# hidasib/GRU4Rec

Hardware: AMD Instinct MI355X
Metric: mini-batches/sec (gru4rec.py:661), RSC15-shaped batch=128 n_sample=2048 BPR-max (higher is better)
Workload: dtype f32

## Files before the change

gru4rec_amd/build.py:

```python
import glob
import os
import subprocess
import sys

HERE = os.path.dirname(os.path.abspath(__file__))
SRC = os.path.join(HERE, 'csrc', 'g4r_api.hip')
SRC_HOST = os.path.join(HERE, 'csrc', 'g4r_io.cpp')
OUT = os.path.join(HERE, 'libgru4rec_hip.so')
DEPS = sorted(p for ext in ('hip', 'cuh', 'hpp', 'cpp') for p in glob.glob(os.path.join(HERE, 'csrc', '*.' + ext))) + \
       [os.path.join(os.path.dirname(HERE), 'include', 'gru4rec_hip.h'), os.path.abspath(__file__)]


def build(force=False, verbose=False, out=None, defs=(), flags=()):
    if out is not None:
        return _compile(out, list(defs), verbose, list(flags))
    if not force and os.path.exists(OUT) and all(os.path.getmtime(OUT) >= os.path.getmtime(d) for d in DEPS):
        return OUT
    return _compile(OUT, [], verbose)


COMMON_FLAGS = ['-mllvm', '-amdgpu-kernarg-preload-count=16']


MUTANTS = {1: 'sparse accumulator increments x 1.01', 2: 'sparse Adagrad steps x 1.01', 3: 'dense accumulator increments x 1.01',
           4: "round 3's stale-register pipeline of gemm_tile2k (tied wait operands in two branches): fails the ISA audit, so it is the "
              "one library built with audit=False",
           5: 'the 1 / nranks factor of the exact-replica joint update (REDUCE / MEAN forms) x 1.01',
           6: 'the Adagrad step of ONE item row per step (the item of score column 0) x 1.5: a single wrong row must not pass',
           7: 'top-k selection (g4r_recommend_step) breaks equal scores by the HIGHER column',
           8: "k_update_l's owner scan skips the last id of every 1024-id slice after the first (an occurrence of a hot item lost)",
           9: "the merge-time exclusion search of g4r_recommend_step_filtered never matches the LAST item of a row's sorted list",
           10: "k_replay_final (g4r_recommend_sessions) reads every row's final state from the buffer of the chunk's LONGEST history",
           11: "k_score_cand (g4r_score_candidates*): a work item past a row's first slice reads the items of the row's first slice",
           12: "the two-stage top-k (g4r_recommend_*_scan) ranks its candidates by the APPROXIMATE bf16 scores: the fp32 re-scoring is skipped",
           13: "cosine (g4r_similar_items): the candidate's inverse norm is read at the candidate POSITION instead of its item index",
           14: "k_rollout_feed (g4r_continue_sessions): the sorted insertion drops an item that sorts ABOVE every item already in the row's "
               "exclusion list, so it is never excluded and can be generated again",
           15: "k_beam_advance (g4r_beam_sessions) reads the hidden state of beam row i ITSELF instead of the row of its parent: a new beam "
               "carries on from the wrong state wherever the selection re-parents",
           16: "the owner walk of k_sparse_update_generic drops the first hit of every pass after the first (an item with more than 64 "
               "earlier occurrences in a step loses one of them per later pass)",
           17: "opt_rule's new second statistic (adadelta's update average, Adam's mean) x 1.01",
           18: "k_loss_rows' grp_fast takes a group of V columns whose last column is the first inactive in-batch one (column M) as wholly "
               "active: the unmasked copy of the element loops runs over it",
           19: "k_loss_rows' first pass starts its loop past the prefetched groups one STEP late: the columns of the first trip keep "
               "whatever the LDS held",
           20: "gumbel_noise (g4r_sample_sessions) ignores the decoding step (Philox counter word 2 = 0): every step of a draw gets the "
               "noise of step 0"}


def mutant_path(k):
    return os.path.join(HERE, '_variants', 'libgru4rec_hip_mut%d.so' % k)


def build_mutants(force=False, verbose=False):
    import fcntl
    from concurrent.futures import ThreadPoolExecutor
    os.makedirs(os.path.join(HERE, '_variants'), exist_ok=True)

    def stale():
        return [k for k in MUTANTS if force or not os.path.exists(mutant_path(k)) or
                any(os.path.getmtime(mutant_path(k)) < os.path.getmtime(d) for d in DEPS)]
    if not stale():
        return [mutant_path(k) for k in MUTANTS]
    with open(os.path.join(HERE, '_variants', '.lock'), 'w') as lock:
        fcntl.flock(lock, fcntl.LOCK_EX)
        todo = stale()
        if todo:
            _host_object(verbose)
            with ThreadPoolExecutor(min(len(todo), 2)) as ex:
                list(ex.map(lambda k: _device(mutant_path(k), ['G4R_MUTATE=%d' % k], verbose, audit=(k != 4)), todo))
    return [mutant_path(k) for k in MUTANTS]


def _host_object(verbose):
    obj = os.path.join(HERE, 'csrc', 'g4r_io.o')
    host = [os.environ.get('CXX', 'g++'), '-O3', '-std=c++17', '-fPIC', '-pthread', '-c', SRC_HOST, '-o', obj]
    if verbose:
        print(' '.join(host))
    subprocess.check_call(host)
    return obj


class AuditError(RuntimeError):
    """The generated code uses the destination of a hand-counted asm load before the wait that retires it (isa_audit.py)."""


def hipcc_version():
    rocm = os.environ.get('ROCM_PATH', '/opt/rocm')
    try:
        out = subprocess.run([os.path.join(rocm, 'bin', 'hipcc'), '--version'], capture_output=True, text=True).stdout
    except OSError:
        return 'unknown'
    hip = [ln for ln in out.splitlines() if ln.startswith('HIP version')]
    return hip[0].split(':', 1)[1].strip() if hip else 'unknown'


def build_dir(OUT):
    return os.path.join(HERE, '_build', os.path.splitext(os.path.basename(OUT))[0])


def kernels_without_device_code(lib, device_kernels):
    import re
    blob = open(lib, 'rb').read()
    out = []
    for mt in set(re.findall(rb'_Z(\d+)__device_stub__(\w+)', blob)):
        n = int(mt[0]) - len('__device_stub__')
        name, rest = mt[1][:n].decode(), mt[1][n:].decode()
        sym = '_Z%d%s%s' % (n, name, rest)
        if sym not in device_kernels:
            out.append(sym)
    return sorted(out)


def _device(OUT, defs, verbose, audit=True, flags=()):
    import glob
    import json
    import shutil
    from . import isa_audit
    rocm = os.environ.get('ROCM_PATH', '/opt/rocm')
    obj = os.path.join(HERE, 'csrc', 'g4r_io.o')
    trace = ['-DG4R_CLK_TRACE'] if os.environ.get('G4R_BUILD_CLK') else []
    tmp = build_dir(OUT)
    shutil.rmtree(tmp, ignore_errors=True)
    os.makedirs(tmp)
    ver = hipcc_version()
    cmd = [os.path.join(rocm, 'bin', 'hipcc'), '--offload-arch=gfx950', '-O3', '-std=c++17', '-shared', '-fPIC', '-save-temps=obj',
           '-DG4R_HIPCC_VERSION="%s"' % ver] + COMMON_FLAGS + list(flags) + trace + ['-D' + d for d in defs] + [
           '-I' + os.path.join(rocm, 'include'), '-o', os.path.join(tmp, os.path.basename(OUT)), SRC, '-Wl,' + obj, '-pthread',
           '-L' + os.path.join(rocm, 'lib'), '-lrccl', '-Wl,-rpath,' + os.path.join(rocm, 'lib')]
    if verbose:
        print(' '.join(cmd))
    subprocess.check_call(cmd)
    listing = glob.glob(os.path.join(tmp, '*amdgcn*gfx950.s'))
    if len(listing) != 1:
        raise AuditError('no device listing next to the library (%s): cannot audit the asm loads' % tmp)
    asm = open(listing[0]).read()
    findings, counted = isa_audit.audit(asm)
    with open(os.path.join(tmp, 'resources.json'), 'w') as f:
        json.dump({'hipcc': ver, 'validated_hipcc': isa_audit.VALIDATED_HIPCC, 'asm_register_loads': counted,
                   'audit_findings': [list(x) for x in findings], 'kernels': isa_audit.resources(asm)}, f, indent=1, sort_keys=True)
    for junk in glob.glob(os.path.join(tmp, '*')):
        if not (junk.endswith('gfx950.s') or junk.endswith('resources.json') or junk.endswith('.so')):
            os.remove(junk)
    built = os.path.join(tmp, os.path.basename(OUT))
    missing = kernels_without_device_code(built, isa_audit.resources(asm))
    if missing:
        os.remove(built)
        if os.path.exists(OUT):
            os.remove(OUT)
        raise AuditError('the host code launches %d kernel(s) the device code does not hold (a __global__ template is only emitted for an '
                         'explicit instantiation: g4r_eval_kernels.cuh), first: %s -- library NOT installed' % (len(missing), missing[0]))
    if findings and audit:
        os.remove(built)
        if os.path.exists(OUT):
            os.remove(OUT)
        raise AuditError('%d premature use(s) of an asm load destination in the code %s generated, first: %s line %d `%s` names '
                         'in-flight v%s -- library NOT installed (gru4rec_amd/isa_audit.py)' % ((len(findings), ver) + tuple(findings[0])))
    if not any('k_score_bwd2' in k for k in counted) and audit:
        os.remove(built)
        raise AuditError('the audit no longer sees the asm loads of k_score_bwd2 it was written for: %s' % sorted(counted))
    os.replace(built, OUT)
    return OUT


def _compile(OUT, defs, verbose, flags=()):
    _host_object(verbose)
    return _device(OUT, defs, verbose, flags=flags)


if __name__ == '__main__':
    if '--variant' in sys.argv:
        k = sys.argv.index('--variant')
        rest = sys.argv[k + 2:]
        print(build(out=os.path.abspath(sys.argv[k + 1]), defs=[a for a in rest if not a.startswith('-')],
                    flags=[a for a in rest if a.startswith('-')], verbose=True))
    else:
        print(build(force='--force' in sys.argv, verbose=True))
```

gru4rec_amd/csrc/g4r_device.cuh:

```cuda
#pragma once
#include <hip/hip_runtime.h>
#include <stdint.h>

#include "../../include/gru4rec_hip.h"

typedef float f32x4 __attribute__((ext_vector_type(4)));

#define G4R_EPS_LOSS 1e-24f
#define G4R_EPS_ADAGRAD 1e-6f
#define G4R_OWN_INLINE 15

#if defined(G4R_MUTATE) && G4R_MUTATE == 1
#define G4R_MUT_ACC(x) ((x) * 1.01f)
#else
#define G4R_MUT_ACC(x) (x)
#endif
#if defined(G4R_MUTATE) && G4R_MUTATE == 2
#define G4R_MUT_STEP(x) ((x) * 1.01f)
#else
#define G4R_MUT_STEP(x) (x)
#endif
#if defined(G4R_MUTATE) && G4R_MUTATE == 3
#define G4R_MUT_DACC(x) ((x) * 1.01f)
#else
#define G4R_MUT_DACC(x) (x)
#endif

#if defined(G4R_MUTATE) && G4R_MUTATE == 6
#define G4R_MUT_ROW(n, x) ((n) == 0 ? (x) * 1.5f : (x))
#else
#define G4R_MUT_ROW(n, x) (x)
#endif
#if defined(G4R_MUTATE) && G4R_MUTATE == 8
#define G4R_MUT_SLICE_SKIP(j, base0, start) ((base0) > (start) && (j) == (base0) + 1023)
#else
#define G4R_MUT_SLICE_SKIP(j, base0, start) false
#endif
#if defined(G4R_MUTATE) && G4R_MUTATE == 5
#define G4R_MUT_XSCALE(x) ((x) * 1.01f)
#else
#define G4R_MUT_XSCALE(x) (x)
#endif
#if defined(G4R_MUTATE) && G4R_MUTATE == 16
#define G4R_MUT_PASS_SKIP(pass, ri) ((pass) > 0 && (ri) == 0)
#else
#define G4R_MUT_PASS_SKIP(pass, ri) false
#endif
#if defined(G4R_MUTATE) && G4R_MUTATE == 17
#define G4R_MUT_STAT2(x) ((x) * 1.01f)
#else
#define G4R_MUT_STAT2(x) (x)
#endif
#if defined(G4R_MUTATE) && G4R_MUTATE == 18
#define G4R_MUT_FAST_M(M) ((M) + 1)
#else
#define G4R_MUT_FAST_M(M) (M)
#endif
#if defined(G4R_MUTATE) && G4R_MUTATE == 19
#define G4R_MUT_FIRST_LATE(step) (step)
#else
#define G4R_MUT_FIRST_LATE(step) 0
#endif

#define G4R_STREAM_SAMPLE 0x53414D50u
#define G4R_STREAM_DROP_EMBED 0x44454D42u
#define G4R_STREAM_DROP_HIDDEN 0x44484944u
#define G4R_STREAM_TIEBREAK 0x54494542u

#if defined(__HIP_DEVICE_COMPILE__)
#define GAS __attribute__((address_space(1)))
#else
#define GAS
#endif
#define GP(T) GAS T*

__device__ __forceinline__ float4 ld4(const GAS float* p) { return *(const GAS float4*)p; }
__device__ __forceinline__ void st4(GAS float* p, float4 v) { *(GAS float4*)p = v; }
__device__ __forceinline__ int4 ldi4(const GAS int* p) { return *(const GAS int4*)p; }
#if defined(__HIP_DEVICE_COMPILE__)
__device__ __forceinline__ float4 ld4(const float* p) { return *(const float4*)p; }
__device__ __forceinline__ void st4(float* p, float4 v) { *(float4*)p = v; }
#endif
__device__ __forceinline__ float4 ld4_if(const GAS float* base, size_t off, bool ok) {
    const float4 v = ld4(base + (ok ? off : (size_t)0));
    return make_float4(ok ? v.x : 0.f, ok ? v.y : 0.f, ok ? v.z : 0.f, ok ? v.w : 0.f);
}
__device__ __forceinline__ float4 ld4_at(const GAS float* base, size_t off, bool ok) { return ld4(base + (ok ? off : (size_t)0)); }
__device__ __forceinline__ float ldf_at(const GAS float* base, size_t off, bool ok) { return base[ok ? off : (size_t)0]; }
__device__ __forceinline__ float ldf_if(const GAS float* base, size_t off, bool ok) {
    const float v = base[ok ? off : (size_t)0];
    return ok ? v : 0.f;
}

#define G4R_NORM_BLOCKS 256

struct StepState {
    long long t_a, t_b;
    long long g_a, g_b;
    int M_a, M_b;
    int nan_flag;
    int pad;
};

struct DevModel {
    int n_items, n_layers, B, ns, N, R, ldSc;
    int loss, final_act, hidden_act, embed_mode;
    float fa_p0, fa_p1, ha_p0, ha_p1;
    float lr, mom, lmbd, bpreg, logq, inv_B, smoothing, pad_f;
    int generic, adapt;
    float ap0, ap1, grad_cap, pad_g;
    GP(float) acc2Wy; GP(float) acc2By; GP(float) acc2E; GP(float) cntWy; GP(float) cntBy; GP(float) cntE;
    GP(float) dense_acc2; GP(float) dense_cnt;
    GP(float) gsq_part;
    GP(float) gclip;
    float drop_h, drop_e;
    unsigned long long seed;
    int D[G4R_MAX_LAYERS], IN[G4R_MAX_LAYERS];
    int Dtop, Ein;
    int offWx[G4R_MAX_LAYERS], offWh[G4R_MAX_LAYERS], offWrz[G4R_MAX_LAYERS], offBh[G4R_MAX_LAYERS];
    int dense_count;
    GP(float) dense_p; GP(float) dense_acc; GP(float) dense_vel; GP(float) dense_g;
    int apply_dense_inplace;
    float grad_scale;
    GP(float) Wy; GP(float) accWy; GP(float) velWy; GP(float) By; GP(float) accBy; GP(float) velBy;
    GP(float) E; GP(float) accE; GP(float) velE;
    GP(float) H[G4R_MAX_LAYERS][2];
    GP(float) r[G4R_MAX_LAYERS]; GP(float) z[G4R_MAX_LAYERS]; GP(float) c[G4R_MAX_LAYERS];
    GP(float) hd[G4R_MAX_LAYERS]; GP(float) Hr[G4R_MAX_LAYERS];
    GP(float) dV[G4R_MAX_LAYERS]; GP(float) dyl[G4R_MAX_LAYERS]; GP(float) Vc[G4R_MAX_LAYERS];
    GP(float) Sc; GP(float) dSx; GP(float) dSy; GP(float) dSBy; GP(float) dhpart; GP(float) lossrow; GP(float) loss_steps;
    GP(float) dAx; GP(float) dAy; GP(float) dABy;
    int ksplit, kch;
    GP(float) yin0;
    GP(int) occ_idx;
    GP(int) col_item;
    GP(int) cur_in;
    GP(int) cur_col;
    GP(int) occ_fl;
    GP(unsigned char) touched;
    GP(const int) in_idx; GP(const int) out_idx; GP(const int) Mplan;
    GP(const unsigned char) reset;
    GP(const int) ST;
    int gl;
    GP(const float) lq_tgt; GP(const float) lq_smp;
    GP(StepState) st;
    GP(long long) dbgclk;
    GP(const float) zrow;
    GP(long long) dbgtile;
    GP(float) xbase;
    long long xstride;
    int xn, xoffSx, xoffSy, xoffSBy;
    int xmode, xoffDg;
    GP(float) dyp;
    int bbn[G4R_MAX_LAYERS];
    GP(float) vp;
    int defer_mask, dRcap;
    long long dSx_stride, dSy_stride, dSBy_stride;
    GP(int) last_use;
    GP(int) dcand;
    GP(int) dlist;
    GP(unsigned) dstat;
    GP(float) drp;
    GP(int) own_pos;
};
#define G4R_SLOT(m, g) ((size_t)((g) & (long long)(m).defer_mask))
#define G4R_DSX(m, g) ((m).dSx + G4R_SLOT(m, g) * (size_t)(m).dSx_stride)
#define G4R_DSY(m, g) ((m).dSy + G4R_SLOT(m, g) * (size_t)(m).dSy_stride)
#define G4R_DSBY(m, g) ((m).dSBy + G4R_SLOT(m, g) * (size_t)(m).dSBy_stride)

#if defined(G4R_CLK_TRACE)
#define G4R_DBGCLK(m) ((m).dbgclk)
#define G4R_DBGTILE(m) ((m).dbgtile)
#else
#define G4R_DBGCLK(m) ((GAS long long*)nullptr)
#define G4R_DBGTILE(m) ((GAS long long*)nullptr)
#endif
#define G4R_TICK(m, kern, phase)                                                                     \
    do {                                                                                             \
        if (G4R_DBGCLK(m) && blockIdx.x == 0 && blockIdx.y == 0 && threadIdx.x == 0)                  \
            G4R_DBGCLK(m)[(kern) * 16 + (phase)] = wall_clock64();                                       \
    } while (0)

template <int CTRL>
__device__ __forceinline__ float dpp_mov(float v) {
    return __builtin_bit_cast(float, __builtin_amdgcn_update_dpp(0, __builtin_bit_cast(int, v), CTRL, 0xF, 0xF, true));
}
__device__ __forceinline__ float readlane_f(float v, int l) {
    return __builtin_bit_cast(float, __builtin_amdgcn_readlane(__builtin_bit_cast(int, v), l));
}
__device__ __forceinline__ float wave_sum(float v) {
    v += dpp_mov<0xB1>(v);
    v += dpp_mov<0x4E>(v);
    v += dpp_mov<0x141>(v);
    v += dpp_mov<0x140>(v);
    return (readlane_f(v, 0) + readlane_f(v, 16)) + (readlane_f(v, 32) + readlane_f(v, 48));
}
__device__ __forceinline__ float wave_max(float v) {
    v = fmaxf(v, dpp_mov<0xB1>(v));
    v = fmaxf(v, dpp_mov<0x4E>(v));
    v = fmaxf(v, dpp_mov<0x141>(v));
    v = fmaxf(v, dpp_mov<0x140>(v));
    return fmaxf(fmaxf(readlane_f(v, 0), readlane_f(v, 16)), fmaxf(readlane_f(v, 32), readlane_f(v, 48)));
}

__device__ __forceinline__ float block_sum_256(float v, float* red) {
    v = wave_sum(v);
    const int lane = threadIdx.x & 63, w = threadIdx.x >> 6;
    __syncthreads();
    if (lane == 0) red[w] = v;
    __syncthreads();
    return (red[0] + red[1]) + (red[2] + red[3]);
}
__device__ __forceinline__ float block_max_256(float v, float* red) {
    v = wave_max(v);
// ... 120 lines not shown
```

gru4rec_amd/csrc/g4r_host_create.hpp:

```cpp

int g4r_device_count(void) {
    int n = 0;
    if (hipGetDeviceCount(&n) != hipSuccess) return 0;
    return n;
}
const char* g4r_last_error(void) { return g_err.c_str(); }
#ifndef G4R_HIPCC_VERSION
#define G4R_HIPCC_VERSION "unknown"
#endif
const char* g4r_version(void) { return "gru4rec_hip 0.4 (gfx950; hipcc " G4R_HIPCC_VERSION "; isa-audited)"; }
int g4r_sizeof_config(void) { return (int)sizeof(g4r_config); }

static int build_lean_args(g4r_model* m) {
    DevModel& d = m->dm;
    const StepKernels& k = m->kern;
    const int L = d.n_layers;
    std::vector<LeanV> av(L); std::vector<LeanH> ah(L); std::vector<LeanDa> aa(L); std::vector<LeanDy> ay(L);
    const bool constrained = d.embed_mode == G4R_EMBED_CONSTRAINED;
    bool any_layer = false;
    for (int l = 0; l < L; ++l) {
        if (k.fwd[l] != FWD_LEAN) continue;
        any_layer = true;
        LeanV& v = av[l]; memset(&v, 0, sizeof(v));
        v.Wx = d.dense_p + d.offWx[l]; v.Wrz = d.dense_p + d.offWrz[l]; v.Bh = d.dense_p + d.offBh[l];
        v.H0 = d.H[l][0]; v.H1 = d.H[l][1];
        v.ysrc = (l == 0) ? (constrained ? d.Wy : d.E) : d.hd[l - 1];
        v.cur_in = d.cur_in; v.Vc = d.Vc[l]; v.r = d.r[l]; v.Hr = d.Hr[l]; v.z = d.z[l]; v.yin0 = d.yin0;
        v.occ_idx = d.occ_idx; v.occ_fl = d.occ_fl + 4 * (constrained ? (size_t)0 : (size_t)d.n_items);
        v.st = d.st; v.seed = d.seed; v.B = d.B; v.D = d.D[l]; v.IN = d.IN[l]; v.R = d.R; v.first = (l == 0) ? 1 : 0; v.pub_fl = d.xmode == 0 ? 1 : 0;
        v.drop_e = d.drop_e; v.dbg = d.dbgclk; v.dbgtile = d.dbgtile; v.n_items = d.n_items;
        LeanH& h = ah[l]; memset(&h, 0, sizeof(h));
        h.Wh = d.dense_p + d.offWh[l]; h.H0 = d.H[l][0]; h.H1 = d.H[l][1]; h.Hr = d.Hr[l]; h.Vc = d.Vc[l]; h.z = d.z[l];
        h.cur_rst = d.cur_in + d.B; h.c = d.c[l]; h.hd = d.hd[l]; h.st = d.st; h.seed = d.seed; h.B = d.B; h.D = d.D[l];
        h.hidden_act = d.hidden_act; h.stream = (int)(G4R_STREAM_DROP_HIDDEN + (unsigned)l); h.ha_p0 = d.ha_p0; h.ha_p1 = d.ha_p1; h.drop_h = d.drop_h; h.dbg = d.dbgclk; h.dbgtile = d.dbgtile;
        LeanDa& q = aa[l]; memset(&q, 0, sizeof(q));
        q.Wh = h.Wh; q.H0 = h.H0; q.H1 = h.H1; q.z = d.z[l]; q.c = d.c[l];
        if (l == L - 1) { q.dsrc = d.dhpart; q.ks = d.ksplit; }
        else if (d.bbn[l + 1] > 0) { q.dsrc = d.dyp; q.ks = d.bbn[l + 1]; }
        else { q.dsrc = d.dyl[l]; q.ks = 1; }
        q.dV = d.dV[l]; q.drp = d.drp; q.st = d.st; q.seed = d.seed; q.B = d.B; q.D = d.D[l]; q.hidden_act = d.hidden_act; q.stream = h.stream;
        q.ha_p0 = d.ha_p0; q.ha_p1 = d.ha_p1; q.drop_h = d.drop_h; q.dbg = d.dbgclk; q.dbgtile = d.dbgtile;
        LeanDy& y = ay[l]; memset(&y, 0, sizeof(y));
        y.Wx = v.Wx; y.H0 = h.H0; y.H1 = h.H1; y.r = d.r[l]; y.drp = d.drp; y.dV = d.dV[l]; y.occ_idx = d.occ_idx; y.occ_fl = v.occ_fl;
        y.accT = constrained ? d.accWy : d.accE; y.dSx = d.dSx; y.dAx = d.dAx; y.dylo = (l > 0) ? d.dyl[l - 1] : nullptr;
        y.st = d.st; y.seed = d.seed; y.dSx_stride = d.dSx_stride; y.B = d.B; y.D = d.D[l]; y.IN = d.IN[l]; y.layer0 = (l == 0) ? 1 : 0;
        y.generic = d.generic; y.defer_mask = d.defer_mask; y.lr = d.lr; y.drop_e = d.drop_e; y.dbg = d.dbgclk; y.dbgtile = d.dbgtile; y.n_items = d.n_items;
    }
    m->h_leanV = av; m->h_leanH = ah; m->h_leanDa = aa; m->h_leanDy = ay;
    if (any_layer) {
        if (dalloc(m, &m->d_leanV, (size_t)L) || dalloc(m, &m->d_leanH, (size_t)L) || dalloc(m, &m->d_leanDa, (size_t)L) || dalloc(m, &m->d_leanDy, (size_t)L)) return -1;
        HIPCHK(hipMemcpyAsync(m->d_leanV, av.data(), L * sizeof(LeanV), hipMemcpyHostToDevice, m->stream));
        HIPCHK(hipMemcpyAsync(m->d_leanH, ah.data(), L * sizeof(LeanH), hipMemcpyHostToDevice, m->stream));
        HIPCHK(hipMemcpyAsync(m->d_leanDa, aa.data(), L * sizeof(LeanDa), hipMemcpyHostToDevice, m->stream));
        HIPCHK(hipMemcpyAsync(m->d_leanDy, ay.data(), L * sizeof(LeanDy), hipMemcpyHostToDevice, m->stream));
    }
    if (k.score_fwd == SF_LEAN) {
        LeanS q; memset(&q, 0, sizeof(q));
        q.col_item = d.col_item; q.occ_idx = d.occ_idx + d.B; q.occ_fl = d.occ_fl; q.mp = nullptr; q.dbg = d.dbgclk; q.dbgtile = d.dbgtile; q.R = d.R; q.pub_fl = d.xmode == 0 ? 1 : 0; q.logq = d.logq;
        m->h_leanS = q;
        if (dalloc(m, &m->d_leanS, (size_t)1)) return -1;
    }
    if (k.score_bwd == SB_LEAN) {
        LeanB q; memset(&q, 0, sizeof(q));
        q.accBy = d.accBy; q.occ_fl = d.occ_fl; q.dSy = d.dSy; q.dAy = d.dAy; q.dSBy = d.dSBy; q.dABy = d.dABy; q.dhpart = d.dhpart; q.dbg = d.dbgclk; q.dbgtile = d.dbgtile;
        q.dSy_stride = d.dSy_stride; q.dSBy_stride = d.dSBy_stride; q.defer_mask = d.defer_mask; q.generic = d.generic;
        q.ndh = cdiv(d.Dtop + 1, 64); q.nA = cdiv(d.ldSc, 16) * q.ndh; q.nrb = cdiv(d.B, 16); q.ndb = cdiv(d.Dtop, 64); q.lr = d.lr;
        m->h_leanB = q;
        if (dalloc(m, &m->d_leanB, (size_t)1)) return -1;
        HIPCHK(hipMemcpyAsync(m->d_leanB, &m->h_leanB, sizeof(LeanB), hipMemcpyHostToDevice, m->stream));
    }
    if (k.update == UP_LEAN) {
        LeanU u; memset(&u, 0, sizeof(u));
        u.mp = nullptr; u.st = d.st; u.Wy = d.Wy; u.E = d.E; u.accWy = d.accWy; u.accE = d.accE; u.velWy = d.velWy; u.velE = d.velE;
        u.By = d.By; u.accBy = d.accBy; u.velBy = d.velBy; u.dAx = d.dAx; u.dAy = d.dAy; u.dABy = d.dABy;
        u.dense_p = d.dense_p; u.dense_acc = d.dense_acc; u.dense_vel = d.dense_vel; u.yin0 = d.yin0; u.meta = d.cur_in + 2 * d.B;
        u.dbg = d.dbgclk; u.dbgtile = d.dbgtile; u.n_items = d.n_items; u.constrained = constrained ? 1 : 0; u.wE = d.Ein; u.wY = d.Dtop;
        u.lr = d.lr; u.mom = d.mom; u.lmbd = d.lmbd;
        m->h_leanU = u;
        const std::vector<DenseTile> tiles = dense_tiles(d, 16, 64);
        m->ntiles16 = (int)tiles.size();
        const size_t nslot = cdiv((long long)d.R * 16 * sizeof(int), (long long)sizeof(DenseTile));
        if (dalloc(m, &m->d_tiles16, tiles.size() + nslot) || dalloc(m, &m->d_leanU, (size_t)1)) return -1;
        d.own_pos = m->sw.owner_scan_in_update ? nullptr : (int*)(m->d_tiles16 + tiles.size());
        m->h_leanU.own_on = d.own_pos ? 1 : 0;
        HIPCHK(hipMemcpyAsync(m->d_tiles16, tiles.data(), tiles.size() * sizeof(DenseTile), hipMemcpyHostToDevice, m->stream));
        HIPCHK(hipStreamSynchronize(m->stream));
    }
    HIPCHK(hipStreamSynchronize(m->stream));
    return 0;
}

static KernelSwitches read_switches(const g4r_config& cfg) {
    KernelSwitches w;
    w.no_lean = getenv("G4R_NO_LEAN") != nullptr; w.no_mt = getenv("G4R_NO_MT") != nullptr; w.no_bmt = getenv("G4R_NO_BMT") != nullptr;
    w.no_merge = getenv("G4R_NO_MERGE") != nullptr; w.owner_scan_in_update = env_int("G4R_OWNER_SCAN", 0) != 0;
    w.score_b_split = env_int("G4R_SCORE_B_SPLIT", 1) != 0;
    w.allow_lean_update = env_int("G4R_LEAN_UPDATE", 1) != 0; w.defer = env_int("G4R_DEFER", cfg.defer_updates) != 0;
    w.p2_geo = env_int("G4R_P2_GEO", -1); w.ba_geo = env_int("G4R_BA_GEO", -1);
    w.wide2 = env_int("G4R_WIDE2", -1); w.p1_ks = env_int("G4R_P1_KS", 128); w.bb_ks = env_int("G4R_BB_KS", 0);
    const char* skip = getenv("G4R_SKIP_KN");
    w.skip_kn = skip ? strtoull(skip, nullptr, 0) : 0ull;
    return w;
}

int g4r_create(const g4r_config* cfg, g4r_model** out) {
    if (!cfg || !out) return fail("null argument");
    if (cfg->n_layers < 1 || cfg->n_layers > G4R_MAX_LAYERS) return fail("n_layers out of range");
    if (cfg->batch_size < 1 || cfg->n_items < 1) return fail("batch_size / n_items must be positive");
    for (int l = 0; l < cfg->n_layers; ++l)
        if (cfg->layers[l] % 4 != 0 || cfg->layers[l] < 4 || cfg->layers[l] > 1024)
            return fail("layer sizes must be multiples of 4 in [4, 1024]");
    if (cfg->embed_mode == G4R_EMBED_SEPARATE && (cfg->embedding % 4 != 0 || cfg->embedding < 4 || cfg->embedding > 1024))
        return fail("embedding must be a multiple of 4 in [4, 1024]");
    if (cfg->embed_mode != G4R_EMBED_CONSTRAINED && cfg->embed_mode != G4R_EMBED_SEPARATE && cfg->embed_mode != G4R_EMBED_ONEHOT)
        return fail("unsupported embedding mode");
    if (cfg->embed_mode == G4R_EMBED_ONEHOT && 3 * cfg->layers[0] > 1024)
        return fail("one-hot input: 3 * layers[0] must be <= 1024 (row width of the Wx[0] table)");
    if (cfg->loss < 0 || cfg->loss > G4R_LOSS_XE_LOGIT) return fail("unsupported loss");
    if (cfg->smoothing != 0.f && cfg->loss != G4R_LOSS_XE && cfg->loss != G4R_LOSS_XE_LOGIT) return fail("smoothing needs a cross-entropy loss");
    if (cfg->hidden_act == G4R_ACT_SOFTMAX_LOGIT) return fail("softmax_logit is not a hidden activation");
    if (cfg->adapt < 0 || cfg->adapt > G4R_ADAPT_NONE) return fail("unknown adapt");
    if (cfg->grad_cap < 0.f) return fail("grad_cap must be >= 0");
    if (cfg->hidden_act == G4R_ACT_SOFTMAX) return fail("softmax is not a hidden activation");
    int ndev = g4r_device_count();
    if (ndev <= 0) return fail("no HIP device visible: the gfx950 path has no CPU fallback");
    if (cfg->device < 0 || cfg->device >= ndev) return fail("device ordinal out of range");
    HIPCHK(hipSetDevice(cfg->device));
    int n_cu = 0;
    HIPCHK(hipDeviceGetAttribute(&n_cu, hipDeviceAttributeMultiprocessorCount, cfg->device));
    g4r_model* m = new g4r_model();
    m->cfg = *cfg;
    m->n_cu = std::max(n_cu, 1);
    if (hipStreamCreateWithFlags(&m->stream, hipStreamNonBlocking) != hipSuccess) { delete m; return fail("stream create"); }
    DevModel& d = m->dm;
    memset(&d, 0, sizeof(d));
    const int L = cfg->n_layers, B = cfg->batch_size;
    d.n_items = cfg->n_items; d.n_layers = L; d.B = B;
    const int ns = std::max(cfg->n_sample, 0);
    int64_t gl = (ns > 0 && cfg->sample_store > 0) ? cfg->sample_store / ns : 0;
    if (ns > 0 && gl <= 1) gl = 1;
    m->gl = gl;
    d.ns = ns; d.N = B + ns; d.R = 2 * B + ns; d.ldSc = (d.N + 15) & ~15;
    d.gl = (int)std::max<int64_t>(gl, 1);
    d.loss = cfg->loss; d.final_act = cfg->final_act; d.hidden_act = cfg->hidden_act; d.embed_mode = cfg->embed_mode;
    d.fa_p0 = cfg->final_act_p0; d.fa_p1 = cfg->final_act_p1; d.ha_p0 = cfg->hidden_act_p0; d.ha_p1 = cfg->hidden_act_p1;
    d.lr = cfg->learning_rate; d.mom = cfg->momentum; d.lmbd = cfg->lmbd; d.bpreg = cfg->bpreg; d.logq = cfg->logq;
    d.inv_B = 1.0f / (float)B;
    d.smoothing = cfg->smoothing;
    d.adapt = cfg->adapt; d.ap0 = cfg->adapt_p0; d.ap1 = cfg->adapt_p1; d.grad_cap = cfg->grad_cap;
    const bool exact = cfg->sparse_exact != 0 && (cfg->nranks > 1 || getenv("G4R_FORCE_STAGED") != nullptr);
    if (cfg->sparse_exact != 0 && cfg->grad_cap > 0.f) { g4r_destroy(m); return fail("sparse_exact does not support grad_cap (the norm would be per rank)"); }
    m->exact = exact;
    d.generic = (cfg->adapt != G4R_ADAPT_ADAGRAD || cfg->grad_cap > 0.f || exact) ? 1 : 0;
    d.drop_h = cfg->dropout_p_hidden; d.drop_e = cfg->dropout_p_embed;
    d.seed = cfg->seed + ((cfg->sparse_exact != 0 && cfg->nranks > 1) ? 7919ull * (unsigned long long)cfg->rank : 0ull);
    d.Dtop = cfg->layers[L - 1];
    d.Ein = (cfg->embed_mode == G4R_EMBED_CONSTRAINED) ? d.Dtop : (cfg->embed_mode == G4R_EMBED_ONEHOT ? 3 * cfg->layers[0] : cfg->embedding);
    int off = 0;
    for (int l = 0; l < L; ++l) {
        d.D[l] = cfg->layers[l];
        d.IN[l] = (l == 0) ? (cfg->embed_mode == G4R_EMBED_ONEHOT ? 0 : d.Ein) : cfg->layers[l - 1];
        d.offWx[l] = off; off += d.IN[l] * 3 * d.D[l];
        d.offWh[l] = off; off += d.D[l] * d.D[l];
        d.offWrz[l] = off; off += d.D[l] * 2 * d.D[l];
        d.offBh[l] = off; off += 3 * d.D[l];
    }
    d.dense_count = off;
    d.apply_dense_inplace = (cfg->nranks <= 1 && !getenv("G4R_FORCE_STAGED") && !d.generic) ? 1 : 0;
    d.grad_scale = 1.0f / (float)std::max(cfg->nranks, 1);
    d.xn = exact ? cfg->nranks : 1;
    d.xmode = exact ? std::min(std::max(cfg->sparse_exact, 1), 3) : 0;
    m->sw = read_switches(*cfg);
    if (m->sw.skip_kn)
        fprintf(stderr, "[g4r] G4R_SKIP_KN=0x%llx: launches are left out of every training step -- its results are invalid (a measurement aid)\n", m->sw.skip_kn);
    m->defer_on = d.apply_dense_inplace && !d.generic && cfg->momentum <= 0.f && cfg->lmbd == 0.f && m->sw.defer;
    m->kern = choose_kernels(d, m->n_cu, m->sw, m->defer_on);
    const StepKernels& k = m->kern;
    d.kch = k.kch; d.ksplit = k.ksplit;
    for (int l = 0; l < L; ++l) d.bbn[l] = (k.wg[l].use & 8) ? k.wg[l].bbn : 0;
    const size_t I = cfg->n_items;
#define DA(p, n) if (dalloc(m, &(p), (n))) { g4r_destroy(m); return -1; }
    DA(d.dense_p, off); DA(d.dense_acc, off); DA(d.dense_vel, off); DA(d.dense_g, off);
    DA(d.Wy, I * d.Dtop); DA(d.accWy, I * d.Dtop); DA(d.By, I); DA(d.accBy, I);
    if (cfg->momentum > 0.f) { DA(d.velWy, I * d.Dtop); DA(d.velBy, I); }
    if (cfg->embed_mode != G4R_EMBED_CONSTRAINED) {
        DA(d.E, I * d.Ein); DA(d.accE, I * d.Ein);
        if (cfg->momentum > 0.f) DA(d.velE, I * d.Ein);
    }
    if (d.generic) {
        const bool two = (cfg->adapt == G4R_ADAPT_ADADELTA || cfg->adapt == G4R_ADAPT_ADAM), cnt = (cfg->adapt == G4R_ADAPT_ADAM);
        if (two) { DA(d.acc2Wy, I * d.Dtop); DA(d.acc2By, I); DA(d.dense_acc2, off); if (d.E) DA(d.acc2E, I * d.Ein); }
        if (cnt) { DA(d.cntWy, I * d.Dtop); DA(d.cntBy, I); DA(d.dense_cnt, off); if (d.E) DA(d.cntE, I * d.Ein); }
        DA(d.gsq_part, G4R_NORM_BLOCKS); DA(d.gclip, 1);
        const float one = 1.f;
        if (hipMemcpyAsync(d.gclip, &one, sizeof(float), hipMemcpyHostToDevice, m->stream) != hipSuccess || hipStreamSynchronize(m->stream) != hipSuccess) {
            g4r_destroy(m); return fail("gclip init");
        }
    }
    int maxD = 0;
    for (int l = 0; l < L; ++l) {
        const size_t bd = (size_t)B * d.D[l];
        maxD = std::max(maxD, d.D[l]);
        DA(d.H[l][0], bd); DA(d.H[l][1], bd);
        DA(d.r[l], bd); DA(d.z[l], bd); DA(d.c[l], bd); DA(d.hd[l], bd); DA(d.Hr[l], bd);
        DA(d.dV[l], bd * 3); DA(d.dyl[l], bd); DA(d.Vc[l], bd);
    }
    DA(m->d_tmpH, (size_t)B * maxD);
    {
        size_t drp_floats = 0;
        for (int l = 0; l < L; ++l) if (k.fwd[l] == FWD_LEAN) drp_floats = std::max(drp_floats, (size_t)cdiv(d.D[l], 16) * B * d.D[l]);
        if (drp_floats) DA(d.drp, drp_floats);
    }
    DA(d.yin0, (size_t)B * std::max(d.IN[0], 4));
    DA(d.Sc, (size_t)B * d.ldSc);
    {
        auto up64 = [](size_t n) { return (n + 63) & ~(size_t)63; };
        const size_t nOcc = up64((size_t)((d.R + 255) & ~255) + 256 + 64);
        d.xoffSx = (int)nOcc;
        d.xoffSy = (int)(nOcc + up64((size_t)B * d.Ein));
        d.xoffSBy = (int)(d.xoffSy + up64((size_t)d.ldSc * d.Dtop));
        d.xoffDg = (int)(d.xoffSBy + up64((size_t)d.ldSc));
        d.xstride = (long long)(d.xoffDg + (exact ? up64((size_t)d.dense_count) : 0));
        float* xb = nullptr;
        DA(xb, (size_t)d.xn * (size_t)d.xstride);
        d.xbase = xb;
        float* own = xb + (size_t)(exact ? cfg->rank : 0) * (size_t)d.xstride;
        d.occ_idx = (int*)own; d.dSx = own + d.xoffSx; d.dSy = own + d.xoffSy; d.dSBy = own + d.xoffSBy;
        if (exact) d.dense_g = own + d.xoffDg;
    }
    DA(d.dAx, (size_t)B * d.Ein); DA(d.dAy, (size_t)d.ldSc * d.Dtop); DA(d.dABy, d.ldSc);
    if (m->defer_on) {
        const size_t W = G4R_DEFER_SLOTS;
        d.defer_mask = (int)W - 1;
        d.dRcap = cdiv(d.R, SP_WAVES) * SP_WAVES;
        d.dSx_stride = (long long)(((size_t)B * d.Ein + 63) & ~(size_t)63);
        d.dSy_stride = (long long)(((size_t)d.ldSc * d.Dtop + 63) & ~(size_t)63);
        d.dSBy_stride = (long long)(((size_t)d.ldSc + 63) & ~(size_t)63);
        float *rx = nullptr, *ry = nullptr, *rb = nullptr;
        DA(rx, W * (size_t)d.dSx_stride); DA(ry, W * (size_t)d.dSy_stride); DA(rb, W * (size_t)d.dSBy_stride);
        d.dSx = rx; d.dSy = ry; d.dSBy = rb;
        DA(d.last_use, (size_t)(cfg->embed_mode != G4R_EMBED_CONSTRAINED ? 2 : 1) * I);
        DA(d.dcand, W * (size_t)d.dRcap); DA(d.dlist, W * (size_t)d.dRcap); DA(d.dstat, 2048);
        if (hipMemsetAsync(d.dlist, 0xFF, W * (size_t)d.dRcap * sizeof(int), m->stream) != hipSuccess) { g4r_destroy(m); return fail("dlist init"); }
        for (auto& e : m->ev_df) if (hipEventCreate(&e) != hipSuccess) { g4r_destroy(m); return fail("event create"); }
    }
    DA(d.lossrow, B);
    DA(d.col_item, d.ldSc); DA(d.cur_in, 2 * (size_t)B + 8); DA(d.cur_col, d.ldSc);
    DA(d.occ_fl, (size_t)(cfg->embed_mode != G4R_EMBED_CONSTRAINED ? 2 : 1) * I * 4);
    DA(d.st, 1);
    DA(d.dhpart, (size_t)d.ksplit * B * d.Dtop);
    m->nblk_occ = cdiv(d.R, SP_WAVES);
    m->nblk_occ_g = m->nblk_occ;
    m->smem_sparse = (size_t)(((d.R + 255) & ~255) + 256) * sizeof(int) + (2 + 64) * SP_WAVES * sizeof(int) +
                     (size_t)SP_WAVES * (std::max(d.Dtop, d.Ein) + 4) * sizeof(float);
    if (ns > 0) DA(m->d_ST, (size_t)gl * ns);
    d.ST = m->d_ST;
    auto tile_table = [&](int edge, DenseTile** dst, int* n) {
        const std::vector<DenseTile> tiles = dense_tiles(d, edge, edge);
        *n = (int)tiles.size();
        return dalloc(m, dst, tiles.size()) == 0 && hipMemcpyAsync(*dst, tiles.data(), tiles.size() * sizeof(DenseTile), hipMemcpyHostToDevice, m->stream) == hipSuccess &&
               hipStreamSynchronize(m->stream) == hipSuccess;
    };
    if (!tile_table(32, &m->d_tiles, &m->ntiles) || (k.wide_dense && !tile_table(64, &m->d_tiles64, &m->ntiles64))) { g4r_destroy(m); return fail("tile upload"); }
    {
        size_t dyp_floats = 0, vp_floats = 0;
        for (int l = 0; l < L; ++l) {
            const WideGeo& G = k.wg[l];
            if (G.use & 1) vp_floats = std::max(vp_floats, (size_t)(G.ny + G.nh) * B * 3 * d.D[l]);
            if (G.use & 8) dyp_floats = std::max(dyp_floats, (size_t)G.bbn * B * d.IN[l]);
        }
        if (dyp_floats) DA(d.dyp, dyp_floats);
        if (vp_floats) DA(d.vp, vp_floats);
    }
#undef DA
    m->smem_score = ((size_t)(SC_BM + 32) * (SC_KC + 2) + 32) * sizeof(float);
    m->smem_loss = (size_t)((k.loss_long ? 1 : 2) * d.ldSc + 18 * LOSS_NW) * sizeof(float);
    const int big = 156 * 1024;
    HIPCHK(hipFuncSetAttribute((const void*)k_gru_p1_n32, hipFuncAttributeMaxDynamicSharedMemorySize, big));
    HIPCHK(hipFuncSetAttribute((const void*)k_gru_p1_n64, hipFuncAttributeMaxDynamicSharedMemorySize, big));
    HIPCHK(hipFuncSetAttribute((const void*)k_gru_p2_w4, hipFuncAttributeMaxDynamicSharedMemorySize, big));
    HIPCHK(hipFuncSetAttribute((const void*)k_gru_p2_w8d, hipFuncAttributeMaxDynamicSharedMemorySize, big));
    HIPCHK(hipFuncSetAttribute((const void*)k_score_fwd_k128, hipFuncAttributeMaxDynamicSharedMemorySize, big));
    HIPCHK(hipFuncSetAttribute((const void*)k_score_fwd_k64, hipFuncAttributeMaxDynamicSharedMemorySize, big));
    HIPCHK(hipFuncSetAttribute((const void*)k_score_fwd_t2, hipFuncAttributeMaxDynamicSharedMemorySize, big));
    HIPCHK(hipFuncSetAttribute((const void*)k_score_fwd_t3, hipFuncAttributeMaxDynamicSharedMemorySize, big));
    HIPCHK(hipFuncSetAttribute((const void*)k_score_mt_4s, hipFuncAttributeMaxDynamicSharedMemorySize, big));
    HIPCHK(hipFuncSetAttribute((const void*)k_score_bmt, hipFuncAttributeMaxDynamicSharedMemorySize, big));
    HIPCHK(hipFuncSetAttribute((const void*)k_score_bwd_n, hipFuncAttributeMaxDynamicSharedMemorySize, big));
    HIPCHK(hipFuncSetAttribute((const void*)k_gru_bwd_fused, hipFuncAttributeMaxDynamicSharedMemorySize, big));
    HIPCHK(hipFuncSetAttribute((const void*)k_gru_fwd_fused, hipFuncAttributeMaxDynamicSharedMemorySize, big));
    HIPCHK(hipFuncSetAttribute((const void*)k_score_bwd_w, hipFuncAttributeMaxDynamicSharedMemorySize, big));
    HIPCHK(hipFuncSetAttribute((const void*)k_score_bwd2, hipFuncAttributeMaxDynamicSharedMemorySize, big));
    HIPCHK(hipFuncSetAttribute((const void*)k_gru_bwd_a_w4, hipFuncAttributeMaxDynamicSharedMemorySize, big));
    HIPCHK(hipFuncSetAttribute((const void*)k_gru_bwd_a_w8d, hipFuncAttributeMaxDynamicSharedMemorySize, big));
    HIPCHK(hipFuncSetAttribute((const void*)k_gru_bwd_b, hipFuncAttributeMaxDynamicSharedMemorySize, big));
    HIPCHK(hipFuncSetAttribute((const void*)k_dense_grad<32>, hipFuncAttributeMaxDynamicSharedMemorySize, big));
    HIPCHK(hipFuncSetAttribute((const void*)k_sparse_update<1, false>, hipFuncAttributeMaxDynamicSharedMemorySize, big));
    HIPCHK(hipFuncSetAttribute((const void*)k_sparse_update<1, true>, hipFuncAttributeMaxDynamicSharedMemorySize, big));
    HIPCHK(hipFuncSetAttribute((const void*)k_sparse_update<2, false>, hipFuncAttributeMaxDynamicSharedMemorySize, big));
    HIPCHK(hipFuncSetAttribute((const void*)k_sparse_update<2, true>, hipFuncAttributeMaxDynamicSharedMemorySize, big));
    HIPCHK(hipFuncSetAttribute((const void*)k_sparse_update_generic<1>, hipFuncAttributeMaxDynamicSharedMemorySize, big));
    HIPCHK(hipFuncSetAttribute((const void*)k_sparse_update_generic<2>, hipFuncAttributeMaxDynamicSharedMemorySize, big));
    HIPCHK(hipFuncSetAttribute((const void*)k_sparse_update<4, false>, hipFuncAttributeMaxDynamicSharedMemorySize, big));
    HIPCHK(hipFuncSetAttribute((const void*)k_sparse_update<4, true>, hipFuncAttributeMaxDynamicSharedMemorySize, big));
    HIPCHK(hipFuncSetAttribute((const void*)k_sparse_update_generic<4>, hipFuncAttributeMaxDynamicSharedMemorySize, big));
    HIPCHK(hipFuncSetAttribute((const void*)k_update<1, 32, false>, hipFuncAttributeMaxDynamicSharedMemorySize, big));
    HIPCHK(hipFuncSetAttribute((const void*)k_update<1, 32, true>, hipFuncAttributeMaxDynamicSharedMemorySize, big));
    HIPCHK(hipFuncSetAttribute((const void*)k_update<2, 32, false>, hipFuncAttributeMaxDynamicSharedMemorySize, big));
    HIPCHK(hipFuncSetAttribute((const void*)k_update<2, 32, true>, hipFuncAttributeMaxDynamicSharedMemorySize, big));
    HIPCHK(hipFuncSetAttribute((const void*)k_score_store, hipFuncAttributeMaxDynamicSharedMemorySize, big));
    HIPCHK(hipFuncSetAttribute((const void*)k_score_count, hipFuncAttributeMaxDynamicSharedMemorySize, big));
    HIPCHK(hipFuncSetAttribute((const void*)k_topk_fused, hipFuncAttributeMaxDynamicSharedMemorySize, big));
    HIPCHK(hipFuncSetAttribute((const void*)k_topk_stored, hipFuncAttributeMaxDynamicSharedMemorySize, big));
    HIPCHK(hipFuncSetAttribute((const void*)k_topk_fused_x, hipFuncAttributeMaxDynamicSharedMemorySize, big));
    HIPCHK(hipFuncSetAttribute((const void*)k_topk_stored_x, hipFuncAttributeMaxDynamicSharedMemorySize, big));
    HIPCHK(hipFuncSetAttribute((const void*)k_topk_fused_g, hipFuncAttributeMaxDynamicSharedMemorySize, big));
    HIPCHK(hipFuncSetAttribute((const void*)k_topk_stored_g, hipFuncAttributeMaxDynamicSharedMemorySize, big));
    HIPCHK(hipFuncSetAttribute((const void*)k_topk_sample, hipFuncAttributeMaxDynamicSharedMemorySize, big));
    HIPCHK(hipFuncSetAttribute((const void*)k_topk_rank, hipFuncAttributeMaxDynamicSharedMemorySize, big));
    HIPCHK(hipFuncSetAttribute((const void*)k_topk_rank_x, hipFuncAttributeMaxDynamicSharedMemorySize, big));
    HIPCHK(hipFuncSetAttribute((const void*)k_topk_stored_ev, hipFuncAttributeMaxDynamicSharedMemorySize, big));
    HIPCHK(hipFuncSetAttribute((const void*)k_sim_range<false>, hipFuncAttributeMaxDynamicSharedMemorySize, big));
    HIPCHK(hipFuncSetAttribute((const void*)k_sim_range<true>, hipFuncAttributeMaxDynamicSharedMemorySize, big));
    HIPCHK(hipFuncSetAttribute((const void*)k_scan_bf16<2>, hipFuncAttributeMaxDynamicSharedMemorySize, big));
    HIPCHK(hipFuncSetAttribute((const void*)k_scan_bf16<4>, hipFuncAttributeMaxDynamicSharedMemorySize, big));
    HIPCHK(hipFuncSetAttribute((const void*)k_scan_bf16<8>, hipFuncAttributeMaxDynamicSharedMemorySize, big));
    HIPCHK(hipFuncSetAttribute((const void*)k_scan_bf16<2, TkGrow>, hipFuncAttributeMaxDynamicSharedMemorySize, big));
    HIPCHK(hipFuncSetAttribute((const void*)k_scan_bf16<4, TkGrow>, hipFuncAttributeMaxDynamicSharedMemorySize, big));
    HIPCHK(hipFuncSetAttribute((const void*)k_scan_bf16<8, TkGrow>, hipFuncAttributeMaxDynamicSharedMemorySize, big));
#define G4R_LOSS_ATTR(L, S)                                                                                                    \
    if (!L) HIPCHK(hipFuncSetAttribute((const void*)k_loss_rows<false, S, 1>, hipFuncAttributeMaxDynamicSharedMemorySize, big)); \
    HIPCHK(hipFuncSetAttribute((const void*)k_loss_rows<L, S, 4>, hipFuncAttributeMaxDynamicSharedMemorySize, big))
    G4R_LOSS_ATTR(false, 0); G4R_LOSS_ATTR(false, 1); G4R_LOSS_ATTR(false, 2); G4R_LOSS_ATTR(false, 3);
    G4R_LOSS_ATTR(true, 0); G4R_LOSS_ATTR(true, 1); G4R_LOSS_ATTR(true, 2); G4R_LOSS_ATTR(true, 3);
#undef G4R_LOSS_ATTR
    if (m->smem_loss > (size_t)big) { g4r_destroy(m); return fail("batch_size + n_sample too large for the row-loss kernel (one copy of a score row must fit the 160 KB of LDS)"); }
    if (m->smem_sparse > (size_t)big) { g4r_destroy(m); return fail("2 * batch_size + n_sample too large for the sparse update (the step's list of gathered rows must fit the 160 KB of LDS)"); }
    if (m->exact) {
        const size_t rlist = d.xmode == 3 ? (size_t)d.xn * 2 * B + d.ns : (size_t)d.R * d.xn;
        m->smem_exact = (size_t)(((rlist + 255) & ~(size_t)255) + 256) * sizeof(int) + 64 * SP_WAVES * sizeof(int);
        if (m->smem_exact > (size_t)big) {
            g4r_destroy(m);
            return fail("sparse_exact: the exchanged occurrence list (REDUCE form: nranks * 2 * batch_size + n_sample entries; MEAN / SUM: nranks * (2 * batch_size + n_sample)) does not fit the 160 KB of LDS the update stages it in -- use the GPU-local mode (sync_every) at this shape");
        }
    }
    { float* z = nullptr; if (dalloc(m, &z, ZROW_FLOATS)) { g4r_destroy(m); return -1; } d.zrow = z; }
    if (getenv("G4R_CLK")) {
        if (dalloc(m, &d.dbgclk, 64 + 8 * (size_t)d.R) || dalloc(m, &d.dbgtile, 8 * (size_t)(4096 + 4096))) { g4r_destroy(m); return -1; }
    }
    if (build_lean_args(m)) { g4r_destroy(m); return -1; }
    if (dalloc(m, &m->d_dm, 1) || sync_dm(m)) { g4r_destroy(m); return -1; }
    if (m->d_leanU) {
        m->h_leanU.mp = m->d_dm;
        if (hipMemcpyAsync(m->d_leanU, &m->h_leanU, sizeof(LeanU), hipMemcpyHostToDevice, m->stream) != hipSuccess || hipStreamSynchronize(m->stream) != hipSuccess) { g4r_destroy(m); return fail("lean args upload"); }
    }
    if (m->d_leanS) {
        m->h_leanS.mp = m->d_dm;
        if (hipMemcpyAsync(m->d_leanS, &m->h_leanS, sizeof(LeanS), hipMemcpyHostToDevice, m->stream) != hipSuccess || hipStreamSynchronize(m->stream) != hipSuccess) { g4r_destroy(m); return fail("lean args upload"); }
    }
    *out = m;
    return 0;
}

void g4r_destroy(g4r_model* m) {
    if (!m) return;
    (void)hipSetDevice(m->cfg.device);
    if (m->stream) (void)hipStreamSynchronize(m->stream);
    if (m->gexec) (void)hipGraphExecDestroy(m->gexec);
    if (m->gexec_small) (void)hipGraphExecDestroy(m->gexec_small);
    if (m->gexec_head) (void)hipGraphExecDestroy(m->gexec_head);
    if (m->comm_ready) (void)ncclCommDestroy(m->comm);
    for (void* q : m->p2p_peer) if (q) (void)hipIpcCloseMemHandle(q);
    if (m->p2p_region) (void)hipFree(m->p2p_region);
    for (auto e : m->evs) (void)hipEventDestroy(e);
    for (auto e : m->ev_df) if (e) (void)hipEventDestroy(e);
    for (g4r_model::Scratch* sc : {&m->sc_ids, &m->sc_blk, &m->sc_cnt, &m->sc_all, &m->sc_send, &m->sc_pack, &m->sc_recv, &m->sc_hall}) {
        if (sc->p) { if (sc->host) (void)hipHostFree(sc->p); else (void)hipFree(sc->p); }
        sc->p = nullptr; sc->cap = 0;
    }
    for (void* p : m->allocs) (void)hipFree(p);
    if (m->stream) (void)hipStreamDestroy(m->stream);
    delete m;
}
```

gru4rec_amd/csrc/g4r_host_debug.hpp:

```cpp
int g4r_get_debug(g4r_model* m, const char* name, float* host, int64_t count) {
    if (!m || !name || !host) return fail("null argument");
    HIPCHK(hipSetDevice(m->cfg.device));
    DevModel& d = m->dm;
    const StepKernels& k = m->kern;
    std::string s(name);
    const float* p = nullptr; int64_t n = 0;
    int l = 0;
    if (!s.empty() && isdigit((unsigned char)s.back())) { l = s.back() - '0'; s.pop_back(); }
    if (l >= d.n_layers) return fail("layer out of range");
    const int64_t bd = (int64_t)d.B * d.D[l];
    if (s == "scores") { p = d.Sc; n = (int64_t)d.B * d.ldSc; }
    else if (s == "dSx") { p = d.dSx + (size_t)((m->gstep - 1) & d.defer_mask) * (size_t)d.dSx_stride; n = (int64_t)d.B * d.Ein; }
    else if (s == "dSy") { p = d.dSy + (size_t)((m->gstep - 1) & d.defer_mask) * (size_t)d.dSy_stride; n = (int64_t)d.ldSc * d.Dtop; }
    else if (s == "dSBy") { p = d.dSBy + (size_t)((m->gstep - 1) & d.defer_mask) * (size_t)d.dSBy_stride; n = d.ldSc; }
    else if (s == "defer_stats") {
        if (count < 4) return fail("count");
        double rows = 0, bias = 0;
        if (m->defer_on) {
            std::vector<unsigned> st(2048);
            HIPCHK(hipStreamSynchronize(m->stream));
            HIPCHK(hipMemcpy(st.data(), d.dstat, st.size() * sizeof(unsigned), hipMemcpyDeviceToHost));
            for (size_t i = 0; i < st.size(); i += 2) { rows += st[i]; bias += st[i + 1]; }
        }
        host[0] = (float)rows; host[1] = (float)bias; host[2] = m->defer_on ? 1.f : 0.f; host[3] = (float)(d.defer_mask + 1);
        return 0;
    }
    else if (s == "scan_table") {
        if (count < 3) return fail("count");
        host[0] = (float)((double)m->s_tab.cap * 16.0); host[1] = m->s_tab_valid ? 1.f : 0.f; host[2] = (float)m->s_tab_builds;
        return 0;
    }
    else if (s == "sim_norms") {
        if (count < 3) return fail("count");
        host[0] = (float)(((m->sim_inv[0] ? 1.0 : 0.0) + (m->sim_inv[1] ? 1.0 : 0.0)) * (double)d.n_items * 4.0);
        host[1] = (m->sim_valid[0] || m->sim_valid[1]) ? 1.f : 0.f; host[2] = (float)m->sim_builds;
        return 0;
    }
    else if (s == "continue_steps") {
        if (count < 2) return fail("count");
        host[0] = (float)m->ro_calls; host[1] = (float)m->ro_steps;
        return 0;
    }
    else if (s == "events_launches") {
        if (count < 4) return fail("count");
        host[0] = (float)m->ev_steps; host[1] = (float)m->ev_scans; host[2] = (float)m->ev_launches; host[3] = (float)m->ev_pieces;
        return 0;
    }
    else if (s == "dhpart") { p = d.dhpart; n = (int64_t)d.ksplit * d.B * d.Dtop; }
    else if (s == "lossrow") { p = d.lossrow; n = d.B; }
    else if (s == "hd") { p = d.hd[l]; n = bd; }
    else if (s == "r") { p = d.r[l]; n = bd; }
    else if (s == "z") { p = d.z[l]; n = bd; }
    else if (s == "c") { p = d.c[l]; n = bd; }
    else if (s == "Hr") { p = d.Hr[l]; n = bd; }
    else if (s == "dV") { p = d.dV[l]; n = bd * 3; }
    else if (s == "dyl") { p = d.dyl[l]; n = bd; }
    else if (s == "Hprev") { p = d.H[l][(m->gstep + 1) & 1]; n = bd; }
    else if (s == "occ_idx") { p = (const float*)d.occ_idx; n = d.R; }
    else if (s == "own_pos") { if (!d.own_pos) return fail("no owner table (k_update_l not chosen, or G4R_OWNER_SCAN=1)"); p = (const float*)d.own_pos; n = 16 * (int64_t)d.R; }
#if !defined(G4R_CLK_TRACE)
    else if (s == "dbgclk" || s == "dbgtile") return fail("in-kernel traces need a library built with G4R_BUILD_CLK=1 (python -m gru4rec_amd.build --force) and G4R_CLK=1 at run time");
#endif
    else if (s == "dbgclk") { if (!d.dbgclk) return fail("G4R_CLK not set"); p = (const float*)d.dbgclk; n = 2 * (64 + 8 * (int64_t)d.R); }
    else if (s == "dbgtile") { if (!d.dbgtile) return fail("G4R_CLK not set"); p = (const float*)d.dbgtile; n = 2 * 8 * (int64_t)8192; }
    else if (s == "ntiles") { if (count < 1) return fail("count"); host[0] = (float)m->ntiles; return 0; }
    else if (s == "ldSc") { if (count < 1) return fail("count"); host[0] = (float)d.ldSc; return 0; }
    else if (s == "wide_mask") {
        if (count < 1) return fail("count");
        int mk = k.wide_dense ? 16 : 0;
        for (int l = 0; l < d.n_layers; ++l) mk |= k.wg[l].use;
        host[0] = (float)mk; return 0;
    }
    else if (s == "deep_geo") {
        if (count < 1) return fail("count");
        host[0] = (float)(k.p2_deep[0] + 2 * k.ba_deep[0]); return 0;
    }
    else if (s == "score_mt") { if (count < 1) return fail("count"); host[0] = k.score_fwd == SF_MT ? 272.f : 0.f; return 0; }
    else if (s == "score_bmt") { if (count < 1) return fail("count"); host[0] = (float)k.bmt_slabs; return 0; }
    else if (s == "lean") {
        if (count < 4) return fail("count");
        int mk = 0;
        for (int l = 0; l < d.n_layers; ++l) mk |= k.fwd[l] == FWD_LEAN ? 1 << l : 0;
        host[0] = (float)mk; host[1] = k.score_fwd == SF_LEAN ? 1.f : 0.f; host[2] = k.score_bwd == SB_LEAN ? 1.f : 0.f;
        host[3] = k.update == UP_LEAN ? 1.f : 0.f;
        return 0;
    }
    else if (s == "kernels") {
        const int ML = G4R_MAX_LAYERS;
        const int tail[] = {k.score_fwd, k.loss_spec, k.loss_long, k.loss_quads, k.score_bwd, k.kch, k.ksplit, k.bmt_slabs, k.update, k.chunks, k.wide_dense, k.finish_rows};
        if (count < 4 * ML + 12) return fail("count");
        for (int i = 0; i < 4 * ML + 12; ++i) host[i] = i < 4 * ML ? 0.f : (float)tail[i - 4 * ML];
        for (int l = 0; l < d.n_layers; ++l) {
            host[l] = (float)k.fwd[l]; host[ML + l] = (float)k.bwd[l]; host[2 * ML + l] = (float)(k.p2_deep[l] + 2 * k.ba_deep[l]); host[3 * ML + l] = (float)k.wg[l].use;
        }
        return 0;
    }
    else if (s == "generic") { if (count < 1) return fail("count"); host[0] = (float)d.generic; return 0; }
    else if (s == "score_b_split") { if (count < 1) return fail("count"); host[0] = (float)k.score_a_host; return 0; }
    else if (s == "n_cu") { if (count < 1) return fail("count"); host[0] = (float)m->n_cu; return 0; }
    else if (s == "ksplit") { if (count < 1) return fail("count"); host[0] = (float)d.ksplit; return 0; }
    else if (s == "dev_syncs") { if (count < 1) return fail("count"); host[0] = (float)m->n_dev_syncs; return 0; }
    else if (s == "dense_count") { if (count < 1) return fail("count"); host[0] = (float)d.dense_count; return 0; }
    else if (s == "occ_score_tile") {
        if (count < 1) return fail("count");
        int nb = 0;
        for (size_t lds = SMEM_SF2; lds >= SMEM_SF2 - 2048; lds -= 512) {
            HIPCHK(hipOccupancyMaxActiveBlocksPerMultiprocessor(&nb, (const void*)k_score_fwd_t2, GT_NTH, lds));
            fprintf(stderr, "[g4r] k_score_fwd_t2 dynamic LDS %zu -> %d workgroups per CU\n", lds, nb);
        }
        host[0] = (float)nb;
        return 0;
    }
    else if (s == "graph_mode") {
        if (count < 1) return fail("count");
        host[0] = m->gexec ? 1.f : (m->gexec_head ? 2.f : 0.f);
        return 0;
    }
    else return fail(std::string("unknown debug buffer ") + name);
    if (count != n) return fail(std::string("size mismatch for debug buffer ") + name + " expected " + std::to_string(n));
    HIPCHK(hipStreamSynchronize(m->stream));
    HIPCHK(hipMemcpy(host, p, n * sizeof(float), hipMemcpyDeviceToHost));
    return 0;
}

int g4r_debug_loss_rows(g4r_model* m, float* scores, int64_t count, int32_t M, float* lossrow) {
    if (!m || !scores || !lossrow) return fail("null argument");
    DevModel& d = m->dm;
    if (count != (int64_t)d.B * d.ldSc) return fail("size mismatch for the score rows: expected " + std::to_string((int64_t)d.B * d.ldSc));
    if (M < 1 || M > d.B) return fail("M outside [1, batch_size]");
    HIPCHK(hipSetDevice(m->cfg.device));
    HIPCHK(hipStreamSynchronize(m->stream));
    StepState saved, mine;
    HIPCHK(hipMemcpy(&saved, (const void*)d.st, sizeof(saved), hipMemcpyDeviceToHost));
    HIPCHK(hipMemcpy((void*)d.Sc, scores, (size_t)count * sizeof(float), hipMemcpyHostToDevice));
    mine = saved;
    mine.M_b = M;
    HIPCHK(hipMemcpy((void*)d.st, &mine, sizeof(mine), hipMemcpyHostToDevice));
    launch_loss_rows(m, dim3(d.B), false, nullptr, nullptr);
    hipError_t e = hipGetLastError();
    if (e == hipSuccess) e = hipStreamSynchronize(m->stream);
    const hipError_t r = hipMemcpy((void*)d.st, &saved, sizeof(saved), hipMemcpyHostToDevice);
    if (e != hipSuccess) return fail(std::string("k_loss_rows: ") + hipGetErrorString(e));
    if (r != hipSuccess) return fail(std::string("step state: ") + hipGetErrorString(r));
    HIPCHK(hipMemcpy(scores, (const void*)d.Sc, (size_t)count * sizeof(float), hipMemcpyDeviceToHost));
    HIPCHK(hipMemcpy(lossrow, (const void*)d.lossrow, (size_t)d.B * sizeof(float), hipMemcpyDeviceToHost));
    return 0;
}

int g4r_debug_gumbel(g4r_model* m, uint64_t seed, uint32_t row_id, uint32_t step, const int32_t* items, int64_t n, float* out) {
    if (!m || !items || !out) return fail("null argument");
    if (n < 1) return fail("n must be positive");
    for (int64_t p = 0; p < n; ++p)
        if (items[p] < 0) return fail("item index out of range");
    HIPCHK(hipSetDevice(m->cfg.device));
    CallTemps tmp(m);
    int* d_it = nullptr;
    float* d_out = nullptr;
    if (tmp.get(&d_it, (size_t)n, false) || tmp.get(&d_out, (size_t)n, false)) return -1;
    HIPCHK(hipMemcpyAsync(d_it, items, (size_t)n * sizeof(int32_t), hipMemcpyHostToDevice, m->stream));
    hipLaunchKernelGGL(k_debug_gumbel, dim3((unsigned)((n + 255) / 256)), dim3(256), 0, m->stream, (unsigned long long)seed, (unsigned)row_id,
                       (unsigned)step, (const int*)d_it, (long long)n, d_out);
    HIPCHK(hipGetLastError());
    HIPCHK(hipMemcpyAsync(out, d_out, (size_t)n * sizeof(float), hipMemcpyDeviceToHost, m->stream));
    HIPCHK(hipStreamSynchronize(m->stream));
    return 0;
}

int g4r_bench_rows(int32_t device, int64_t n_items, int32_t W, int64_t rows_per_launch, int32_t launches, int32_t mode, uint64_t seed,
                   double* kernel_us, double* wall_us) {
    if (n_items < 1 || W < 4 || W % 4 != 0 || W > 512 || rows_per_launch < 1 || launches < 1 || mode < 0 || mode > 2 || !kernel_us || !wall_us)
        return fail("bad argument");
    if (device < 0 || device >= g4r_device_count()) return fail("device ordinal out of range");
    HIPCHK(hipSetDevice(device));
    float *table = nullptr, *acc = nullptr, *buf = nullptr;
    int* idx = nullptr;
    hipStream_t s = nullptr;
    std::vector<hipEvent_t> ev;
    auto cleanup = [&]() {
        (void)hipFree(table); (void)hipFree(acc); (void)hipFree(buf); (void)hipFree(idx);
        for (auto e : ev) (void)hipEventDestroy(e);
        if (s) (void)hipStreamDestroy(s);
    };
#define MBCHK(x) do { hipError_t e_ = (x); if (e_ != hipSuccess) { cleanup(); return fail(std::string(#x ": ") + hipGetErrorString(e_)); } } while (0)
    const size_t tab = (size_t)n_items * W;
    const int warm = 3, total = launches + warm;
    MBCHK(hipStreamCreateWithFlags(&s, hipStreamNonBlocking));
    MBCHK(hipMalloc((void**)&table, tab * sizeof(float)));
    MBCHK(hipMemsetAsync(table, 0, tab * sizeof(float), s));
    if (mode == 2) { MBCHK(hipMalloc((void**)&acc, tab * sizeof(float))); MBCHK(hipMemsetAsync(acc, 0, tab * sizeof(float), s)); }
    MBCHK(hipMalloc((void**)&buf, (size_t)rows_per_launch * W * sizeof(float)));
    MBCHK(hipMemsetAsync(buf, 0, (size_t)rows_per_launch * W * sizeof(float), s));
    std::vector<int> h((size_t)total * rows_per_launch);
    unsigned long long x = seed * 0x9E3779B97F4A7C15ull + 0x632BE59BD9B4E019ull;
    for (auto& v : h) { x ^= x >> 12; x ^= x << 25; x ^= x >> 27; v = (int)(((x * 0x2545F4914F6CDD1Dull) >> 11) % (unsigned long long)n_items); }
    MBCHK(hipMalloc((void**)&idx, h.size() * sizeof(int)));
    MBCHK(hipMemcpyAsync(idx, h.data(), h.size() * sizeof(int), hipMemcpyHostToDevice, s));
    MBCHK(hipStreamSynchronize(s));
    ev.resize(2 * (size_t)launches + 2);
    for (auto& e : ev) MBCHK(hipEventCreate(&e));
    const long long waves = (rows_per_launch + MB_RPW - 1) / MB_RPW;
    const dim3 grid((unsigned)((waves + 3) / 4)), block(256);
    for (int l = 0; l < total; ++l) {
        const int* ix = idx + (size_t)l * rows_per_launch;
        const int t = l - warm;
        if (t == 0) MBCHK(hipEventRecord(ev[2 * (size_t)launches], s));
        hipEvent_t a = t >= 0 ? ev[2 * (size_t)t] : nullptr, b = t >= 0 ? ev[2 * (size_t)t + 1] : nullptr;
        if (W <= 256) hipExtLaunchKernelGGL(k_micro_rows<1>, grid, block, 0, s, a, b, 0, (const float*)table, acc, ix, buf, (long long)rows_per_launch, (int)W, (int)mode);
        else hipExtLaunchKernelGGL(k_micro_rows<2>, grid, block, 0, s, a, b, 0, (const float*)table, acc, ix, buf, (long long)rows_per_launch, (int)W, (int)mode);
    }
    MBCHK(hipEventRecord(ev[2 * (size_t)launches + 1], s));
    MBCHK(hipStreamSynchronize(s));
    MBCHK(hipGetLastError());
// ... 76 lines not shown
```

gru4rec_amd/csrc/g4r_host_model.hpp:

```cpp
static thread_local std::string g_err;
static int fail(const std::string& s) { g_err = s; return -1; }
void g4r_set_error(const char* fmt, ...) {
    char buf[1024];
    va_list ap;
    va_start(ap, fmt);
    vsnprintf(buf, sizeof(buf), fmt, ap);
    va_end(ap);
    g_err = buf;
}
#define HIPCHK(x)                                                                                        \
    do {                                                                                                 \
        hipError_t e_ = (x);                                                                             \
        if (e_ != hipSuccess)                                                                            \
            return fail(std::string(#x) + ": " + hipGetErrorString(e_) + " @" + std::to_string(__LINE__)); \
    } while (0)
#define NCCLCHK(x)                                                                                         \
    do {                                                                                                   \
        ncclResult_t e_ = (x);                                                                             \
        if (e_ != ncclSuccess)                                                                             \
            return fail(std::string(#x) + ": " + ncclGetErrorString(e_) + " @" + std::to_string(__LINE__)); \
    } while (0)

enum { KN_GRU_P1 = 0, KN_GRU_P2, KN_SCORE_FWD, KN_LOSS, KN_SCORE_BWD, KN_BWD_PRE, KN_BWD_A, KN_BWD_B, KN_DENSE, KN_ALLREDUCE,
       KN_DENSE_APPLY, KN_SPARSE, KN_UPDATE, KN_BWD_FUSED, KN_FWD_FUSED, KN_GATE, KN_FLUSH, KN_SCAN, KN_FINISH, KN_GRU_V, KN_GRU_H, KN_GRU_DA, KN_GRU_DY, KN_COUNT };
static const char* KN_NAMES[KN_COUNT] = {"k_gru_p1", "k_gru_p2", "k_score_fwd", "k_loss_rows", "k_score_bwd", "k_gru_bwd_pre",
                                         "k_gru_bwd_a", "k_gru_bwd_b", "k_dense_grad", "rccl_allreduce", "k_dense_apply",
                                         "k_sparse_update", "k_update", "k_gru_bwd", "k_gru_fwd", "k_gru_gate", "k_sparse_flush", "k_defer_scan", "k_finish_rows", "k_gru_v", "k_gru_h", "k_gru_da", "k_gru_dy"};

struct EvRec { int kn; hipEvent_t a, b; };

struct KernelSwitches {
    bool no_lean = false;
    bool no_mt = false, no_bmt = false;
    bool no_merge = false;
    bool allow_lean_update = true;
    bool score_b_split = true;
    bool owner_scan_in_update = false;
    bool defer = false;
    int p2_geo = -1, ba_geo = -1;
    int wide2 = -1, p1_ks = 128, bb_ks = 0;
    unsigned long long skip_kn = 0;
};
enum GruFwdKind { FWD_LEAN = 0 , FWD_FUSED = 1 , FWD_P1S = 2 ,
                  FWD_P1_N64 = 3, FWD_P1_N32 = 4 };
enum GruBwdKind { BWD_LEAN = 0 , BWD_FUSED = 1 , BWD_ONEHOT = 2, BWD_BW = 3, BWD_B = 4 };
enum ScoreFwdKind { SF_LEAN = 0 , SF_MT = 1 , SF_T3 = 2, SF_T2 = 3, SF_K64 = 4, SF_K128 = 5  };
enum ScoreBwdKind { SB_LEAN = 0 , SB_BMT = 1 , SB_BWD2 = 2 , SB_W = 3, SB_N = 4  };
enum UpdateKind { UP_LEAN = 0 , UP_MERGED = 1 , UP_SPLIT = 2 };
struct WideGeo { int use = 0, ny = 1, nh = 1, kys = 0, khs = 0, bbn = 1, bbk = 0; };
struct StepKernels {
    int fwd[G4R_MAX_LAYERS], bwd[G4R_MAX_LAYERS];
    int p2_deep[G4R_MAX_LAYERS], ba_deep[G4R_MAX_LAYERS];
    WideGeo wg[G4R_MAX_LAYERS];
    int score_fwd;
    int loss_spec, loss_long, loss_quads;
    int score_bwd;
    int score_a_host;
    int kch, ksplit;
    int bmt_slabs;
    int nblkA, nblkB, ndtA, ndtB, nrtB;
    int update;
    int chunks;
    int wide_dense;
    int finish_rows;
};

template <class T>
struct DevBuf {
    T* p = nullptr;
    int64_t cap = 0;
    int reserve(g4r_model* m, int64_t n);
};

struct g4r_model {
    g4r_config cfg;
    DevModel dm;
    DevModel* d_dm = nullptr;
    int n_cu = 256;
    KernelSwitches sw;
    StepKernels kern;
    hipStream_t stream = nullptr;
    std::vector<void*> allocs;
    int *d_in = nullptr, *d_out = nullptr, *d_M = nullptr, *d_cmaps = nullptr;
    unsigned char* d_reset = nullptr;
    float* d_loss = nullptr;
    int64_t T = 0, loss_cap = 0;
    std::vector<int64_t> compact_steps;
    int* d_ST = nullptr;
    float *d_P = nullptr, *d_lqt = nullptr, *d_lqs = nullptr;
    int64_t gl = 0;
    bool store_frozen = false, have_pop = false;
    unsigned refills = 0;
    int64_t gstep = 0;
    DenseTile* d_tiles = nullptr;
    int ntiles = 0, nblk_occ = 0, nblk_occ_g = 0;
    size_t smem_score = 0, smem_loss = 0, smem_sparse = 0;
    bool defer_on = false;
    bool defer_broken = false;
    hipEvent_t ev_df[4] = {nullptr, nullptr, nullptr, nullptr};
    DenseTile* d_tiles64 = nullptr;
    int ntiles64 = 0;
    float* d_tmpH = nullptr;
    LeanS h_leanS;
    std::vector<LeanV> h_leanV; std::vector<LeanH> h_leanH; std::vector<LeanDa> h_leanDa; std::vector<LeanDy> h_leanDy;
    LeanS* d_leanS = nullptr;
    LeanB* d_leanB = nullptr; LeanB h_leanB;
    LeanU* d_leanU = nullptr; LeanU h_leanU;
    DenseTile* d_tiles16 = nullptr; int ntiles16 = 0;
    LeanV* d_leanV = nullptr; LeanH* d_leanH = nullptr; LeanDa* d_leanDa = nullptr; LeanDy* d_leanDy = nullptr;
    hipGraphExec_t gexec = nullptr;
    hipGraphExec_t gexec_small = nullptr;
    hipGraphExec_t gexec_head = nullptr;
    int graph_steps = 0;
    bool dist_graph_failed = false;
    bool profiling = false;
    bool profile_split = false;
    bool exact = false;
    size_t smem_exact = 0;
    double kn_ms[KN_COUNT] = {0};
    int64_t kn_n[KN_COUNT] = {0};
    std::vector<hipEvent_t> evs;
    int pbatch = 0, ppar = 0;
    float* pH[G4R_MAX_LAYERS][2] = {{nullptr}};
    float* phout[G4R_MAX_LAYERS] = {nullptr};
    float *pVc[G4R_MAX_LAYERS] = {nullptr}, *pz[G4R_MAX_LAYERS] = {nullptr}, *pHr[G4R_MAX_LAYERS] = {nullptr};
    int *p_in = nullptr, *p_tgt = nullptr, *p_keep = nullptr;
    DevBuf<int> p_items;
    unsigned char* p_zero = nullptr;
    float* p_ranks = nullptr;
    DevBuf<float> p_scores;
    int* p_cnt = nullptr;
    int64_t p_nsel = 0, p_ldo = 0;
    DevBuf<uint2> p_topk;
    DevBuf<int> p_tcols;
    DevBuf<float> p_tscores;
    DevBuf<long long> p_xoffs;
    DevBuf<int> p_xitems;
    DevBuf<unsigned> p_xmask;
    int r_cap = 0;
    float* rH[G4R_MAX_LAYERS][2] = {{nullptr}};
    float* rhout[G4R_MAX_LAYERS] = {nullptr};
    float *rVc[G4R_MAX_LAYERS] = {nullptr}, *rz[G4R_MAX_LAYERS] = {nullptr}, *rHr[G4R_MAX_LAYERS] = {nullptr};
    float* rio[G4R_MAX_LAYERS] = {nullptr};
    int *r_perm = nullptr, *r_len = nullptr;
    DevBuf<int> r_in;
    DevBuf<float> r_scores;
    DevBuf<int> ro_cols, ro_in, ro_xlen;
    DevBuf<float> ro_scores;
    int64_t ro_calls = 0, ro_steps = 0;
    DevBuf<int> bm_in, bm_sel, bm_xlen, bm_xitems, bm_out;
    DevBuf<long long> bm_beg;
    DevBuf<unsigned> sm_rowid;
    DevBuf<int> sm_pick;
    DevBuf<float> sm_z;
    DevBuf<long long> c_offs;
    DevBuf<int> c_items;
    DevBuf<float> c_scores;
    DevBuf<int4> c_work;
    DevBuf<uint2> c_topk;
    DevBuf<int> c_tpos;
    DevBuf<float> c_tscores;
    DevBuf<uint4> s_tab;
    int64_t s_tab_builds = 0;
    bool s_tab_valid = false;
    DevBuf<int> s_cols;
    DevBuf<int> s_cnt;
    std::vector<int4> s_work;
    float* sim_inv[2] = {nullptr, nullptr};
    bool sim_valid[2] = {false, false};
    int64_t sim_builds = 0;
    DevBuf<int> sim_q;
    DevBuf<float> sim_rows;
    unsigned tie_ctr = 0;
    int64_t ev_steps = 0, ev_scans = 0, ev_launches = 0, ev_pieces = 0;
    ncclComm_t comm = nullptr;
    bool comm_ready = false;
    bool p2p_ready = false;
    void* p2p_region = nullptr;
    void* p2p_peer[G4R_P2P_MAX] = {nullptr};
    unsigned* p2p_round = nullptr;
    int p2p_nblk = 0, p2p_cap = 0;
    P2PArgs p2p_args;
    bool virtual_ranks = false;
    float* d_vsum = nullptr;
    struct SyncPlane { float* cur; float* base; int W; int kind; };
    std::vector<SyncPlane> planes[2];
    int sync_rule[2] = {G4R_SYNC_MEAN, G4R_SYNC_SUM};
    bool sync_rule_user = false;
    unsigned char* d_touched = nullptr;
    unsigned char* d_rowcnt = nullptr;
    int sync_every_dev = 0;
    int64_t since_sync = 0, n_dev_syncs = 0;
    struct Scratch { void* p = nullptr; size_t cap = 0; bool host = false; };
    Scratch sc_ids, sc_blk, sc_cnt, sc_all, sc_send, sc_pack, sc_recv, sc_hall;
    float* d_dense[2] = {nullptr, nullptr};
    bool sync_on = false;
};

static inline void weights_changed(g4r_model* m) { m->s_tab_valid = false; m->sim_valid[0] = m->sim_valid[1] = false; }

template <class T>
static int dalloc(g4r_model* m, T** p, size_t n, bool zero = true) {
    void* q = nullptr;
    if (n == 0) n = 1;
    HIPCHK(hipMalloc(&q, n * sizeof(T)));
    if (zero) HIPCHK(hipMemsetAsync(q, 0, n * sizeof(T), m->stream));
    m->allocs.push_back(q);
    *p = (T*)q;
    return 0;
}
static void dfree(g4r_model* m, void* p) {
    if (!p) return;
    auto it = std::find(m->allocs.begin(), m->allocs.end(), p);
    if (it != m->allocs.end()) m->allocs.erase(it);
    (void)hipFree(p);
}
template <class T>
int DevBuf<T>::reserve(g4r_model* m, int64_t n) {
    if (n <= cap) return 0;
    HIPCHK(hipStreamSynchronize(m->stream));
    dfree(m, p);
    p = nullptr; cap = 0;
    if (dalloc(m, &p, (size_t)n, false)) return -1;
    cap = n;
    return 0;
}
struct CallTemps {
    g4r_model* m;
    std::vector<void*> held;
    explicit CallTemps(g4r_model* m_) : m(m_) {}
    CallTemps(const CallTemps&) = delete;
    CallTemps& operator=(const CallTemps&) = delete;
    ~CallTemps() { for (void* q : held) dfree(m, q); }
    template <class T>
    int get(T** p, size_t n, bool zero = true) {
        if (dalloc(m, p, n, zero)) return -1;
        held.push_back(*p);
        return 0;
    }
};
static inline bool is_softmax(const DevModel& d) { return d.final_act == G4R_ACT_SOFTMAX || d.final_act == G4R_ACT_SOFTMAX_LOGIT; }
static inline int cdiv(long long a, long long b) { return (int)((a + b - 1) / b); }
static constexpr auto k_score_store = k_score_all<32, false>;
static constexpr auto k_score_count = k_score_all<32, true>;
static constexpr auto k_topk_fused = k_topk_range<false, false>;
static constexpr auto k_topk_stored = k_topk_range<true, false>;
static constexpr auto k_topk_fused_x = k_topk_range<false, true, TkExcl>;
static constexpr auto k_topk_stored_x = k_topk_range<true, true, TkExcl>;
static constexpr auto k_topk_fused_g = k_topk_range<false, true, TkGrow>;
static constexpr auto k_topk_stored_g = k_topk_range<true, true, TkGrow>;
static constexpr auto k_topk_sample = k_topk_range<false, true, TkSample>;
static constexpr auto k_topk_rank = k_topk_range<false, false, TkEvents>;
static constexpr auto k_topk_rank_x = k_topk_range<false, true, TkEvents>;
static constexpr auto k_topk_stored_ev = k_topk_range<true, true, TkEvents>;

static inline int env_int(const char* name, int dflt) { const char* v = getenv(name); return v ? atoi(v) : dflt; }
template <int BM, int BN, int BK, bool AKM, bool BNK>
static constexpr size_t tile_smem() { return (size_t)TileCfg<BM, BN, BK, AKM, BNK>::SMEM_FLOATS * sizeof(float); }
static const size_t SMEM_NN = tile_smem<GT_BM, GT_BN, GT_BK, false, false>() + GT_BM * sizeof(int);
static const size_t SMEM_NT = tile_smem<GT_BM, GT_BN, GT_BK, false, true>() + GT_BM * sizeof(int);
static const size_t SMEM_TN = tile_smem<GT_BM, GT_BN, GT_BK, true, false>();
static constexpr auto k_gru_p1_n32 = k_gru_p1<GT_BN, P1_BK>;
static constexpr auto k_gru_p1_n64 = k_gru_p1<64, 256>;
static const size_t SMEM_P1_N64 = tile_smem<GT_BM, 64, 256, false, false>() + GT_BM * sizeof(int);
static inline size_t smem_bwd_fused(int D) { return (size_t)((((BF_ROWS + 32) * (3 * D + 2) + D * (D + 2) + 32 + 3) & ~3) + 4 * 6 * 64) * sizeof(float); }
static inline bool wide_layer(int D) { return D >= 256; }
static const size_t SMEM_P1 = tile_smem<GT_BM, GT_BN, P1_BK, false, false>() + GT_BM * sizeof(int);
static constexpr auto k_gru_p2_w4 = k_gru_p2<GT_NTH, GT_BK>;
static constexpr auto k_gru_p2_w8d = k_gru_p2<512, 256>;
static const size_t SMEM_P2_256 = tile_smem<GT_BM, GT_BN, 256, false, false>() + GT_BM * sizeof(int);
static constexpr auto k_gru_bwd_a_w4 = k_gru_bwd_a<GT_NTH, GT_BK>;
static constexpr auto k_gru_bwd_a_w8d = k_gru_bwd_a<512, 256>;
static const size_t SMEM_BA_256 = tile_smem<GT_BM, GT_BN, 256, false, true>();
static const size_t SMEM_BB = tile_smem<GT_BM, GT_BN, BB_BK, false, true>() + GT_BM * sizeof(int);
static constexpr auto k_score_fwd_k128 = k_score_fwd<GT_BN, GT_BK>;
#define SFW_BN 32
#define SFW_BK 64
static constexpr auto k_score_fwd_k64 = k_score_fwd<SFW_BN, SFW_BK>;
static constexpr auto k_score_fwd_t2 = k_score_fwd<64, 32, T2_BK>;
static const size_t SMEM_SF2 = (size_t)Tile2Cfg<T2_BK>::SMEM_FLOATS * sizeof(float);
static constexpr auto k_score_fwd_t3 = k_score_fwd<64, 32, 3>;
static const size_t SMEM_SF3 = (size_t)Tile3Cfg<T3_NST, T3_BKS>::SMEM_FLOATS * sizeof(float);
static const size_t SMEM_BMT = std::max((size_t)BMT_NST_A * BMT_STAGE_A * sizeof(float), (size_t)BMT_NST_B * BMT_STAGE_B * sizeof(float) + 2048 * sizeof(int));
static const size_t SMEM_SF64 = tile_smem<SF_BM, SFW_BN, SFW_BK, false, true>() + SFW_BN * sizeof(int);
static constexpr auto k_score_bwd_n = k_score_bwd<32, GT_BK>;
static constexpr auto k_score_bwd_w = k_score_bwd<64, 64>;
static const size_t SMEM_SBW = std::max(tile_smem<64, 64, 64, true, false>(), tile_smem<64, 64, 64, false, false>());
#define ZROW_FLOATS 8192
#define G4R_DEFER_SLOTS 16
static const size_t SMEM_SF = tile_smem<SF_BM, GT_BN, GT_BK, false, true>() + GT_BN * sizeof(int);
static constexpr auto k_score_mt_4s = k_score_mt<4, true>;
static const size_t SMEM_MT_4S = (size_t)MtCfg<4, true>::SMEM_FLOATS * sizeof(float);
static const size_t SMEM_T2K = (size_t)(4 * 64 * 16) * sizeof(float);
static const size_t SMEM_T3 = (size_t)Tile3Cfg<3, 32>::SMEM_FLOATS * sizeof(float);

static std::vector<DenseTile> dense_tiles(const DevModel& d, int TR, int TC) {
    std::vector<DenseTile> tiles;
    for (int l = 0; l < d.n_layers; ++l) {
        const int D = d.D[l], IN = d.IN[l];
        auto add = [&](const float* x0, const float* x1, int ldx, int nrows, int ncols, int coff, int ldo, long long base) {
            for (int r = 0; r < nrows; r += TR)
                for (int c = 0; c < ncols; c += TC) {
                    DenseTile t;
                    t.X0 = x0; t.X1 = x1; t.dV = d.dV[l]; t.base = base; t.ldx = ldx; t.ldv = 3 * D; t.nrows = nrows;
                    t.ncols = ncols; t.coff = coff; t.ldo = ldo; t.r0 = r; t.c0 = c; t.gather = (x0 == nullptr && nrows > 1) ? 1 : 0; t.pad = 0;
                    tiles.push_back(t);
                }
        };
        const float* yin = (l == 0) ? nullptr : d.hd[l - 1];
        add(yin, yin, IN, IN, 3 * D, 0, 3 * D, d.offWx[l]);
        add(d.Hr[l], d.Hr[l], D, D, D, 0, D, d.offWh[l]);
        add(d.H[l][0], d.H[l][1], D, D, 2 * D, D, 2 * D, d.offWrz[l]);
        add(nullptr, nullptr, 0, 1, 3 * D, 0, 3 * D, d.offBh[l]);
    }
    return tiles;
}

static StepKernels choose_kernels(const DevModel& d, int n_cu, const KernelSwitches& sw, bool defer_on) {
    StepKernels k = {};
    const int L = d.n_layers, B = d.B, top = L - 1;
    const bool onehot = d.embed_mode == G4R_EMBED_ONEHOT;
    auto deep = [&](int forced, int D) { return forced >= 0 ? forced != 0 : (D >= 384 && cdiv(D, GT_BN) * cdiv(B, GT_BM) <= n_cu); };
    int dmax = 0;
    for (int l = 0; l < L; ++l) dmax = std::max(dmax, d.D[l]);
    const bool automask = sw.wide2 < 0;
    const int mask = automask ? (1 | 8 | (6 * dmax >= d.R ? 16 : 0)) : sw.wide2;
    k.wide_dense = (mask & 16) && wide_layer(dmax) && !onehot;
    for (int l = 0; l < L; ++l) {
        const int D = d.D[l], IN = d.IN[l];
        const bool onehot0 = l == 0 && onehot;
        const bool lean = !sw.no_lean && D <= LN_MAXD && IN <= LN_MAXD && D % 4 == 0 && IN % 4 == 0 && IN >= 4 && !onehot0;
        const bool ffwd = D <= FF_LDR && IN <= FF_LDR && D % 4 == 0 && IN % 4 == 0 && IN >= 4 && !onehot0 &&
                          (size_t)fwd_fused_lds(IN, D).total * sizeof(float) <= 156 * 1024;
        const bool fbwd = D <= BF_MAXD && D % 4 == 0 && IN % 4 == 0 && !onehot0;
        WideGeo& G = k.wg[l];
        G = WideGeo();
        if (wide_layer(D) && D % 64 == 0 && IN % 16 == 0 && IN >= 64 && !onehot0) {
            if ((mask & 1) && (!automask || D >= 512)) {
                const int ks = std::min(128, std::max(16, sw.p1_ks / 16 * 16));
                G.ny = cdiv(IN, ks); G.kys = ((cdiv(IN, G.ny) + 15) / 16) * 16; G.ny = cdiv(IN, G.kys);
                G.nh = cdiv(D, ks); G.khs = ((cdiv(D, G.nh) + 15) / 16) * 16; G.nh = cdiv(D, G.khs);
                if (G.ny <= 8 && G.ny + G.nh <= 16) G.use |= 1;
            }
            const bool consumer = l == 0 || k.bwd[l - 1] != BWD_FUSED;
            if ((mask & 8) && consumer) {
                const int K = 3 * D, tiles = cdiv(IN, 64) * cdiv(B, 64);
                const int n = std::min(std::max(1, cdiv(n_cu, std::max(tiles, 1))), std::max(1, K / 128));
                int ks = ((cdiv(K, n) + 31) / 32) * 32;
                if (sw.bb_ks > 0) ks = std::max(32, sw.bb_ks / 32 * 32);
                if (cdiv(K, ks) <= 16) { G.use |= 8; G.bbk = ks; G.bbn = cdiv(K, ks); }
            }
        }
        k.fwd[l] = lean ? FWD_LEAN : ffwd ? FWD_FUSED : (G.use & 1) ? FWD_P1S : wide_layer(D) ? FWD_P1_N64 : FWD_P1_N32;
        k.bwd[l] = lean ? BWD_LEAN : fbwd ? BWD_FUSED : onehot0 ? BWD_ONEHOT : (G.use & 8) ? BWD_BW : BWD_B;
        k.p2_deep[l] = deep(sw.p2_geo, D);
        k.ba_deep[l] = deep(sw.ba_geo, D);
    }
    const int Dt = d.Dtop;
    const bool wide = (B >= 256 && d.ldSc >= 4096) || (Dt % 64 == 0 && B >= 192 && d.ldSc >= 2048);
    const bool dma = Dt % 32 == 0 && (wide || (Dt >= 256 && B >= 64 && d.ldSc >= 1024));
    bool mt = false;
    if (!sw.no_mt && dma && Dt % 32 == 0 && Dt >= 32 && n_cu / cdiv(B, 64) >= 1) {
        const int nrb = cdiv(B, 64), W = 16 * cdiv(d.ldSc, 16 * (n_cu / nrb));
        mt = W == 272 && nrb * cdiv(d.ldSc, W) * 8 >= n_cu * 7;
    }
    const bool lean_s = !sw.no_lean && Dt <= LN_MAXD && Dt % 4 == 0 && !wide && !dma && B < 65536 && d.ldSc < 65536;
    k.score_fwd = lean_s ? SF_LEAN : mt ? SF_MT : dma ? SF_T3 : (wide && Dt % T2_BK == 0) ? SF_T2 : wide ? SF_K64 : SF_K128;
    k.loss_spec = (d.final_act == G4R_ACT_ELU && d.loss == G4R_LOSS_BPR_MAX) ? 1 : (d.final_act == G4R_ACT_SOFTMAX && d.loss == G4R_LOSS_XE) ? 2
                : (d.final_act == G4R_ACT_ELU && d.loss == G4R_LOSS_TOP1_MAX) ? 3 : 0;
    k.loss_long = (size_t)(2 * d.ldSc + 18 * LOSS_NW) * sizeof(float) > (size_t)(156 * 1024);
    k.loss_quads = d.ldSc >= 4 * LOSS_T;
    const bool bwd2 = wide && Dt % 64 == 0;
    const bool top_tiles = k.bwd[top] != BWD_LEAN && k.bwd[top] != BWD_FUSED;
    if (!sw.no_bmt && bwd2 && top_tiles && Dt % 128 == 0 && Dt <= 512 && d.ldSc % BMT_WA == 0 && d.ldSc <= 0xFFFF && B <= 0xFFFF) {
        const int ntA = d.ldSc / BMT_WA * (Dt / 32), den = cdiv(B, 64) * (Dt / 128), ks = ntA / den;
        if (ntA % den == 0 && ntA % 8 == 0 && ntA <= n_cu && ntA * 8 >= n_cu * 7 && BMT_WA % (Dt / 32) == 0 && 4 * (BMT_WA / (Dt / 32)) <= 256 &&
            ks >= 2 && ks <= 24 && d.ldSc % ks == 0 && (d.ldSc / ks) % 32 == 0 && d.ldSc / ks <= 2048)
            k.bmt_slabs = ks;
    }
    k.score_bwd = (lean_s && B <= 128) ? SB_LEAN : k.bmt_slabs ? SB_BMT : bwd2 ? SB_BWD2 : wide ? SB_W : SB_N;
    k.score_a_host = (sw.score_b_split && k.score_bwd == SB_LEAN && k.bwd[top] == BWD_LEAN) ? 1 : 0;
    const int slabs_target = top_tiles ? 17 : 9;
    k.kch = GT_BK * std::max(1, (cdiv(d.ldSc, GT_BK) + slabs_target / 2) / slabs_target);
    if (k.score_bwd == SB_LEAN) k.kch = 128;
    else if (k.score_bwd == SB_BMT) k.kch = d.ldSc / k.bmt_slabs;
    else if (k.score_bwd == SB_BWD2) {
        const int ndt = Dt / 64, nrt = cdiv(B, 64), nA = cdiv(d.ldSc, 64) * ndt;
        double best = 2.0;
        for (int ks = 12; ks <= 24; ++ks) {
            const int kch = (cdiv(d.ldSc, ks) + 7) & ~7;
            if (cdiv(d.ldSc, kch) != ks) continue;
            const double rounds = (double)(nA + ks * nrt * ndt) / n_cu;
            const double waste = (std::ceil(rounds) - rounds) / std::ceil(rounds) + 1e-3 * std::abs(ks - 17);
            if (waste < best) { best = waste; k.kch = kch; }
        }
    }
    k.ksplit = cdiv(d.ldSc, k.kch);
    const int TB = wide ? 64 : 32;
    k.ndtA = cdiv(Dt + 1, TB); k.nblkA = cdiv(d.ldSc, TB) * k.ndtA;
    k.ndtB = cdiv(Dt, TB); k.nrtB = cdiv(B, TB); k.nblkB = k.ksplit * k.nrtB * k.ndtB;
    const int w = std::max(Dt, d.Ein);
    k.chunks = w <= 256 ? 1 : (w <= 512 ? 2 : 4);
    const bool dy0_parts = (k.wg[0].use & 8) != 0;
    const bool merged = !d.generic && !sw.no_merge && k.chunks <= 2 && !k.wide_dense;
    const bool lean_u = !sw.no_lean && sw.allow_lean_update && merged && d.apply_dense_inplace && B <= 128 && k.chunks == 1 && !defer_on && d.xmode == 0 &&
                        !d.touched && !dy0_parts && d.R < 65536 && cdiv(d.R, 8) < 65536 && dense_tiles(d, 16, 64).size() < 65536;
    k.update = lean_u ? UP_LEAN : merged ? UP_MERGED : UP_SPLIT;
    k.finish_rows = dy0_parts && !k.wide_dense;
    return k;
}
static int sync_dm(g4r_model* m) {
    HIPCHK(hipMemcpyAsync(m->d_dm, &m->dm, sizeof(DevModel), hipMemcpyHostToDevice, m->stream));
    HIPCHK(hipStreamSynchronize(m->stream));
    return 0;
}
```

gru4rec_amd/csrc/g4r_host_step.hpp:

```cpp
static void launch_loss_rows(g4r_model* m, dim3 grid, bool timed, hipEvent_t ev_a, hipEvent_t ev_b) {
    const StepKernels& k = m->kern;
    const DevModel* dmp = (const DevModel*)m->d_dm;
    StepState* stp = (StepState*)m->dm.st;
#define G4R_LK_LOSS1(kern)                                                                                            \
    do {                                                                                                              \
        if (timed) hipExtLaunchKernelGGL(kern, grid, dim3(LOSS_T), m->smem_loss, m->stream, ev_a, ev_b, 0, dmp, stp); \
        else hipLaunchKernelGGL(kern, grid, dim3(LOSS_T), m->smem_loss, m->stream, dmp, stp);                         \
    } while (0)
#define G4R_LK_LOSS(L, V)                                                      \
    do {                                                                       \
        if (k.loss_spec == 1) G4R_LK_LOSS1((k_loss_rows<L, 1, V>));            \
        else if (k.loss_spec == 2) G4R_LK_LOSS1((k_loss_rows<L, 2, V>));       \
        else if (k.loss_spec == 3) G4R_LK_LOSS1((k_loss_rows<L, 3, V>));       \
        else G4R_LK_LOSS1((k_loss_rows<L, 0, V>));                             \
    } while (0)
    if (k.loss_long) G4R_LK_LOSS(true, 4);
    else { if (k.loss_quads) G4R_LK_LOSS(false, 4); else G4R_LK_LOSS(false, 1); }
#undef G4R_LK_LOSS
#undef G4R_LK_LOSS1
}

static int launch_step(g4r_model* m, std::vector<EvRec>* recs, int part = 0) {
    DevModel& d = m->dm;
    const StepKernels& k = m->kern;
    const int L = d.n_layers, B = d.B;
    hipStream_t s = m->stream;
    GruFwdPredict nopa = {};
    size_t evi = 0;
    hipEvent_t cur_a = nullptr, cur_b = nullptr;
    static const bool trace = getenv("G4R_TRACE") != nullptr;
    int trace_kn = -1;
    auto begin = [&](int kn) {
        trace_kn = kn;
        if (trace) { fprintf(stderr, "[g4r] launch %s\n", KN_NAMES[kn]); fflush(stderr); }
        if (!recs) return;
        while (m->evs.size() < evi + 2) { hipEvent_t e; (void)hipEventCreate(&e); m->evs.push_back(e); }
        EvRec r = {kn, m->evs[evi], m->evs[evi + 1]};
        evi += 2;
        cur_a = r.a; cur_b = r.b;
        recs->push_back(r);
    };
    auto end = [&]() {
        if (trace) {
            hipError_t e = hipStreamSynchronize(s);
            fprintf(stderr, "[g4r] done   %s: %s\n", KN_NAMES[trace_kn], hipGetErrorString(e));
            fflush(stderr);
        }
    };
#define LK(kern, grid, block, smem, strm, ...)                                                             \
    do {                                                                                                  \
        if (m->sw.skip_kn && trace_kn >= 0 && ((m->sw.skip_kn >> trace_kn) & 1ull)) break;                \
        if (recs) hipExtLaunchKernelGGL(kern, grid, block, smem, strm, cur_a, cur_b, 0, __VA_ARGS__);     \
        else hipLaunchKernelGGL(kern, grid, block, smem, strm, __VA_ARGS__);                              \
    } while (0)
    const DevModel* dmp = (const DevModel*)m->d_dm;
    StepState* stp = (StepState*)d.st;
    const bool merged = k.update != UP_SPLIT && !(recs && m->profile_split);
    const bool a_hosted = k.score_a_host && !recs;
    if (part != 2) {
    for (int l = 0; l < L; ++l) {
        if (k.fwd[l] == FWD_LEAN) {
            const int ntd = cdiv(d.D[l], 16), nrb = cdiv(B, 16);
            begin(KN_GRU_V);
            {
                const LeanV& v = m->h_leanV[l];
                const unsigned dims = (unsigned)d.D[l] | ((unsigned)d.IN[l] << 16);
#define G4R_LK_V(L0_, DR_) LK((k_gru_v<L0_, DR_>), dim3(ntd, nrb, 3), dim3(512), 0, s, (const LeanV*)(m->d_leanV + l), (StepState*)v.st, (const int*)v.cur_in, \
                              (const float*)v.Wx, (const float*)v.Wrz, (const float*)v.H0, (const float*)v.H1, dims, (unsigned)B)
                if (l > 0) G4R_LK_V(false, false); else if (d.drop_e > 0.f) G4R_LK_V(true, true); else G4R_LK_V(true, false);
#undef G4R_LK_V
            }
            end();
            begin(KN_GRU_H);
            {
                const LeanH& h = m->h_leanH[l];
                LK(k_gru_h, dim3(ntd, nrb), dim3(512), 0, s, (const LeanH*)(m->d_leanH + l), (const float*)h.Wh, (const float*)h.Hr,
                   (const float*)h.Vc, (const float*)h.z, (const int*)h.cur_rst, (const float*)h.H0, (const float*)h.H1, (unsigned)d.D[l], (unsigned)B);
            }
            end();
            continue;
        }
        if (k.fwd[l] == FWD_FUSED) {
            begin(KN_FWD_FUSED);
            LK(k_gru_fwd_fused, dim3(cdiv(d.D[l], 32), cdiv(B, FF_ROWS)), dim3(512), (size_t)fwd_fused_lds(d.IN[l], d.D[l]).total * sizeof(float), s, dmp, stp, l, l == 0 ? 1 : 0);
            end();
            continue;
        }
        const WideGeo& G = k.wg[l];
        const int nrt64 = cdiv(B, 64), nct64 = d.D[l] / 64;
        begin(KN_GRU_P1);
        if (k.fwd[l] == FWD_P1S) {
            LK(k_gru_p1s, dim3(nct64 * nrt64 * (3 * G.ny + 2 * G.nh)), dim3(256), SMEM_T2K, s, dmp, stp, l, l == 0 ? 1 : 0, G.ny, G.nh, G.kys, G.khs);
            end();
            begin(KN_GATE);
            LK(k_gru_gate, dim3(cdiv((long long)B * (d.D[l] / 4), 256)), dim3(256), 0, s, dmp, stp, l, G.ny, G.nh);
        } else if (k.fwd[l] == FWD_P1_N64) LK(k_gru_p1_n64, dim3(cdiv(3 * d.D[l], 64), cdiv(B, GT_BM)), dim3(GT_NTH_FEW), SMEM_P1_N64, s, dmp, stp, l, 1, l == 0 ? 1 : 0, nopa);
        else LK(k_gru_p1_n32, dim3(cdiv(3 * d.D[l], GT_BN), cdiv(B, GT_BM)), dim3(GT_NTH_FEW), SMEM_P1, s, dmp, stp, l, 1, l == 0 ? 1 : 0, nopa);
        end();
        begin(KN_GRU_P2);
        {
            const dim3 g2(cdiv(d.D[l], GT_BN), cdiv(B, GT_BM));
            if (k.p2_deep[l]) LK(k_gru_p2_w8d, g2, dim3(512), SMEM_P2_256, s, dmp, stp, l, 1, nopa);
            else LK(k_gru_p2_w4, g2, dim3(GT_NTH), SMEM_NN, s, dmp, stp, l, 1, nopa);
        }
        end();
    }
    begin(KN_SCORE_FWD);
    switch (k.score_fwd) {
    case SF_LEAN: {
        const unsigned dimsA = (unsigned)d.Dtop | ((unsigned)B << 16), dimsB = (unsigned)d.N | ((unsigned)d.ldSc << 16);
        const dim3 gs(cdiv(d.ldSc, 32), cdiv(B, 32));
        if (d.logq != 0.f) LK(k_score_s<true>, gs, dim3(256), 0, s, (const LeanS*)m->d_leanS, (const int*)(d.cur_in + 2 * B), (const int*)d.cur_col, (const float*)d.hd[L - 1],
                              (const float*)d.Wy, (const float*)d.By, (float*)d.Sc, dimsA, dimsB);
        else LK(k_score_s<false>, gs, dim3(256), 0, s, (const LeanS*)m->d_leanS, (const int*)(d.cur_in + 2 * B), (const int*)d.cur_col, (const float*)d.hd[L - 1],
                (const float*)d.Wy, (const float*)d.By, (float*)d.Sc, dimsA, dimsB);
        break;
    }
    case SF_MT: LK(k_score_mt_4s, dim3(cdiv(B, 64) * cdiv(d.ldSc, 272)), dim3(256), SMEM_MT_4S, s, (const int*)d.cur_col, (const int*)(d.cur_in + 2 * B),
                   (const float*)d.hd[L - 1], (const float*)d.Wy, (const float*)d.zrow, dmp, (unsigned)d.Dtop | ((unsigned)cdiv(B, 64) << 16),
                   (unsigned)d.N, (unsigned)d.ldSc, (unsigned)B); break;
    case SF_T3: LK(k_score_fwd_t3, dim3(cdiv(d.ldSc, 64), cdiv(B, 64)), dim3(GT_NTH), SMEM_SF3, s, dmp, stp); break;
    case SF_T2: LK(k_score_fwd_t2, dim3(cdiv(d.ldSc, 64), cdiv(B, 64)), dim3(GT_NTH), SMEM_SF2, s, dmp, stp); break;
    case SF_K64: LK(k_score_fwd_k64, dim3(cdiv(d.ldSc, SFW_BN), cdiv(B, SF_BM)), dim3(GT_NTH), SMEM_SF64, s, dmp, stp); break;
    default: LK(k_score_fwd_k128, dim3(cdiv(d.ldSc, GT_BN), cdiv(B, SF_BM)), dim3(GT_NTH), SMEM_SF, s, dmp, stp); break;
    }
    end();
    begin(KN_LOSS);
    {
        const int nown = std::min(cdiv(d.R, LOSS_NW), std::max(2 * m->n_cu - B, 32));
        const dim3 gloss(B + (merged && k.update == UP_LEAN && d.own_pos ? nown : 0));
        if (!(m->sw.skip_kn && ((m->sw.skip_kn >> KN_LOSS) & 1ull))) launch_loss_rows(m, gloss, recs != nullptr, cur_a, cur_b);
    }
    end();
    begin(KN_SCORE_BWD);
    switch (k.score_bwd) {
    case SB_LEAN: {
        const LeanB& q = m->h_leanB;
#define G4R_LK_SB(RA, NWG) LK(k_score_b<RA>, dim3(NWG), dim3(512), 0, s, (const LeanB*)m->d_leanB, (const int*)(d.cur_in + 2 * B), (const int*)d.cur_col,   \
           (const float*)d.Sc, (const float*)d.hd[L - 1], (const float*)d.Wy, (float*)d.accWy, (unsigned)d.Dtop | ((unsigned)B << 16), (unsigned)d.N | ((unsigned)d.ldSc << 16))
        if (a_hosted) G4R_LK_SB(false, d.ksplit * q.nrb * q.ndb);
        else G4R_LK_SB(true, q.nA + d.ksplit * q.nrb * q.ndb);
#undef G4R_LK_SB
        break;
    }
    case SB_BMT: {
        const int ntile = d.ldSc / BMT_WA * (d.Dtop / 32);
        LK(k_score_bmt, dim3(2 * ntile), dim3(256), SMEM_BMT, s, (const float*)d.Sc, (const float*)d.hd[L - 1], (const float*)d.Wy, (const int*)d.col_item,
           (const int*)(d.cur_in + 2 * B), (const float*)d.zrow, dmp, (unsigned)d.Dtop | ((unsigned)(d.Dtop / 32) << 16), (unsigned)d.N | ((unsigned)d.ldSc << 16),
           (unsigned)B | ((unsigned)d.kch << 16), (unsigned)cdiv(B, 64) | ((unsigned)(d.Dtop / 128) << 16));
        break;
    }
    case SB_BWD2: {
        const int ndt = d.Dtop / 64, nrt = cdiv(B, 64);
        int nA = cdiv(d.ldSc, 64) * ndt, nB = d.ksplit * nrt * ndt, nC = cdiv(d.ldSc, 64);
        LK(k_score_bwd2, dim3(nA + nB + nC), dim3(GT_NTH), (size_t)(4 * 64 * 16) * sizeof(float) + (size_t)std::max(d.kch, 64) * sizeof(int), s, dmp, stp, nA, nB, ndt, nrt);
        break;
    }
    case SB_W: LK(k_score_bwd_w, dim3(k.nblkA + k.nblkB), dim3(GT_NTH), SMEM_SBW + (size_t)d.kch * sizeof(int), s, dmp, stp, k.nblkA, k.ndtA, k.ndtB, k.nrtB); break;
    default: LK(k_score_bwd_n, dim3(k.nblkA + k.nblkB), dim3(GT_NTH), std::max(SMEM_TN, SMEM_NN) + (size_t)d.kch * sizeof(int), s, dmp, stp, k.nblkA, k.ndtA, k.ndtB, k.nrtB); break;
    }
    end();
    for (int l = L - 1; l >= 0; --l) {
        if (k.bwd[l] == BWD_LEAN) {
            const int nrb = cdiv(B, 16);
            begin(KN_GRU_DA);
            {
                const LeanDa& q = m->h_leanDa[l];
                LK(k_gru_da, dim3(cdiv(d.D[l], 16), nrb), dim3(128), 0, s, (const LeanDa*)(m->d_leanDa + l), (const int*)(d.cur_in + 2 * B), (const float*)q.dsrc,
                   (const float*)q.Wh, (const float*)q.z, (const float*)q.c, (const float*)q.H0, (const float*)q.H1, (unsigned)d.D[l] | ((unsigned)q.ks << 16), (unsigned)B);
            }
            end();
            begin(KN_GRU_DY);
            {
                const LeanDy& y = m->h_leanDy[l];
                if (a_hosted && l == L - 1) {
                    const LeanB& q = m->h_leanB;
                    const int gx = cdiv(d.IN[l], 16);
                    LK(k_gru_dy_a, dim3(gx, nrb + cdiv(cdiv(q.nA, 2), gx)), dim3(1024), 0, s, (const LeanDy*)(m->d_leanDy + l), (const int*)(d.cur_in + 2 * B),
                       (const int*)y.occ_idx, (const float*)y.dV, (const float*)y.drp, (const float*)y.Wx, (const float*)y.r, (unsigned)d.D[l] | ((unsigned)d.IN[l] << 16),
                       (unsigned)B, (const LeanB*)m->d_leanB, (const int*)d.cur_col, (const float*)d.Sc, (const float*)d.hd[L - 1], (float*)d.accWy,
                       (unsigned)d.Dtop | ((unsigned)B << 16), (unsigned)d.N | ((unsigned)d.ldSc << 16), (unsigned)q.nA | ((unsigned)q.ndh << 16));
                } else
                LK(k_gru_dy, dim3(cdiv(d.IN[l], 16), nrb), dim3(1024), 0, s, (const LeanDy*)(m->d_leanDy + l), (const int*)(d.cur_in + 2 * B), (const int*)y.occ_idx,
                   (const float*)y.dV, (const float*)y.drp, (const float*)y.Wx, (const float*)y.r, (unsigned)d.D[l] | ((unsigned)d.IN[l] << 16), (unsigned)B);
            }
            end();
            continue;
        }
        if (k.bwd[l] == BWD_FUSED) {
            begin(KN_BWD_FUSED);
            LK(k_gru_bwd_fused, dim3(cdiv(d.IN[l], 32), cdiv(B, BF_ROWS)), dim3(512), smem_bwd_fused(d.D[l]), s, dmp, stp, l);
            end();
            continue;
        }
        begin(KN_BWD_PRE);
        LK(k_gru_bwd_pre, dim3(cdiv((long long)B * d.D[l], 256)), dim3(256), 0, s, dmp, stp, l);
        end();
        const WideGeo& G = k.wg[l];
        const int nrt64 = cdiv(B, 64);
        begin(KN_BWD_A);
        {
            dim3 ga(cdiv(d.D[l], GT_BN), cdiv(B, GT_BM));
            int nfin = 0;
            if (l == L - 1 && k.score_bwd == SB_BMT) { nfin = cdiv(cdiv(d.N, 16), (int)ga.x); ga.y += nfin; }
            if (k.ba_deep[l]) LK(k_gru_bwd_a_w8d, ga, dim3(512), SMEM_BA_256, s, dmp, stp, l, nfin);
            else LK(k_gru_bwd_a_w4, ga, dim3(GT_NTH), SMEM_NT, s, dmp, stp, l, nfin);
        }
        end();
        begin(KN_BWD_B);
        if (k.bwd[l] == BWD_ONEHOT) LK(k_onehot_step, dim3(cdiv((long long)B * d.Ein, 4 * 256)), dim3(256), 0, s, dmp, stp);
        else if (k.bwd[l] == BWD_BW) LK(k_gru_bwd_bw, dim3(cdiv(d.IN[l], 64) * nrt64 * G.bbn), dim3(256), SMEM_T3, s, dmp, stp, l, G.bbn, G.bbk);
        else LK(k_gru_bwd_b, dim3(cdiv(d.IN[l], GT_BN), cdiv(B, GT_BM)), dim3(GT_NTH_FEW), SMEM_BB, s, dmp, stp, l);
        end();
    }
    if (merged) {
        if (k.finish_rows) {
            begin(KN_FINISH);
            LK(k_finish_rows, dim3(cdiv((long long)B * (d.IN[0] / 4), 256)), dim3(256), 0, s, dmp, stp);
            end();
        }
        begin(KN_UPDATE);
        const bool mo = d.mom > 0.f;
        if (k.update == UP_LEAN) {
            const int nb8 = cdiv(d.R, 8);
            const unsigned packA = (unsigned)m->ntiles16 | ((unsigned)nb8 << 16), packB = (unsigned)d.R | ((unsigned)B << 16);
            const unsigned nbk = 1u + (unsigned)cdiv(d.ldSc, 512);
            const dim3 gl(nbk + m->ntiles16 + nb8);
            if (mo) LK(k_update_l<true>, gl, dim3(512), 0, s, (const LeanU*)m->d_leanU, (const DenseTile*)m->d_tiles16, (const int*)d.occ_idx, (int*)d.occ_fl,
                       (const float*)d.dSx, (const float*)d.dSy, (const float*)d.dSBy, packA, packB, nbk);
            else LK(k_update_l<false>, gl, dim3(512), 0, s, (const LeanU*)m->d_leanU, (const DenseTile*)m->d_tiles16, (const int*)d.occ_idx, (int*)d.occ_fl,
                    (const float*)d.dSx, (const float*)d.dSy, (const float*)d.dSBy, packA, packB, nbk);
            end();
            HIPCHK(hipGetLastError());
            return 0;
        }
        const size_t smem = std::max(SMEM_TN, m->smem_sparse);
        const dim3 grid(m->ntiles + m->nblk_occ + 1), blk(SP_WAVES * 64);
#define G4R_LK_UPDATE(CH, DT_)                                                                                                          \
        do {                                                                                                                            \
            if (mo) LK((k_update<CH, DT_, true>), grid, blk, smem, s, dmp, stp, (const DenseTile*)m->d_tiles, m->ntiles, m->nblk_occ);  \
            else LK((k_update<CH, DT_, false>), grid, blk, smem, s, dmp, stp, (const DenseTile*)m->d_tiles, m->ntiles, m->nblk_occ);    \
        } while (0)
        if (k.chunks == 1) G4R_LK_UPDATE(1, 32); else G4R_LK_UPDATE(2, 32);
#undef G4R_LK_UPDATE
        end();
        if (d.apply_dense_inplace || part == 1) { HIPCHK(hipGetLastError()); return 0; }
    } else {
    begin(KN_DENSE);
    if (k.wide_dense) LK(k_dense_grad2, dim3(m->ntiles64 + (d.bbn[0] > 0 ? cdiv((long long)B * (d.IN[0] / 4), 256) : 0)), dim3(256), SMEM_T2K, s, dmp, stp, (const DenseTile*)m->d_tiles64, m->ntiles64);
    else {
        if (k.finish_rows) LK(k_finish_rows, dim3(cdiv((long long)B * (d.IN[0] / 4), 256)), dim3(256), 0, s, dmp, stp);
        LK(k_dense_grad<32>, dim3(m->ntiles), dim3(GT_NTH_FEW), SMEM_TN, s, dmp, stp, (const DenseTile*)m->d_tiles);
    }
    end();
    }
    }
    if (part == 1) { HIPCHK(hipGetLastError()); return 0; }
    if (!d.apply_dense_inplace) {
        const bool dist = !m->virtual_ranks && (m->cfg.nranks > 1 || m->comm_ready || m->p2p_ready);
        if (m->cfg.nranks > 1 && !m->comm_ready && !m->p2p_ready && !m->virtual_ranks) return fail("nranks > 1 but g4r_comm_init was not called");
        if (dist && !m->exact) {
            begin(KN_ALLREDUCE);
            if (recs) (void)hipEventRecord(cur_a, s);
            if (m->p2p_ready) hipLaunchKernelGGL(k_p2p_allreduce, dim3(m->p2p_nblk), dim3(256), 0, s, m->p2p_args, (float*)d.dense_g);
            else NCCLCHK(ncclAllReduce(d.dense_g, d.dense_g, d.dense_count, ncclFloat, ncclSum, m->comm, s));
            if (recs) (void)hipEventRecord(cur_b, s);
            end();
        }
        if (d.generic && d.grad_cap > 0.f) {
            hipLaunchKernelGGL(k_grad_sqsum, dim3(G4R_NORM_BLOCKS), dim3(256), 0, s, dmp, stp);
            hipLaunchKernelGGL(k_grad_clip, dim3(1), dim3(64), 0, s, dmp);
        }
        if (!d.generic) {
            begin(KN_DENSE_APPLY);
            LK(k_dense_apply, dim3(cdiv(d.dense_count, 256)), dim3(256), 0, s, (const DevModel*)m->d_dm);
            end();
        }
    }
    if (d.generic) {
        int nblk_g = m->nblk_occ_g;
        size_t smem_g = m->smem_sparse;
        if (m->exact) {
            if (!m->virtual_ranks) {
                if (!m->comm_ready) return fail("sparse_exact needs the RCCL communicator (g4r_comm_init)");
                NCCLCHK(ncclAllGather((const float*)d.xbase + (size_t)m->cfg.rank * (size_t)d.xstride, (float*)d.xbase, (size_t)d.xstride, ncclFloat, m->comm, s));
            }
            const long long rlist = d.xmode == 3 ? (long long)d.xn * 2 * B + d.ns : (long long)d.R * d.xn;
            hipLaunchKernelGGL(k_exact_occ, dim3(cdiv(rlist, 256)), dim3(256), 0, s, dmp);
            nblk_g = cdiv(rlist, SP_WAVES);
            smem_g = m->smem_exact;
        }
        begin(KN_SPARSE);
        const int nda = d.apply_dense_inplace ? 0 : cdiv(d.dense_count, SP_WAVES * 64);
        if (k.chunks == 1) LK(k_sparse_update_generic<1>, dim3(nblk_g + 1 + nda), dim3(SP_WAVES * 64), smem_g, s, dmp, stp, nblk_g, nda);
        else if (k.chunks == 2) LK(k_sparse_update_generic<2>, dim3(nblk_g + 1 + nda), dim3(SP_WAVES * 64), smem_g, s, dmp, stp, nblk_g, nda);
        else LK(k_sparse_update_generic<4>, dim3(nblk_g + 1 + nda), dim3(SP_WAVES * 64), smem_g, s, dmp, stp, nblk_g, nda);
        end();
        HIPCHK(hipGetLastError());
        return 0;
    }
    if (merged) { HIPCHK(hipGetLastError()); return 0; }
    begin(KN_SPARSE);
    {
        const bool mo = d.mom > 0.f;
        const dim3 grid(m->nblk_occ + 1), blk(SP_WAVES * 64);
#define G4R_LK_SPARSE(CH)                                                                                            \
        do {                                                                                                         \
            if (mo) LK((k_sparse_update<CH, true>), grid, blk, m->smem_sparse, s, dmp, stp, m->nblk_occ);            \
            else LK((k_sparse_update<CH, false>), grid, blk, m->smem_sparse, s, dmp, stp, m->nblk_occ);              \
        } while (0)
        if (k.chunks == 1) G4R_LK_SPARSE(1); else if (k.chunks == 2) G4R_LK_SPARSE(2); else G4R_LK_SPARSE(4);
#undef G4R_LK_SPARSE
    }
    end();
#undef LK
    HIPCHK(hipGetLastError());
    return 0;
}

static int apply_compaction(g4r_model* m, int64_t ci) {
    DevModel& d = m->dm;
    const int B = d.B;
    for (int l = 0; l < d.n_layers; ++l) {
        float* Hc = d.H[l][m->gstep & 1];
        const int W = d.D[l];
        hipLaunchKernelGGL(k_gather_rows, dim3(cdiv((long long)B * W, 256)), dim3(256), 0, m->stream, m->d_tmpH, (const float*)Hc,
                           (const int*)(m->d_cmaps + ci * B), B, W);
        HIPCHK(hipMemcpyAsync(Hc, m->d_tmpH, (size_t)B * W * sizeof(float), hipMemcpyDeviceToDevice, m->stream));
    }
    return 0;
}

#define G4R_GRAPH_STEPS 16
#define G4R_GRAPH_STEPS_SMALL 4
static inline bool local_staged(const g4r_model* m) {
    return !m->dm.apply_dense_inplace && m->cfg.nranks <= 1 && !m->comm_ready && !m->p2p_ready && !m->virtual_ranks;
}
static inline bool dist_graph_wanted(const g4r_model* m) {
    return !m->dm.apply_dense_inplace && !m->dist_graph_failed &&
           (m->p2p_ready || m->comm_ready || local_staged(m));
}
static int ensure_graph(g4r_model* m) {
    if (m->gexec) return 0;
    const bool dist = !m->dm.apply_dense_inplace && !local_staged(m);
    const bool rccl_in_graph = dist && (!m->p2p_ready || (m->exact && m->comm_ready));
    if (dist) {
        if (!m->p2p_ready) NCCLCHK(ncclAllReduce(m->dm.dense_g, m->dm.dense_g, m->dm.dense_count, ncclFloat, ncclSum, m->comm, m->stream));
        if (m->exact && m->comm_ready)
            NCCLCHK(ncclAllGather((const float*)m->dm.xbase + (size_t)m->cfg.rank * (size_t)m->dm.xstride, (float*)m->dm.xbase, (size_t)m->dm.xstride,
                                  ncclFloat, m->comm, m->stream));
        HIPCHK(hipStreamSynchronize(m->stream));
    }
    hipGraph_t graph = nullptr;
    HIPCHK(hipStreamBeginCapture(m->stream, rccl_in_graph ? hipStreamCaptureModeRelaxed : hipStreamCaptureModeThreadLocal));
    int rc = 0;
    for (int i = 0; i < G4R_GRAPH_STEPS && !rc; ++i) rc = launch_step(m, nullptr);
    hipError_t e = hipStreamEndCapture(m->stream, &graph);
    if (rc || e != hipSuccess || !graph) {
        if (graph) (void)hipGraphDestroy(graph);
        (void)hipGetLastError();
        if (!rc) fail(std::string("graph capture: ") + hipGetErrorString(e));
        return -1;
    }
    e = hipGraphInstantiate(&m->gexec, graph, nullptr, nullptr, 0);
    (void)hipGraphDestroy(graph);
    if (e != hipSuccess) { m->gexec = nullptr; (void)hipGetLastError(); return fail(std::string("graph instantiate: ") + hipGetErrorString(e)); }
    m->graph_steps = G4R_GRAPH_STEPS;
    if (!dist) {
        hipGraph_t g2 = nullptr;
        if (hipStreamBeginCapture(m->stream, hipStreamCaptureModeThreadLocal) == hipSuccess) {
            int rc2 = 0;
            for (int i = 0; i < G4R_GRAPH_STEPS_SMALL && !rc2; ++i) rc2 = launch_step(m, nullptr);
            hipError_t e2 = hipStreamEndCapture(m->stream, &g2);
            if (!rc2 && e2 == hipSuccess && g2 && hipGraphInstantiate(&m->gexec_small, g2, nullptr, nullptr, 0) != hipSuccess) m->gexec_small = nullptr;
            if (g2) (void)hipGraphDestroy(g2);
            (void)hipGetLastError();
        }
    }
    return 0;
}
static int ensure_head_graph(g4r_model* m);
static int ensure_step_graph(g4r_model* m, bool* whole) {
    if (m->dm.apply_dense_inplace) { *whole = true; return ensure_graph(m); }
    if (dist_graph_wanted(m)) {
        if (ensure_graph(m) == 0) { *whole = true; return 0; }
        m->dist_graph_failed = true;
        fprintf(stderr, "[g4r] RCCL all-reduce could not be captured into the step graph (%s); launching it eagerly\n", g_err.c_str());
    }
    *whole = false;
    return ensure_head_graph(m);
}

static int ensure_head_graph(g4r_model* m) {
    if (m->gexec_head) return 0;
    hipGraph_t graph;
    HIPCHK(hipStreamBeginCapture(m->stream, hipStreamCaptureModeThreadLocal));
    if (launch_step(m, nullptr, 1)) { hipGraph_t g2; (void)hipStreamEndCapture(m->stream, &g2); return -1; }
    HIPCHK(hipStreamEndCapture(m->stream, &graph));
    HIPCHK(hipGraphInstantiate(&m->gexec_head, graph, nullptr, nullptr, 0));
    (void)hipGraphDestroy(graph);
    return 0;
}

int g4r_train_steps(g4r_model* m, int64_t t0, int64_t n_steps) {
    if (!m) return fail("null model");
    if (!m->d_in) return fail("no plan uploaded");
    if (t0 < 0 || n_steps < 0 || t0 + n_steps > m->T) return fail("step range outside the plan");
    if (m->dm.ns > 0 && !m->have_pop && !m->store_frozen) return fail("negative sampling needs g4r_set_popularity first");
    weights_changed(m);
    if (m->defer_on) {
        if (m->gstep + n_steps >= ((int64_t)1 << 31) - 64) return fail("deferred row updates: the global step would pass 2^31 -- rebase it with g4r_set_step_counters (epoch boundary) or create the model without defer_updates");
        if (m->defer_broken) return fail("deferred row updates: an earlier call failed between a window's scan and its flush launch; the row updates pending then are lost -- recreate the model");
    }
    struct WindowGuard { g4r_model* m; bool open = false; ~WindowGuard() { if (open) m->defer_broken = true; } } wguard{m};
    HIPCHK(hipSetDevice(m->cfg.device));
    hipLaunchKernelGGL(k_set_state, dim3(1), dim3(512), 0, m->stream, (const DevModel*)m->d_dm, (StepState*)m->dm.st, (long long)t0, (long long)m->gstep);
    bool use_graph = m->cfg.use_graph && !m->profiling && !getenv("G4R_TRACE") && (m->dm.apply_dense_inplace || dist_graph_wanted(m));
    if (use_graph && !m->dm.apply_dense_inplace) {
        bool whole = false;
        if (ensure_step_graph(m, &whole)) return -1;
        use_graph = whole;
    }
    size_t ci = std::lower_bound(m->compact_steps.begin(), m->compact_steps.end(), t0) - m->compact_steps.begin();
    int64_t t = t0;
    const int64_t tend = t0 + n_steps;
    std::vector<EvRec> recs;
    while (t < tend) {
        while (ci < m->compact_steps.size() && m->compact_steps[ci] == t) { if (apply_compaction(m, (int64_t)ci)) return -1; ++ci; }
        if (m->dm.ns > 0 && !m->store_frozen && m->gstep > 0 && m->gstep % m->gl == 0)
        {
            if (refill_store(m)) return -1;
            hipLaunchKernelGGL(k_restage_inputs, dim3(1), dim3(512), 0, m->stream, (const DevModel*)m->d_dm, (StepState*)m->dm.st);
        }
        const bool devsync = m->sync_every_dev > 0 && m->comm_ready;
        if (devsync && m->since_sync >= m->sync_every_dev) {
            if (sync_dense_enqueue(m)) return -1;
            ++m->n_dev_syncs;
        }
        int64_t run = tend - t;
        if (devsync) run = std::min<int64_t>(run, m->sync_every_dev - m->since_sync);
        if (ci < m->compact_steps.size()) run = std::min(run, m->compact_steps[ci] - t);
        if (m->dm.ns > 0 && !m->store_frozen) run = std::min<int64_t>(run, m->gl - (m->gstep % m->gl));
        if (run <= 0) return fail("internal: empty run");
        int64_t done = 0;
        auto window_open = [&](int64_t nw) {
            if (!m->defer_on) return;
            wguard.open = true;
            const dim3 gs(cdiv(nw * m->dm.R, 256));
            if (m->profiling) (void)hipEventRecord(m->ev_df[0], m->stream);
            hipLaunchKernelGGL(k_defer_scan, gs, dim3(256), 0, m->stream, (const DevModel*)m->d_dm, (long long)(t + done), (long long)(m->gstep + done), (int)nw, 0);
            hipLaunchKernelGGL(k_defer_scan, gs, dim3(256), 0, m->stream, (const DevModel*)m->d_dm, (long long)(t + done), (long long)(m->gstep + done), (int)nw, 1);
            if (m->profiling) (void)hipEventRecord(m->ev_df[1], m->stream);
        };
        auto window_close = [&](int64_t nw, int64_t first) -> int {
            if (!m->defer_on) return 0;
            if (m->profiling) (void)hipEventRecord(m->ev_df[2], m->stream);
            hipLaunchKernelGGL(k_sparse_flush, dim3(cdiv(nw * m->dm.dRcap, SP_WAVES * FL_NR)), dim3(SP_WAVES * 64), 0, m->stream, (const DevModel*)m->d_dm, (long long)(m->gstep + first), (int)nw);
            if (m->profiling) {
                (void)hipEventRecord(m->ev_df[3], m->stream);
                HIPCHK(hipStreamSynchronize(m->stream));
                float ms = 0.f;
                if (hipEventElapsedTime(&ms, m->ev_df[0], m->ev_df[1]) == hipSuccess) { m->kn_ms[KN_SCAN] += ms; m->kn_n[KN_SCAN]++; }
                if (hipEventElapsedTime(&ms, m->ev_df[2], m->ev_df[3]) == hipSuccess) { m->kn_ms[KN_FLUSH] += ms; m->kn_n[KN_FLUSH]++; }
            }
            wguard.open = false;
            return 0;
        };
        if (use_graph && run >= G4R_GRAPH_STEPS_SMALL) {
            if (ensure_graph(m)) return -1;
            for (; done + m->graph_steps <= run; done += m->graph_steps) {
                window_open(m->graph_steps);
                HIPCHK(hipGraphLaunch(m->gexec, m->stream));
                if (window_close(m->graph_steps, done)) return -1;
            }
            if (m->gexec_small)
                for (; done + G4R_GRAPH_STEPS_SMALL <= run; done += G4R_GRAPH_STEPS_SMALL) {
                    window_open(G4R_GRAPH_STEPS_SMALL);
                    HIPCHK(hipGraphLaunch(m->gexec_small, m->stream));
                    if (window_close(G4R_GRAPH_STEPS_SMALL, done)) return -1;
                }
        }
        int64_t win_first = -1, win_n = 0;
        for (; done < run; ++done) {
            if (m->defer_on && win_n == 0) {
                win_n = std::min<int64_t>(G4R_DEFER_SLOTS, run - done); win_first = done;
                window_open(win_n);
            }
            if (m->profiling) {
                recs.clear();
                if (launch_step(m, &recs)) return -1;
                HIPCHK(hipStreamSynchronize(m->stream));
                for (auto& r : recs) {
                    float ms = 0.f;
                    if (hipEventElapsedTime(&ms, r.a, r.b) == hipSuccess) { m->kn_ms[r.kn] += ms; m->kn_n[r.kn]++; }
                }
            } else if (m->cfg.use_graph && !m->dm.apply_dense_inplace && !getenv("G4R_TRACE")) {
                if (ensure_head_graph(m)) return -1;
                HIPCHK(hipGraphLaunch(m->gexec_head, m->stream));
                if (launch_step(m, nullptr, 2)) return -1;
            } else if (launch_step(m, nullptr)) return -1;
            if (win_n > 0 && done + 1 == win_first + win_n) {
                if (window_close(win_n, win_first)) return -1;
                win_n = 0;
            }
        }
        t += run;
        m->gstep += run;
        m->since_sync += run;
    }
    HIPCHK(hipStreamSynchronize(m->stream));
    if (m->p2p_ready) {
        unsigned late = 0;
        HIPCHK(hipMemcpy(&late, m->p2p_round + m->p2p_nblk, sizeof(late), hipMemcpyDeviceToHost));
        if (late) return fail("p2p all-reduce: a peer did not publish its gradients within G4R_P2P_TIMEOUT_MS (dead rank?)");
    }
    return 0;
}

int g4r_virtual_train_steps(g4r_model* const* ms, int32_t n, int64_t t0, int64_t n_steps) {
    if (!ms || n < 1 || n > 16) return fail("virtual ranks: 1..16 handles");
    for (int q = 0; q < n; ++q) {
        g4r_model* m = ms[q];
        if (!m || !m->d_in) return fail("virtual ranks: null model / no plan uploaded");
        if (m->cfg.nranks != n || m->cfg.rank != q) return fail("virtual ranks: handle q must be created with rank = q, nranks = n");
        if (m->cfg.device != ms[0]->cfg.device || m->dm.dense_count != ms[0]->dm.dense_count || m->exact != ms[0]->exact || m->dm.xstride != ms[0]->dm.xstride)
            return fail("virtual ranks: handles differ");
        if (m->comm_ready || m->p2p_ready) return fail("virtual ranks: the handle already has a communicator / peer mappings");
        if (t0 < 0 || n_steps < 0 || t0 + n_steps > m->T) return fail("step range outside the plan");
        if (m->dm.ns > 0 && !m->have_pop && !m->store_frozen) return fail("negative sampling needs g4r_set_popularity first");
        m->virtual_ranks = true;
    }
    for (int q = 0; q < n; ++q) weights_changed(ms[q]);
    HIPCHK(hipSetDevice(ms[0]->cfg.device));
    g4r_model* m0 = ms[0];
    const int cnt = m0->dm.dense_count;
    if (!m0->d_vsum && dalloc(m0, &m0->d_vsum, (size_t)cnt)) return -1;
    VSumArgs va;
    memset(&va, 0, sizeof(va));
    std::vector<size_t> ci(n);
    for (int q = 0; q < n; ++q) {
        g4r_model* m = ms[q];
        va.src[q] = m->dm.dense_g; va.dst[q] = m->dm.dense_g;
        hipLaunchKernelGGL(k_set_state, dim3(1), dim3(512), 0, m->stream, (const DevModel*)m->d_dm, (StepState*)m->dm.st, (long long)t0, (long long)m->gstep);
        ci[q] = std::lower_bound(m->compact_steps.begin(), m->compact_steps.end(), t0) - m->compact_steps.begin();
    }
    for (int64_t t = t0; t < t0 + n_steps; ++t) {
        for (int q = 0; q < n; ++q) {
            g4r_model* m = ms[q];
            while (ci[q] < m->compact_steps.size() && m->compact_steps[ci[q]] == t) { if (apply_compaction(m, (int64_t)ci[q])) return -1; ++ci[q]; }
            if (m->dm.ns > 0 && !m->store_frozen && m->gstep > 0 && m->gstep % m->gl == 0) {
                if (refill_store(m)) return -1;
                hipLaunchKernelGGL(k_restage_inputs, dim3(1), dim3(512), 0, m->stream, (const DevModel*)m->d_dm, (StepState*)m->dm.st);
            }
            if (launch_step(m, nullptr, 1)) return -1;
        }
        for (int q = 0; q < n; ++q) HIPCHK(hipStreamSynchronize(ms[q]->stream));
        if (m0->exact) {
            for (int q = 0; q < n; ++q)
                for (int p = 0; p < n; ++p)
                    if (p != q) HIPCHK(hipMemcpyAsync((float*)ms[q]->dm.xbase + (size_t)p * (size_t)m0->dm.xstride,
                                                      (const float*)ms[p]->dm.xbase + (size_t)p * (size_t)m0->dm.xstride,
                                                      (size_t)m0->dm.xstride * sizeof(float), hipMemcpyDeviceToDevice, ms[q]->stream));
            for (int q = 0; q < n; ++q) HIPCHK(hipStreamSynchronize(ms[q]->stream));
        }
        if (!m0->exact) {
            hipLaunchKernelGGL(k_virtual_sum, dim3(cdiv(cnt, 256)), dim3(256), 0, m0->stream, va, n, cnt, m0->d_vsum);
            hipLaunchKernelGGL(k_virtual_bcast, dim3(cdiv(cnt, 256)), dim3(256), 0, m0->stream, va, n, cnt, (const float*)m0->d_vsum);
            HIPCHK(hipStreamSynchronize(m0->stream));
        }
        for (int q = 0; q < n; ++q) {
            if (launch_step(ms[q], nullptr, 2)) return -1;
            ms[q]->gstep += 1;
        }
    }
    for (int q = 0; q < n; ++q) HIPCHK(hipStreamSynchronize(ms[q]->stream));
    return 0;
}

int g4r_get_losses(g4r_model* m, int64_t t0, int64_t n, float* out) {
    if (!m || !out) return fail("null argument");
    if (t0 < 0 || n < 0 || t0 + n > m->T) return fail("range outside the plan");
    HIPCHK(hipSetDevice(m->cfg.device));
    HIPCHK(hipStreamSynchronize(m->stream));
    HIPCHK(hipMemcpy(out, m->d_loss + t0, n * sizeof(float), hipMemcpyDeviceToHost));
    return 0;
}
int g4r_synchronize(g4r_model* m) {
    if (!m) return fail("null model");
    HIPCHK(hipSetDevice(m->cfg.device));
    HIPCHK(hipStreamSynchronize(m->stream));
    return 0;
}
int64_t g4r_global_step(g4r_model* m) { return m ? m->gstep : -1; }
int64_t g4r_refills(g4r_model* m) { return m ? (int64_t)m->refills : -1; }
int g4r_set_step_counters(g4r_model* m, int64_t global_step, int64_t refills) {
    if (!m) return fail("null model");
    if (global_step < 0 || refills < 0) return fail("negative counter");
    HIPCHK(hipSetDevice(m->cfg.device));
    m->gstep = global_step;
    if (m->defer_on)
        HIPCHK(hipMemsetAsync(m->dm.last_use, 0, (size_t)(m->cfg.embed_mode != G4R_EMBED_CONSTRAINED ? 2 : 1) * m->dm.n_items * sizeof(int), m->stream));
    if (m->dm.ns > 0 && !m->store_frozen) {
        if (!m->have_pop) return fail("g4r_set_popularity first");
        if (refills < 1) return fail("a model with negative sampling has filled its store at least once");
        m->refills = (unsigned)(refills - 1);
        if (refill_store(m)) return -1;
        HIPCHK(hipStreamSynchronize(m->stream));
    } else {
        m->refills = (unsigned)refills;
    }
    return 0;
}
int g4r_profile(g4r_model* m, int32_t enable) {
    if (!m) return fail("null model");
    m->profiling = enable != 0;
    m->profile_split = enable == 2;
    if (enable) for (int i = 0; i < KN_COUNT; ++i) { m->kn_ms[i] = 0; m->kn_n[i] = 0; }
    return 0;
}
int g4r_kernel_time(g4r_model* m, int32_t which, const char** name, double* total_ms, int64_t* launches) {
    if (!m || which < 0 || which >= KN_COUNT) return fail("bad kernel index");
    if (name) *name = KN_NAMES[which];
    if (total_ms) *total_ms = m->kn_ms[which];
    if (launches) *launches = m->kn_n[which];
    return 0;
}

int g4r_reset_hidden(g4r_model* m) {
    if (!m) return fail("null model");
    HIPCHK(hipSetDevice(m->cfg.device));
    for (int l = 0; l < m->dm.n_layers; ++l)
        for (int q = 0; q < 2; ++q)
            HIPCHK(hipMemsetAsync(m->dm.H[l][q], 0, (size_t)m->dm.B * m->dm.D[l] * sizeof(float), m->stream));
    HIPCHK(hipStreamSynchronize(m->stream));
    return 0;
}
```

gru4rec_amd/csrc/g4r_lean_kernels.cuh:

```cuda
#pragma once

#define LN_MAXD 128

__device__ __forceinline__ float ldu(const GAS float* base, unsigned boff) { return *(const GAS float*)((const GAS char*)base + boff); }
__device__ __forceinline__ int ldu_i(const GAS int* base, unsigned boff) { return *(const GAS int*)((const GAS char*)base + boff); }
__device__ __forceinline__ float4 ldu4(const GAS float* base, unsigned boff) { return *(const GAS float4*)((const GAS char*)base + boff); }
__device__ __forceinline__ void stu(GAS float* base, unsigned boff, float v) { *(GAS float*)((GAS char*)base + boff) = v; }
__device__ __forceinline__ void stu4(GAS float* base, unsigned boff, float4 v) { *(GAS float4*)((GAS char*)base + boff) = v; }

#if defined(G4R_CLK_TRACE)
#define LCLK_INIT(dbgp, slot) GAS long long* clk_ = ((dbgp) && blockIdx.x == 1 && blockIdx.y == 1 && blockIdx.z == 0 && threadIdx.x == 0) ? (dbgp) + (slot) : nullptr
#define LCLK(i) do { if (clk_) clk_[i] = wall_clock64(); } while (0)
#define LCLK_USE(x) do { if (clk_ && (x) == 123.456f) clk_[15] = 0; } while (0)
#define LSPAN_BEGIN(tilep, base) GAS long long* span_ = ((tilep) && threadIdx.x == 0) ? (tilep) + 8 * (size_t)((base) + (blockIdx.z * gridDim.y + blockIdx.y) * gridDim.x + blockIdx.x) : nullptr; \
    if (span_) span_[0] = wall_clock64()
#define LSPAN_END() do { if (span_) span_[1] = wall_clock64(); } while (0)
#define LSPAN_BEGIN_AT(tilep, idx, lead) GAS long long* span_ = ((tilep) && (lead)) ? (tilep) + 8 * (size_t)(idx) : nullptr; \
    if (span_) span_[0] = wall_clock64()
#else
#define LCLK_INIT(dbgp, slot)
#define LCLK(i)
#define LCLK_USE(x)
#define LSPAN_BEGIN(tilep, base)
#define LSPAN_END()
// ... 883 lines not shown
                        }
                    }
                }
            }
        }
    }
    const float fn = (float)n;
    const float p0[4] = {pz.x, pz.y, pz.z, pz.w}, v0[4] = {vz.x, vz.y, vz.z, vz.w}, sl[4] = {sk.x, sk.y, sk.z, sk.w};
    const float ss[4] = {S.x + sk.x, S.y + sk.y, S.z + sk.z, S.w + sk.w};
    float pn[4], vn[4];
#pragma unroll
    for (int e = 0; e < 4; ++e) {
        const float reg = (lmbd > 0.f) ? lr * lmbd * p0[e] : 0.f;
        const float tot = (lmbd > 0.f) ? ss[e] + fn * reg : ss[e];
        if (MOM) { vn[e] = momc * v0[e] - (sl[e] + reg); pn[e] = p0[e] + (fn * (momc * v0[e]) - tot); }
        else { vn[e] = 0.f; pn[e] = p0[e] - tot; }
    }
    float bn = 0.f, bvn = 0.f;
    if (bias) {
        const float fb = (float)(nb_e + 1);
        const float reg = (lmbd > 0.f) ? lr * lmbd * bpz : 0.f;
        const float sb = Sb + bsk;
        const float tot = (lmbd > 0.f) ? sb + fb * reg : sb;
        if (MOM) { bn = bpz + (fb * (momc * bvz) - tot); bvn = momc * bvz - (bsk + reg); }
        else bn = bpz - tot;
    }
    lean_keep(bn); lean_keep(bvn); lean_keep(bak);
    const size_t o = (size_t)item * W + 4 * c4;
    if (lok) {
        st4(P + o, make_float4(pn[0], pn[1], pn[2], pn[3]));
        if (MOM) st4(V + o, make_float4(vn[0], vn[1], vn[2], vn[3]));
        if (n > 1) st4(A + o, ak);
    }
    if (bias && lane == 0) {
        a.By[item] = bn;
        if (MOM) a.velBy[item] = bvn;
        if (n > 1) a.accBy[item] = bak;
    }
}

template <bool MOM>
__device__ __forceinline__ void lean_dense_tile(const LeanU& a, const DenseTile* tiles_, unsigned tile, unsigned B) {
    __shared__ f32x4 sJ[4 * 8 * 64];
    const unsigned tid = threadIdx.x, lane = tid & 63, li = lane & 15, lg = lane >> 4;
    const unsigned wid = __builtin_amdgcn_readfirstlane(tid >> 6);
    const GAS DenseTile* tiles = (const GAS DenseTile*)tiles_;
    const DenseTile tl = tiles[tile];
    const GAS StepState* sg = (const GAS StepState*)a.st;
    const long long g_ = sg->g_b;
    const int M = sg->M_b;
    const unsigned row = tl.r0 + li, rowc = min(row, (unsigned)tl.nrows - 1);
    const unsigned cq = tl.c0 + 4 * li, cqc = min(cq, (unsigned)tl.ncols - 4);
    const bool ones = tl.X0 == nullptr && !tl.gather;
    const GAS float* Xa = tl.gather ? a.yin0 : (ones ? tl.dV : tl.X0);
    const GAS float* Xb = tl.gather ? a.yin0 : (ones ? tl.dV : tl.X1);
    float4 av[4];
    float x0[4], x1[4];
#pragma unroll
    for (int s_ = 0; s_ < 4; ++s_) {
        const unsigned b = min(16 * wid + 4 * s_ + lg, B - 1);
        av[s_] = ldu4(tl.dV, 4 * (b * (unsigned)tl.ldv + (unsigned)tl.coff + cqc));
        const unsigned ox = ones ? 0u : 4 * (b * (unsigned)tl.ldx + rowc);
        x0[s_] = ldu(Xa, ox); x1[s_] = ldu(Xb, ox);
    }
    const unsigned ce = tl.c0 + 16 * lg + 4 * (wid & 3), cec = min(ce, (unsigned)tl.ncols - 4);
    const size_t off = (size_t)tl.base + (size_t)rowc * tl.ldo + cec;
    const float4 acc4 = ld4(a.dense_acc + off), p4 = ld4(a.dense_p + off);
    float4 v4 = make_float4(0.f, 0.f, 0.f, 0.f);
    if (MOM) v4 = ld4(a.dense_vel + off);
    __builtin_amdgcn_sched_barrier(0);
    const bool odd = (g_ & 1) != 0;
    f32x4 acc[4];
#pragma unroll
    for (int c = 0; c < 4; ++c) acc[c] = (f32x4){0.f, 0.f, 0.f, 0.f};
#pragma unroll
    for (int s_ = 0; s_ < 4; ++s_) {
        const unsigned b = 16 * wid + 4 * s_ + lg;
        const bool bok = (int)b < M;
        float xv = ones ? 1.f : (odd ? x1[s_] : x0[s_]);
        if (!(bok && row < (unsigned)tl.nrows)) xv = 0.f;
        const float4 d4 = (cq < (unsigned)tl.ncols) ? av[s_] : make_float4(0.f, 0.f, 0.f, 0.f);
        acc[0] = mfma16(d4.x, xv, acc[0]);
        acc[1] = mfma16(d4.y, xv, acc[1]);
        acc[2] = mfma16(d4.z, xv, acc[2]);
        acc[3] = mfma16(d4.w, xv, acc[3]);
    }
#pragma unroll
    for (int rg = 0; rg < 4; ++rg) sJ[(rg * 8 + wid) * 64 + lane] = (f32x4){acc[0][rg], acc[1][rg], acc[2][rg], acc[3][rg]};
    __syncthreads();
    if (wid >= 4) return;
    f32x4 g4 = sJ[(wid * 8 + 0) * 64 + lane];
#pragma unroll
    for (int w = 1; w < 8; ++w) g4 += sJ[(wid * 8 + w) * 64 + lane];
    if (row >= (unsigned)tl.nrows || ce >= (unsigned)tl.ncols) return;
    const float gg[4] = {g4[0], g4[1], g4[2], g4[3]}, a0[4] = {acc4.x, acc4.y, acc4.z, acc4.w}, pp[4] = {p4.x, p4.y, p4.z, p4.w}, vv[4] = {v4.x, v4.y, v4.z, v4.w};
    float an[4], pn[4], vn[4];
    const float lr = a.lr, momc = a.mom, lmbd = a.lmbd;
#pragma unroll
    for (int c = 0; c < 4; ++c) {
        an[c] = a0[c] + G4R_MUT_DACC(gg[c] * gg[c]);
        const float gs = gg[c] * frsq(an[c] + G4R_EPS_ADAGRAD);
        if (MOM) { vn[c] = momc * vv[c] - lr * (gs + lmbd * pp[c]); pn[c] = pp[c] + vn[c]; }
        else { vn[c] = 0.f; pn[c] = pp[c] * (1.0f - lr * lmbd) - lr * gs; }
    }
    st4(a.dense_acc + off, make_float4(an[0], an[1], an[2], an[3]));
    st4(a.dense_p + off, make_float4(pn[0], pn[1], pn[2], pn[3]));
    if (MOM) st4(a.dense_vel + off, make_float4(vn[0], vn[1], vn[2], vn[3]));
}

__device__ __forceinline__ void lean_bookkeep(const LeanU& a, unsigned part, unsigned B) {
    const DevModel& m = *a.mp;
    const unsigned tid = threadIdx.x;
    const GAS StepState* sg = (const GAS StepState*)a.st;
    const long long t = sg->t_b, g = sg->g_b;
    const int M = sg->M_b;
    const GAS int *in_idx = m.in_idx, *out_idx = m.out_idx, *Mplan = m.Mplan, *ST = m.ST;
    const GAS unsigned char* reset = m.reset;
    const int gl = m.gl, ns = m.ns, N = m.N, ld = m.ldSc;
    GAS int *ci = m.cur_in, *cc = m.cur_col;
    GAS float* loss_steps = m.loss_steps;
    const GAS float* lossrow = m.lossrow;
    const float inv_B = m.inv_B;
    lean_pin(in_idx, out_idx, Mplan, ST, reset, gl, ns, N, ld, ci, cc, loss_steps, lossrow, inv_B);
    const long long t1 = t + 1, g1 = g + 1;
    const int Mn = Mplan[t1];
    if (part == 0) {
        if (tid < 64) {
            float s_ = 0.f;
            for (int i = (int)tid; i < M; i += 64) s_ += lossrow[i];
            s_ = wave_sum(s_);
            if (tid == 0) {
                const float cost = s_ * inv_B;
                loss_steps[t] = cost;
                GAS StepState* sw = (GAS StepState*)a.st;
                if (isnan(cost)) sw->nan_flag = 1;
                sw->t_a = t1; sw->g_a = g1; sw->M_a = Mn;
                ci[2 * B] = (int)(unsigned)g1; ci[2 * B + 1] = (int)(g1 >> 32); ci[2 * B + 2] = Mn; ci[2 * B + 3] = (int)(unsigned)t1; ci[2 * B + 4] = (int)(t1 >> 32);
            }
        } else if (tid - 64 < B) {
            const unsigned b = tid - 64;
            ci[b] = in_idx[t1 * B + b];
            ci[B + b] = reset[t1 * B + b];
        }
        return;
    }
    const int n = 512 * (int)(part - 1) + (int)tid;
    const int vo = out_idx[t1 * B + min(n, (int)B - 1)];
    const int vs = (ns > 0) ? ST[(size_t)(gl > 0 ? g1 % gl : 0) * ns + min(max(n - (int)B, 0), ns - 1)] : -1;
    if (n < ld) cc[n] = (n < Mn) ? vo : (n >= (int)B && n < N && Mn > 0) ? vs : -1;
}

template <bool MOM>
__global__ __launch_bounds__(512) void k_update_l(const LeanU* __restrict__ ap, const DenseTile* __restrict__ tiles_, const int* occ_idx_, int* occ_fl_,
                                                  const float* dSx_, const float* dSy_, const float* dSBy_, unsigned packA, unsigned packB, unsigned nbk) {
    const unsigned ntiles = packA & 0xFFFFu, nblk = packA >> 16, R = packB & 0xFFFFu, B = packB >> 16;
    const LeanU a = *ap;
    LSPAN_BEGIN(a.dbgtile, 2700);
    if (blockIdx.x < nbk) { lean_bookkeep(a, blockIdx.x, B); LSPAN_END(); return; }
    const unsigned b = blockIdx.x - nbk;
    if (b < ntiles) { lean_dense_tile<MOM>(a, tiles_, b, B); LSPAN_END(); return; }
    const unsigned q = b - ntiles, wid = __builtin_amdgcn_readfirstlane(threadIdx.x >> 6);
    lean_rows_update<MOM>(a, (const GAS int*)occ_idx_, (GAS int*)occ_fl_, (const GAS float*)dSx_, (const GAS float*)dSy_, (const GAS float*)dSBy_,
                          (const GAS int*)(tiles_ + ntiles), wid * nblk + q, R, B);
    LSPAN_END();
}
template __global__ void k_update_l<false>(const LeanU*, const DenseTile*, const int*, int*, const float*, const float*, const float*, unsigned, unsigned, unsigned);
template __global__ void k_update_l<true>(const LeanU*, const DenseTile*, const int*, int*, const float*, const float*, const float*, unsigned, unsigned, unsigned);
```

gru4rec_amd/csrc/g4r_loss_kernel.cuh:

```cuda
#pragma once
#ifndef LOSS_T
#define LOSS_T 1024
#endif
#define LOSS_NW (LOSS_T / 64)
template <int NV, bool MAX>
__device__ __forceinline__ void block_reduce(float (&v)[NV], float* red) {
    const int lane = threadIdx.x & 63, w = threadIdx.x >> 6;
#pragma unroll
    for (int q = 0; q < NV; ++q) v[q] = MAX ? wave_max(v[q]) : wave_sum(v[q]);
    if (lane == 0) {
#pragma unroll
        for (int q = 0; q < NV; ++q) red[q * LOSS_NW + w] = v[q];
    }
    __syncthreads();
#pragma unroll
    for (int q = 0; q < NV; ++q) {
        float a = red[q * LOSS_NW];
#pragma unroll
        for (int u = 1; u < LOSS_NW; ++u) a = MAX ? fmaxf(a, red[q * LOSS_NW + u]) : a + red[q * LOSS_NW + u];
        v[q] = a;
    }
}

__device__ __forceinline__ float softplusf_(float x) {
    return fmaxf(x, 0.f) + log1pf(fexp(-fabsf(x)));
}

template <int V, class Ptr>
__device__ __forceinline__ void vld(float (&o)[V], Ptr p) {
    if constexpr (V == 4) { const float4 t = ld4(p); o[0] = t.x; o[1] = t.y; o[2] = t.z; o[3] = t.w; }
    else o[0] = p[0];
}
template <int V, class Ptr>
__device__ __forceinline__ void vst(Ptr p, const float (&o)[V]) {
    if constexpr (V == 4) st4(p, make_float4(o[0], o[1], o[2], o[3]));
    else p[0] = o[0];
}

__device__ __forceinline__ void owner_prescan(const DevModel& m, unsigned k) {
    const unsigned lane = threadIdx.x & 63;
    const unsigned R = (unsigned)m.R, B = (unsigned)m.B;
    const GAS int* occ_idx = m.occ_idx;
    int item = occ_idx[min(k, R - 1)];
    if (k >= R) item = -1;
    if (item < 0) return;
    const bool constrained = m.embed_mode == G4R_EMBED_CONSTRAINED;
    const bool tableE = k < B && !constrained;
    const int4 fl = ldi4(m.occ_fl + 4 * ((tableE ? (size_t)m.n_items : 0) + (unsigned)item));
    if (fl.x != (int)k + 1 || fl.z < 2) return;
    const int lo = (constrained || k < B) ? 0 : (int)B;
    const int first_j = max(lo, (int)R - fl.y);
    if (first_j >= 2 * (int)B) return;
    GAS int* pos = m.own_pos + 16 * (size_t)k;
    if (fl.z - 1 > G4R_OWN_INLINE) {
        if (lane == 0) pos[0] = -1;
        return;
    }
    const unsigned long long below = (1ull << lane) - 1ull;
    int cnt = 0;
    for (int base0 = first_j & ~3; base0 < (int)k; base0 += 1024) {
        int4 vv[4];
#pragma unroll
        for (int u = 0; u < 4; ++u) vv[u] = ldi4(occ_idx + min(base0 + 256 * u + 4 * (int)lane, (int)((R + 3) & ~3u) - 4));
#pragma unroll
        for (int u = 0; u < 4; ++u) {
            const int j0 = base0 + 256 * u + 4 * (int)lane;
            const int ids[4] = {vv[u].x, vv[u].y, vv[u].z, vv[u].w};
            unsigned long long mk[4];
            int at = cnt;
#pragma unroll
            for (int e = 0; e < 4; ++e) {
                mk[e] = __ballot(ids[e] == item && j0 + e >= first_j && j0 + e < (int)k && !G4R_MUT_SLICE_SKIP(j0 + e, base0, first_j & ~3));
                at += __popcll(mk[e] & below);
                cnt += __popcll(mk[e]);
            }
#pragma unroll
            for (int e = 0; e < 4; ++e) {
                if ((mk[e] >> lane) & 1ull) {
                    if ((unsigned)at < (unsigned)G4R_OWN_INLINE) pos[1 + at] = j0 + e;
                    ++at;
                }
            }
        }
    }
    if (lane == 0) pos[0] = min(cnt, G4R_OWN_INLINE);
}

template <bool LONG_ROW, int SPEC, int V>
__global__ __launch_bounds__(LOSS_T) void k_loss_rows(const DevModel* __restrict__ mp, StepState* st) {
    const DevModel& m = *mp;
    extern __shared__ __attribute__((aligned(16))) float smem[];
    const int tid = threadIdx.x;
    const int B = m.B, N = m.N, i = blockIdx.x;
    const int fact = SPEC == 1 || SPEC == 3 ? (int)G4R_ACT_ELU : (SPEC == 2 ? (int)G4R_ACT_SOFTMAX : m.final_act);
    const int lossk = SPEC == 1 ? (int)G4R_LOSS_BPR_MAX : (SPEC == 2 ? (int)G4R_LOSS_XE : (SPEC == 3 ? (int)G4R_LOSS_TOP1_MAX : m.loss));
    const int ldSc = m.ldSc;
    const float fp0 = m.fa_p0, fp1 = m.fa_p1, invB = m.inv_B, bpreg = m.bpreg, smooth = m.smoothing;
    GAS float* row = m.Sc + (size_t)i * ldSc;
    float* sy = smem;
    std::conditional_t<LONG_ROW, GAS float*, float*> se;
    if constexpr (LONG_ROW) se = row; else se = smem + ldSc;
    float* red = smem + (LONG_ROW ? 1 : 2) * ldSc;
    constexpr int STEP = V * LOSS_T;
    const int jt = V * tid;
    constexpr int LOSS_PRE = (V == 4) ? 2 : 4;
#if defined(G4R_CLK_TRACE)
    struct Span { GAS long long* p; __device__ ~Span() { if (p) p[1] = wall_clock64(); } } span_{(m.dbgtile && tid == 0 && i < 1024) ? m.dbgtile + 8 * (size_t)(7168 + i) : nullptr};
    if (span_.p) span_.p[0] = wall_clock64();
#endif
    const StepCtx c = load_ctx(st);
    if (i >= B) {
        const unsigned nown = gridDim.x - B, R = m.R;
        for (unsigned k = (threadIdx.x >> 6) * nown + (unsigned)(i - B); k < R; k += LOSS_NW * nown) owner_prescan(m, k);
        return;
    }
    float pre_s[LOSS_PRE][V];
#pragma unroll
    for (int q = 0; q < LOSS_PRE; ++q) vld<V>(pre_s[q], row + min(jt + q * STEP, ldSc - V));
    const int M = c.M;
    if (i >= M) return;
    const bool fsm = (fact == G4R_ACT_SOFTMAX), fsl = (fact == G4R_ACT_SOFTMAX_LOGIT);
    const float n_out = (float)(M + (N - B));
    auto active = [&](int j) { return j < N && (j < M || j >= B); };
    auto grp_fast = [&](int j0) { return (j0 >= B && j0 + V <= N) || (j0 + V <= G4R_MUT_FAST_M(M) && (i < j0 || i >= j0 + V)); };
    using Fast = std::true_type;
    using Slow = std::false_type;
#define G4R_GROUPS(lim, fn) for (int j0 = jt; j0 < (lim); j0 += STEP) { if (grp_fast(j0)) fn(Fast{}, j0); else fn(Slow{}, j0); }
    float mneg[1] = {0.f};
    if (fsm || fsl) {
        float mx[1] = {-INFINITY};
        auto first = [&](auto F, int j0, const float (&v)[V]) {
            float o[V];
#pragma unroll
            for (int e = 0; e < V; ++e) {
                const bool a = F.value || active(j0 + e);
                o[e] = a ? v[e] : 0.f;
                mx[0] = a ? fmaxf(mx[0], v[e]) : mx[0];
            }
            vst<V>(sy + j0, o);
        };
#pragma unroll
        for (int q = 0; q < LOSS_PRE; ++q) {
            const int j0 = jt + q * STEP;
            if (j0 < N) { if (grp_fast(j0)) first(Fast{}, j0, pre_s[q]); else first(Slow{}, j0, pre_s[q]); }
        }
        for (int j0 = jt + LOSS_PRE * STEP + G4R_MUT_FIRST_LATE(STEP); j0 < N; j0 += STEP) {
            float v[V];
            vld<V>(v, row + j0);
            if (grp_fast(j0)) first(Fast{}, j0, v); else first(Slow{}, j0, v);
        }
        block_reduce<1, true>(mx, red);
        float sm[1] = {0.f};
        auto numer = [&](auto F, int j0) {
            float y[V];
            vld<V>(y, sy + j0);
#pragma unroll
            for (int e = 0; e < V; ++e) {
                const bool a = F.value || active(j0 + e);
                const float ex = fexp(a ? y[e] - mx[0] : 0.f);
                if (fsm) y[e] = ex;
                sm[0] += a ? ex : 0.f;
            }
            if (fsm) vst<V>(sy + j0, y);
        };
        G4R_GROUPS(N, numer)
        block_reduce<1, false>(sm, red + 3 * LOSS_NW);
        const float inv_z = 1.f / sm[0], lse = logf(sm[0]);
        auto norm = [&](auto F, int j0) {
            float y[V];
            vld<V>(y, sy + j0);
#pragma unroll
            for (int e = 0; e < V; ++e) {
                const int j = j0 + e;
                const float yy = fsm ? y[e] * inv_z : lse - (y[e] - mx[0]);
                y[e] = yy;
                mneg[0] = (F.value || (active(j) && j != i)) ? fmaxf(mneg[0], yy) : mneg[0];
            }
            vst<V>(sy + j0, y);
        };
        G4R_GROUPS(N, norm)
    } else {
        auto first = [&](auto F, int j0, const float (&v)[V]) {
            float o[V];
#pragma unroll
            for (int e = 0; e < V; ++e) {
                const int j = j0 + e;
                const bool a = F.value || active(j);
                const float y = act_fwd_sel(fact, fp0, fp1, a ? v[e] : 0.f);
                o[e] = y;
                mneg[0] = (F.value || (a && j != i)) ? fmaxf(mneg[0], y) : mneg[0];
            }
            vst<V>(sy + j0, o);
        };
#pragma unroll
        for (int q = 0; q < LOSS_PRE; ++q) {
            const int j0 = jt + q * STEP;
            if (j0 < N) { if (grp_fast(j0)) first(Fast{}, j0, pre_s[q]); else first(Slow{}, j0, pre_s[q]); }
        }
        for (int j0 = jt + LOSS_PRE * STEP + G4R_MUT_FIRST_LATE(STEP); j0 < N; j0 += STEP) {
            float v[V];
            vld<V>(v, row + j0);
            if (grp_fast(j0)) first(Fast{}, j0, v); else first(Slow{}, j0, v);
        }
    }
    block_reduce<1, true>(mneg, red + 6 * LOSS_NW);
    const float yd = sy[i];
    const bool own_i = tid == ((i / V) % LOSS_T);
    float Lrow = 0.f;
    if (lossk == G4R_LOSS_XE && fsm && smooth == 0.f) {
        Lrow = -logf(yd + G4R_EPS_LOSS);
        const float coef = yd / (yd + G4R_EPS_LOSS);
        auto grad = [&](auto F, int j0) {
            float y[V], o[V];
            vld<V>(y, sy + j0);
#pragma unroll
            for (int e = 0; e < V; ++e) {
                const int j = j0 + e;
                if (F.value) o[e] = coef * y[e] * invB;
                else o[e] = active(j) ? coef * (y[e] - (j == i ? 1.f : 0.f)) * invB : 0.f;
            }
            vst<V>(row + j0, o);
        };
        G4R_GROUPS(ldSc, grad)
        if (tid == 0) m.lossrow[i] = Lrow;
        return;
    }
    if (lossk == G4R_LOSS_XE || lossk == G4R_LOSS_XE_LOGIT) {
        const bool lg = (lossk == G4R_LOSS_XE_LOGIT);
        const float wd = 1.f - n_out / (n_out - 1.f) * smooth, wa = smooth / (n_out - 1.f);
        float sa[1] = {0.f};
        for (int j0 = jt; j0 < N; j0 += STEP) {
            float y[V], d[V];
            vld<V>(y, sy + j0);
#pragma unroll
            for (int e = 0; e < V; ++e) {
                const int j = j0 + e;
                const bool a = active(j);
                const float yy = a ? y[e] : 1.f;
                float dd = 0.f;
                if (smooth != 0.f) { sa[0] += a ? (lg ? yy : -logf(yy + G4R_EPS_LOSS)) : 0.f; dd = lg ? wa : -wa / (yy + G4R_EPS_LOSS); }
                if (j == i) dd += lg ? wd : -wd / (yy + G4R_EPS_LOSS);
                d[e] = dd;
            }
            vst<V>(se + j0, d);
        }
        if (smooth != 0.f) block_reduce<1, false>(sa, red + 9 * LOSS_NW);
        Lrow = wd * (lg ? yd : -logf(yd + G4R_EPS_LOSS)) + wa * sa[0];
    } else if (lossk == G4R_LOSS_BPR || lossk == G4R_LOSS_TOP1) {
        float s[2] = {0.f, 0.f};
        if (lossk == G4R_LOSS_BPR) {
            for (int j0 = jt; j0 < N; j0 += STEP) {
                float y[V], d[V];
                vld<V>(y, sy + j0);
#pragma unroll
                for (int e = 0; e < V; ++e) {
                    const int j = j0 + e;
                    const bool a = active(j);
                    const float yy = a ? y[e] : yd;
                    s[0] += a ? softplusf_(yy - yd) : 0.f;
                    const float dd = (a && j != i) ? sigmoidf_(yy - yd) : 0.f;
// ... 146 lines not shown
```

gru4rec_amd/csrc/g4r_update_kernels.cuh:

```cuda
#pragma once
__global__ __launch_bounds__(256) void k_onehot_step(const DevModel* __restrict__ mp, StepState* st) {
    const DevModel& m = *mp;
    const StepCtx c = load_ctx(st);
    const int W = m.Ein, nc4 = W >> 2;
    const long long q = (long long)blockIdx.x * 256 + threadIdx.x;
    const int row = (int)(q / nc4), c4 = (int)(q % nc4);
    if (row >= c.M) return;
    const int item = m.occ_idx[row];
    if (item < 0) return;
    const float lr = m.lr;
    const float4 g = ld4(m.dV[0] + (size_t)row * W + 4 * c4);
    const float4 a = ld4(m.accE + (size_t)item * W + 4 * c4);
    const int cnt = m.occ_fl[4 * ((size_t)m.n_items + item) + 2];
    const float4 an = make_float4(a.x + g.x * g.x, a.y + g.y * g.y, a.z + g.z * g.z, a.w + g.w * g.w);
    if (!m.generic && cnt == 1) st4(m.accE + (size_t)item * W + 4 * c4, an);
    else st4(m.dAx + (size_t)row * W + 4 * c4, an);
    if (m.generic) { st4(G4R_DSX(m, c.g) + (size_t)row * W + 4 * c4, g); return; }
    st4(G4R_DSX(m, c.g) + (size_t)row * W + 4 * c4, make_float4(lr * g.x * frsq(an.x + G4R_EPS_ADAGRAD), lr * g.y * frsq(an.y + G4R_EPS_ADAGRAD),
                                                         lr * g.z * frsq(an.z + G4R_EPS_ADAGRAD), lr * g.w * frsq(an.w + G4R_EPS_ADAGRAD)));
}

struct DenseTile {
    GP(const float) X0; GP(const float) X1; GP(const float) dV;
    long long base;
// ... 363 lines not shown
                for (int q = 0; q < 4; ++q) v[q] = g_occ4[min(j0 + q * SP_WAVES * 64 + tid, n4 - 1)];
#pragma unroll
                for (int q = 0; q < 4; ++q) commit4(j0 + q * SP_WAVES * 64 + tid, v[q]);
            }
        }
        __syncthreads();
        if (G4R_DBGCLK(m)) t_col = wall_clock64();
        unsigned hm = (unsigned)__ballot(lane < SP_WAVES && sHot[lane & (SP_WAVES - 1)] >= 0);
        for (int h = -1; h < SP_WAVES; h = hm ? (int)__builtin_ctz(hm) : SP_WAVES, hm &= hm - 1) {
            int it = item, a = first_j, b = k, tW = W, tnc4 = nc4;
            bool tb = bias, active = dup && !hot;
            if (h >= 0) {
                it = sHot[h];
                if (it < 0) continue;
                const int hk = h * nblk_occ + blk, hlo = sHot[SP_WAVES + h];
                const int slice = (((hk - hlo + SP_WAVES - 1) / SP_WAVES) + 63) & ~63;
                a = hlo + wid * slice; b = min(hk, a + slice);
                tW = (hk < B && !constrained) ? wE : wY; tnc4 = tW >> 2;
                tb = hk >= B; active = true;
            }
            float4 T[MAXCH];
            float Tb = 0.f;
            int n_w = 0, nb_w = 0;
            if (G4R_DBGCLK(m) && h >= 0) t_h[0] = wall_clock64();
#pragma unroll
            for (int q = 0; q < MAXCH; ++q) T[q] = make_float4(0.f, 0.f, 0.f, 0.f);
            if (active) {
                for (int pass = 0;; ++pass) {
                    if (h < 0 && fl.z == 2) {
                        if (lane == 0) myList[0] = a;
                        n_w = 1; nb_w = (a >= B) ? 1 : 0;
                    } else {
                        n_w = scan(it, a, b, pass, nb_w);
                    }
                    if (G4R_DBGCLK(m) && h >= 0 && pass == 0) t_h[1] = wall_clock64();
                    const int cnt = min(n_w - 64 * pass, 64);
                    const int myj = lane < cnt ? myList[lane] : -1;
                    const float bd = (tb && myj >= B) ? g_dSBy[max(myj - B, 0)] : 0.f;
                    for (int i0 = 0; i0 < cnt; i0 += UB) {
                        float4 g[UB][MAXCH];
                        float w[UB];
#pragma unroll
                        for (int u = 0; u < UB; ++u) {
                            w[u] = (i0 + u < cnt) ? 1.f : 0.f;
                            const int jj = __builtin_amdgcn_readlane(myj, min(i0 + u, cnt - 1) & 63);
                            const GAS float* srow = (jj < B) ? g_dSx + (size_t)jj * tW : g_dSy + (size_t)(jj - B) * tW;
#pragma unroll
                            for (int q = 0; q < MAXCH; ++q) g[u][q] = ld4(srow + 4 * min(lane + 64 * q, tnc4 - 1));
                        }
#pragma unroll
                        for (int u = 0; u < UB; ++u) {
#pragma unroll
                            for (int q = 0; q < MAXCH; ++q) {
                                T[q].x = fmaf(w[u], g[u][q].x, T[q].x); T[q].y = fmaf(w[u], g[u][q].y, T[q].y);
                                T[q].z = fmaf(w[u], g[u][q].z, T[q].z); T[q].w = fmaf(w[u], g[u][q].w, T[q].w);
                            }
                        }
                    }
                    if (tb) Tb += wave_sum(bd);
                    if (n_w <= 64 * (pass + 1)) break;
                }
            }
            if (h < 0) {
                if (active) {
#pragma unroll
                    for (int q = 0; q < MAXCH; ++q) S[q] = T[q];
                    Sb = Tb; n_e = n_w; nb_e = nb_w;
                }
                if (G4R_DBGCLK(m)) t_app = wall_clock64();
                continue;
            }
            if (G4R_DBGCLK(m)) t_h[2] = wall_clock64();
            float* part = sPart + wid * PW;
#pragma unroll
            for (int q = 0; q < MAXCH; ++q) {
                const int c4 = lane + 64 * q;
                if (c4 < tnc4) *reinterpret_cast<float4*>(part + 4 * c4) = T[q];
            }
            if (lane == 0) { part[PW - 4] = Tb; part[PW - 3] = __int_as_float(n_w); part[PW - 2] = __int_as_float(nb_w); }
            __syncthreads();
            if (G4R_DBGCLK(m)) t_h[3] = wall_clock64();
            if (wid == h) {
                for (int w = 0; w < SP_WAVES; ++w) {
#pragma unroll
                    for (int q = 0; q < MAXCH; ++q) {
                        const float4 x = *reinterpret_cast<const float4*>(sPart + w * PW + 4 * min(lane + 64 * q, nc4 - 1));
                        S[q].x += x.x; S[q].y += x.y; S[q].z += x.z; S[q].w += x.w;
                    }
                    Sb += sPart[w * PW + PW - 4];
                    n_e += __float_as_int(sPart[w * PW + PW - 3]);
                    nb_e += __float_as_int(sPart[w * PW + PW - 2]);
                }
            }
            __syncthreads();
            if (G4R_DBGCLK(m)) t_h[4] = wall_clock64();
        }
    }
    if (allsmp) {
        for (int cdup = 1; cdup < fl.z; ++cdup) {
#pragma unroll
            for (int q = 0; q < MAXCH; ++q) { S[q].x += sk[q].x; S[q].y += sk[q].y; S[q].z += sk[q].z; S[q].w += sk[q].w; }
            Sb += bsk;
        }
        n_e = fl.z - 1; nb_e = fl.z - 1;
    }
    if (owner && !single) {
        if constexpr (MAXCH == 2 && MOM) {
#pragma unroll
            for (int q = 0; q < MAXCH; ++q) vz[q] = ld4(V + (size_t)item * W + 4 * min(lane + 64 * q, nc4 - 1));
        }
        finish(S, Sb, n_e + 1, nb_e + (bias ? 1 : 0));
#pragma unroll
        for (int q = 0; q < MAXCH; ++q) {
            const int c4 = lane + 64 * q;
            if (c4 < nc4) st4(A + (size_t)item * W + 4 * c4, ak[q]);
        }
        if (bias && lane == 0) m.accBy[item] = bak;
    }
    if (G4R_DBGCLK(m) && lane == 0 && k < R) {
        const long long t_end = wall_clock64();
        GAS long long* tr = G4R_DBGCLK(m) + 64 + 8 * k;
        tr[0] = t_start; tr[1] = t_own; tr[2] = t_col; tr[3] = t_app; tr[4] = t_end; tr[5] = (owner ? fl.z : 0) | ((t_h[0] ? t_h[0] - t_app : 0) << 20); tr[6] = load_ctx(st).t;
        tr[7] = (t_h[1] - t_h[0]) | ((t_h[2] - t_h[1]) << 16) | ((t_h[3] - t_h[2]) << 32) | ((t_h[4] - t_h[3]) << 48);
    }
}

template <int MAXCH, bool MOM>
__global__ __launch_bounds__(SP_WAVES * 64, MAXCH > 2 ? 2 : 4) void k_sparse_update(const DevModel* __restrict__ mp, StepState* st, int nblk_occ) {
    extern __shared__ __attribute__((aligned(16))) float smem[];
    sparse_update_block<MAXCH, MOM>(mp, st, nblk_occ, blockIdx.x == 0 ? nblk_occ : (int)blockIdx.x - 1, smem);
}

__device__ __forceinline__ int defer_item(const DevModel& m, long long t, long long g, int k, int& table) {
    const int B = m.B, M = m.Mplan[t];
    table = 0;
    int item = -1;
    if (k < B) { if (k < M) item = m.in_idx[t * B + k]; table = (m.embed_mode == G4R_EMBED_CONSTRAINED) ? 0 : 1; }
    else if (k < 2 * B) { if (k - B < M) item = m.out_idx[t * B + (k - B)]; }
    else if (M > 0) item = m.ST[(size_t)(m.gl > 0 ? g % m.gl : 0) * m.ns + (k - 2 * B)];
    return item;
}
__global__ __launch_bounds__(256) void k_defer_scan(const DevModel* __restrict__ mp, long long t0, long long g0, int n, int pass) {
    const DevModel& m = *mp;
    const long long idx = (long long)blockIdx.x * 256 + threadIdx.x;
    const int R = m.R, s = (int)(idx / R), k = (int)(idx - (long long)s * R);
    if (s >= n) return;
    int table;
    const int item = defer_item(m, t0 + s, g0 + s, k, table);
    const size_t slot = G4R_SLOT(m, g0 + s) * (size_t)m.dRcap + k;
    if (item < 0) { if (pass) m.dcand[slot] = 0; return; }
    GAS int* lu = m.last_use + (size_t)table * m.n_items + item;
    if (pass == 0) atomicMax((int*)lu, (int)(g0 + s));
    else m.dcand[slot] = (*lu == (int)(g0 + s)) ? 1 : 0;
}
#define FL_NR 4
__global__ __launch_bounds__(SP_WAVES * 64) void k_sparse_flush(const DevModel* __restrict__ mp, long long g0, int n) {
    const DevModel& m = *mp;
    const int lane = threadIdx.x & 63, wid = threadIdx.x >> 6;
    const long long e0 = ((long long)blockIdx.x * SP_WAVES + wid) * FL_NR;
    const int Rc = m.dRcap, s = (int)(e0 / Rc), k0 = (int)(e0 - (long long)s * Rc);
    if (s >= n) return;
    const size_t slot = G4R_SLOT(m, g0 + s) * (size_t)Rc + k0;
    int it[FL_NR];
#pragma unroll
    for (int u = 0; u < FL_NR; ++u) it[u] = m.dlist[slot + u];
    if (lane < FL_NR) { m.dcand[slot + lane] = 0; m.dlist[slot + lane] = -1; }
    const int B = m.B;
    const bool sep = m.embed_mode != G4R_EMBED_CONSTRAINED;
    const GAS float *sx = G4R_DSX(m, g0 + s), *sy = G4R_DSY(m, g0 + s), *sb = G4R_DSBY(m, g0 + s);
    const float lr = m.lr, lmbd = m.lmbd;
    auto upd = [&](float p0, float sl) { const float ss = 0.f + sl; const float reg = (lmbd > 0.f) ? lr * lmbd * p0 : 0.f; return p0 - ((lmbd > 0.f) ? ss + 1.0f * reg : ss); };
    int napp = 0, nbias = 0;
    const int wmax = max(m.Ein, m.Dtop);
    if (wmax <= 256) {
        float4 p[FL_NR], g[FL_NR];
        float bp = 0.f, bs = 0.f;
#pragma unroll
        for (int u = 0; u < FL_NR; ++u) {
            const int k = k0 + u, item = max(it[u], 0);
            const bool tE = k < B && sep;
            const int W = tE ? m.Ein : m.Dtop, cc = 4 * min(lane, (W >> 2) - 1);
            const GAS float* P = tE ? m.E : m.Wy;
            const GAS float* srow = (k < B) ? sx + (size_t)min(k, B - 1) * W : sy + (size_t)(k - B) * W;
            p[u] = ld4(P + (size_t)item * W + cc);
            g[u] = ld4(it[u] >= 0 ? srow + cc : P + (size_t)item * W + cc);
            if (lane == u && it[u] >= 0 && k >= B) { bp = m.By[item]; bs = sb[k - B]; }
        }
#pragma unroll
        for (int u = 0; u < FL_NR; ++u) {
            if (it[u] < 0) continue;
            const int k = k0 + u;
            const bool tE = k < B && sep;
            const int W = tE ? m.Ein : m.Dtop;
            GAS float* P = tE ? m.E : m.Wy;
            if (lane < (W >> 2)) st4(P + (size_t)it[u] * W + 4 * lane, make_float4(upd(p[u].x, g[u].x), upd(p[u].y, g[u].y), upd(p[u].z, g[u].z), upd(p[u].w, g[u].w)));
            if (lane == u && k >= B) m.By[it[u]] = upd(bp, bs);
            ++napp; nbias += (k >= B) ? 1 : 0;
        }
    } else {
        for (int u = 0; u < FL_NR; ++u) {
            if (it[u] < 0) continue;
            const int k = k0 + u, item = it[u];
            const bool tE = k < B && sep;
            const int W = tE ? m.Ein : m.Dtop, nc4 = W >> 2;
            GAS float* P = tE ? m.E : m.Wy;
            const GAS float* srow = (k < B) ? sx + (size_t)k * W : sy + (size_t)(k - B) * W;
            float4 p[4], g[4];
#pragma unroll
            for (int q = 0; q < 4; ++q) {
                const int cc = 4 * min(lane + 64 * q, nc4 - 1);
                p[q] = ld4(P + (size_t)item * W + cc);
                g[q] = ld4(srow + cc);
            }
#pragma unroll
            for (int q = 0; q < 4; ++q)
                if (lane + 64 * q < nc4)
                    st4(P + (size_t)item * W + 4 * (lane + 64 * q), make_float4(upd(p[q].x, g[q].x), upd(p[q].y, g[q].y), upd(p[q].z, g[q].z), upd(p[q].w, g[q].w)));
            if (k >= B && lane == 0) m.By[item] = upd(m.By[item], sb[k - B]);
            ++napp; nbias += (k >= B) ? 1 : 0;
        }
    }
    if (lane == 0 && napp) { GAS unsigned* ds = m.dstat + 2 * (blockIdx.x & 1023u); atomicAdd((unsigned*)ds, (unsigned)napp); if (nbias) atomicAdd((unsigned*)ds + 1, (unsigned)nbias); }
}

static_assert(GT_NTH_FEW == SP_WAVES * 64, "both roles use the same workgroup size");
template <int MAXCH, int DT, bool MOM>
__global__ __launch_bounds__(SP_WAVES * 64, 4) void k_update(const DevModel* __restrict__ mp, StepState* st, const DenseTile* __restrict__ tiles_,
                                                             int ntiles, int nblk_occ) {
    extern __shared__ __attribute__((aligned(16))) float smem[];
    const int b = (int)blockIdx.x - 1;
    if (b < 0) sparse_update_block<MAXCH, MOM>(mp, st, nblk_occ, nblk_occ, smem);
    else if (b < ntiles) {
        const int t = G4R_XCD_TILE(b, ntiles);
        dense_grad_tile<DT>(*mp, st, tiles_, t, smem);
    } else sparse_update_block<MAXCH, MOM>(mp, st, nblk_occ, b - ntiles, smem);
}

struct XPos { int q, k; };
__device__ __forceinline__ int xlist_len(const DevModel& m) { return m.xmode == 3 ? m.xn * 2 * m.B + m.ns : m.xn * m.R; }
__device__ __forceinline__ XPos xlist_pos(const DevModel& m, int K) {
    XPos p;
    if (m.xmode == 3) {
        const int nxy = m.xn * 2 * m.B;
        if (K >= nxy) { p.q = -1; p.k = 2 * m.B + (K - nxy); }
        else { p.q = K / (2 * m.B); p.k = K - p.q * 2 * m.B; }
    } else { p.q = K / m.R; p.k = K - p.q * m.R; }
    return p;
}
__device__ __forceinline__ int xlist_item(const DevModel& m, XPos p) {
    if (p.q >= 0) return ((const GAS int*)(m.xbase + (long long)p.q * m.xstride))[p.k];
    int item = -1;
    for (int r = 0; r < m.xn; ++r) {
        const int v = ((const GAS int*)(m.xbase + (long long)r * m.xstride))[p.k];
        if (item < 0) item = v;
    }
    return item;
}
__global__ __launch_bounds__(256) void k_exact_occ(const DevModel* __restrict__ mp) {
    const DevModel& m = *mp;
    const int K = blockIdx.x * 256 + threadIdx.x, R = xlist_len(m);
    if (K >= R) return;
    const XPos ps = xlist_pos(m, K);
    const int k = ps.k;
    const int item = xlist_item(m, ps);
    if (ps.q < 0) {
        for (int r = 0; r < m.xn; ++r) {
            const int v = ((const GAS int*)(m.xbase + (long long)r * m.xstride))[k];
            if (v >= 0 && v != item) m.st->nan_flag = 2;
        }
    }
    if (item < 0) return;
    const bool tableE = (k < m.B && m.embed_mode != G4R_EMBED_CONSTRAINED);
    int* fl = (int*)m.occ_fl + 4 * ((tableE ? (size_t)m.n_items : 0) + item);
    atomicMax(fl, K + 1);
    atomicMax(fl + 1, R - K);
    atomicAdd(fl + 2, 1);
}

template <int MAXCH>
__global__ __launch_bounds__(SP_WAVES * 64, MAXCH == 1 ? 4 : 2) void k_sparse_update_generic(const DevModel* __restrict__ mp, StepState* st, int nblk_occ, int nda) {
    extern __shared__ __attribute__((aligned(16))) float smem[];
    const DevModel& m = *mp;
    const int tid = threadIdx.x, lane = tid & 63, wid = tid >> 6;
    const int B = m.B, Rl = m.R, xn = m.xn, R = xlist_len(m);
    if ((int)blockIdx.x < nda) {
        const int i = (int)blockIdx.x * (SP_WAVES * 64) + tid;
        if (i < m.dense_count) dense_apply_elem(m, i);
        return;
    }
    const int bid = (int)blockIdx.x - nda;
    if (bid == nblk_occ) {
        const StepCtx c = load_ctx(st);
        const int Mn = m.Mplan[c.t + 1];
        if (wid == 0) {
            float s = 0.f;
            for (int i = lane; i < c.M; i += 64) s += m.lossrow[i];
            s = wave_sum(s);
            if (lane == 0) {
                GAS StepState* sg = (GAS StepState*)st;
                const float cost = (sg->nan_flag == 2) ? __builtin_nanf("") : s * m.inv_B;
                m.loss_steps[c.t] = cost;
                if (isnan(cost) && sg->nan_flag == 0) sg->nan_flag = 1;
                sg->t_a = c.t + 1;
                sg->g_a = c.g + 1;
                sg->M_a = Mn;
            }
// ... 246 lines not shown
```

Before: 26460.

## Batch owner-table construction for a whole step window into one kernel

Adds k_owner_window, which builds the per-step owner tables (duplicate-occurrence positions of each item in the batch and sample lists) for all steps of a graph window in a single launch. The tables go into a 16-slot ring, and the loss kernel no longer spends extra workgroups on the owner scan for each step. k_update_l reads the slot for its step. The aim is to take owner-scan work off the critical per-step loss kernel and amortise it across the window. In exchange it uses more device memory for the ring, launches one more kernel per window, and enables this automatically only when the list is short enough to fit in LDS and long enough to pay off.

```diff
diff --git a/gru4rec_amd/build.py b/gru4rec_amd/build.py
--- a/gru4rec_amd/build.py
+++ b/gru4rec_amd/build.py
@@ -46,7 +46,9 @@
            19: "k_loss_rows' first pass starts its loop past the prefetched groups one STEP late: the columns of the first trip keep "
                "whatever the LDS held",
            20: "gumbel_noise (g4r_sample_sessions) ignores the decoding step (Philox counter word 2 = 0): every step of a draw gets the "
-               "noise of step 0"}
+               "noise of step 0",
+           21: "k_owner_window takes the sample-store row of every step of its window from the window's FIRST global step: the owner "
+               "tables of the later steps are those of another list"}
 
 
 def mutant_path(k):
diff --git a/gru4rec_amd/csrc/g4r_device.cuh b/gru4rec_amd/csrc/g4r_device.cuh
--- a/gru4rec_amd/csrc/g4r_device.cuh
+++ b/gru4rec_amd/csrc/g4r_device.cuh
@@ -9,6 +9,9 @@
 #define G4R_EPS_LOSS 1e-24f
 #define G4R_EPS_ADAGRAD 1e-6f
 #define G4R_OWN_INLINE 15
+#define G4R_OWN_SLOTS 16
+#define G4R_OWN_WINDOW_MAXR 12288
+#define G4R_OWN_WINDOW_MINWG 4
 
 #if defined(G4R_MUTATE) && G4R_MUTATE == 1
 #define G4R_MUT_ACC(x) ((x) * 1.01f)
@@ -60,6 +63,12 @@
 #define G4R_MUT_FIRST_LATE(step) (step)
 #else
 #define G4R_MUT_FIRST_LATE(step) 0
+#endif
+
+#if defined(G4R_MUTATE) && G4R_MUTATE == 21
+#define G4R_MUT_WIN_G(g0, s) (g0)
+#else
+#define G4R_MUT_WIN_G(g0, s) ((g0) + (s))
 #endif
 
 #define G4R_STREAM_SAMPLE 0x53414D50u
diff --git a/gru4rec_amd/csrc/g4r_host_create.hpp b/gru4rec_amd/csrc/g4r_host_create.hpp
--- a/gru4rec_amd/csrc/g4r_host_create.hpp
+++ b/gru4rec_amd/csrc/g4r_host_create.hpp
@@ -79,10 +79,12 @@
         m->h_leanU = u;
         const std::vector<DenseTile> tiles = dense_tiles(d, 16, 64);
         m->ntiles16 = (int)tiles.size();
-        const size_t nslot = cdiv((long long)d.R * 16 * sizeof(int), (long long)sizeof(DenseTile));
+        const size_t nslot = cdiv((long long)G4R_OWN_SLOTS * d.R * 16 * sizeof(int), (long long)sizeof(DenseTile));
         if (dalloc(m, &m->d_tiles16, tiles.size() + nslot) || dalloc(m, &m->d_leanU, (size_t)1)) return -1;
         d.own_pos = m->sw.owner_scan_in_update ? nullptr : (int*)(m->d_tiles16 + tiles.size());
         m->h_leanU.own_on = d.own_pos ? 1 : 0;
+        const bool pays = cdiv(d.R, LOSS_NW) > G4R_OWN_WINDOW_MINWG;
+        m->own_window = d.own_pos && d.R <= G4R_OWN_WINDOW_MAXR && (m->sw.owner_window > 0 || (m->sw.owner_window < 0 && pays));
         HIPCHK(hipMemcpyAsync(m->d_tiles16, tiles.data(), tiles.size() * sizeof(DenseTile), hipMemcpyHostToDevice, m->stream));
         HIPCHK(hipStreamSynchronize(m->stream));
     }
@@ -94,6 +96,7 @@
     KernelSwitches w;
     w.no_lean = getenv("G4R_NO_LEAN") != nullptr; w.no_mt = getenv("G4R_NO_MT") != nullptr; w.no_bmt = getenv("G4R_NO_BMT") != nullptr;
     w.no_merge = getenv("G4R_NO_MERGE") != nullptr; w.owner_scan_in_update = env_int("G4R_OWNER_SCAN", 0) != 0;
+    w.owner_window = env_int("G4R_OWNER_WINDOW", -1);
     w.score_b_split = env_int("G4R_SCORE_B_SPLIT", 1) != 0;
     w.allow_lean_update = env_int("G4R_LEAN_UPDATE", 1) != 0; w.defer = env_int("G4R_DEFER", cfg.defer_updates) != 0;
     w.p2_geo = env_int("G4R_P2_GEO", -1); w.ba_geo = env_int("G4R_BA_GEO", -1);
@@ -374,6 +377,7 @@
     if (m->p2p_region) (void)hipFree(m->p2p_region);
     for (auto e : m->evs) (void)hipEventDestroy(e);
     for (auto e : m->ev_df) if (e) (void)hipEventDestroy(e);
+    for (auto e : m->ev_ow) if (e) (void)hipEventDestroy(e);
     for (g4r_model::Scratch* sc : {&m->sc_ids, &m->sc_blk, &m->sc_cnt, &m->sc_all, &m->sc_send, &m->sc_pack, &m->sc_recv, &m->sc_hall}) {
         if (sc->p) { if (sc->host) (void)hipHostFree(sc->p); else (void)hipFree(sc->p); }
         sc->p = nullptr; sc->cap = 0;
diff --git a/gru4rec_amd/csrc/g4r_host_debug.hpp b/gru4rec_amd/csrc/g4r_host_debug.hpp
--- a/gru4rec_amd/csrc/g4r_host_debug.hpp
+++ b/gru4rec_amd/csrc/g4r_host_debug.hpp
@@ -57,7 +57,12 @@
     else if (s == "dyl") { p = d.dyl[l]; n = bd; }
     else if (s == "Hprev") { p = d.H[l][(m->gstep + 1) & 1]; n = bd; }
     else if (s == "occ_idx") { p = (const float*)d.occ_idx; n = d.R; }
-    else if (s == "own_pos") { if (!d.own_pos) return fail("no owner table (k_update_l not chosen, or G4R_OWNER_SCAN=1)"); p = (const float*)d.own_pos; n = 16 * (int64_t)d.R; }
+    else if (s == "own_pos") {
+        if (!d.own_pos) return fail("no owner table (k_update_l not chosen, or G4R_OWNER_SCAN=1)");
+        p = (const float*)(d.own_pos + (m->own_window ? (size_t)m->own_last * d.R * 16 : (size_t)0)); n = 16 * (int64_t)d.R;
+    }
+    else if (s == "own_pos_ring") { if (!d.own_pos) return fail("no owner table (k_update_l not chosen, or G4R_OWNER_SCAN=1)"); p = (const float*)d.own_pos; n = (int64_t)G4R_OWN_SLOTS * 16 * d.R; }
+    else if (s == "owner_window") { if (count < 1) return fail("count"); host[0] = (m->own_window && k.update == UP_LEAN) ? 1.f : 0.f; return 0; }
 #if !defined(G4R_CLK_TRACE)
     else if (s == "dbgclk" || s == "dbgtile") return fail("in-kernel traces need a library built with G4R_BUILD_CLK=1 (python -m gru4rec_amd.build --force) and G4R_CLK=1 at run time");
 #endif
diff --git a/gru4rec_amd/csrc/g4r_host_model.hpp b/gru4rec_amd/csrc/g4r_host_model.hpp
--- a/gru4rec_amd/csrc/g4r_host_model.hpp
+++ b/gru4rec_amd/csrc/g4r_host_model.hpp
@@ -22,10 +22,10 @@
     } while (0)
 
 enum { KN_GRU_P1 = 0, KN_GRU_P2, KN_SCORE_FWD, KN_LOSS, KN_SCORE_BWD, KN_BWD_PRE, KN_BWD_A, KN_BWD_B, KN_DENSE, KN_ALLREDUCE,
-       KN_DENSE_APPLY, KN_SPARSE, KN_UPDATE, KN_BWD_FUSED, KN_FWD_FUSED, KN_GATE, KN_FLUSH, KN_SCAN, KN_FINISH, KN_GRU_V, KN_GRU_H, KN_GRU_DA, KN_GRU_DY, KN_COUNT };
+       KN_DENSE_APPLY, KN_SPARSE, KN_UPDATE, KN_BWD_FUSED, KN_FWD_FUSED, KN_GATE, KN_FLUSH, KN_SCAN, KN_FINISH, KN_GRU_V, KN_GRU_H, KN_GRU_DA, KN_GRU_DY, KN_OWNER_WINDOW, KN_COUNT };
 static const char* KN_NAMES[KN_COUNT] = {"k_gru_p1", "k_gru_p2", "k_score_fwd", "k_loss_rows", "k_score_bwd", "k_gru_bwd_pre",
                                          "k_gru_bwd_a", "k_gru_bwd_b", "k_dense_grad", "rccl_allreduce", "k_dense_apply",
-                                         "k_sparse_update", "k_update", "k_gru_bwd", "k_gru_fwd", "k_gru_gate", "k_sparse_flush", "k_defer_scan", "k_finish_rows", "k_gru_v", "k_gru_h", "k_gru_da", "k_gru_dy"};
+                                         "k_sparse_update", "k_update", "k_gru_bwd", "k_gru_fwd", "k_gru_gate", "k_sparse_flush", "k_defer_scan", "k_finish_rows", "k_gru_v", "k_gru_h", "k_gru_da", "k_gru_dy", "k_owner_window"};
 
 struct EvRec { int kn; hipEvent_t a, b; };
 
@@ -36,6 +36,7 @@
     bool allow_lean_update = true;
     bool score_b_split = true;
     bool owner_scan_in_update = false;
+    int owner_window = -1;
     bool defer = false;
     int p2_geo = -1, ba_geo = -1;
     int wide2 = -1, p1_ks = 128, bb_ks = 0;
@@ -107,6 +108,9 @@
     LeanB* d_leanB = nullptr; LeanB h_leanB;
     LeanU* d_leanU = nullptr; LeanU h_leanU;
     DenseTile* d_tiles16 = nullptr; int ntiles16 = 0;
+    bool own_window = false;
+    int own_last = 0;
+    hipEvent_t ev_ow[2] = {nullptr, nullptr};
     LeanV* d_leanV = nullptr; LeanH* d_leanH = nullptr; LeanDa* d_leanDa = nullptr; LeanDy* d_leanDy = nullptr;
     hipGraphExec_t gexec = nullptr;
     hipGraphExec_t gexec_small = nullptr;
@@ -288,6 +292,7 @@
 static const size_t SMEM_SBW = std::max(tile_smem<64, 64, 64, true, false>(), tile_smem<64, 64, 64, false, false>());
 #define ZROW_FLOATS 8192
 #define G4R_DEFER_SLOTS 16
+static_assert(G4R_OWN_SLOTS == G4R_DEFER_SLOTS, "the windows of g4r_train_steps serve the deferral ring and the owner ring alike");
 static const size_t SMEM_SF = tile_smem<SF_BM, GT_BN, GT_BK, false, true>() + GT_BN * sizeof(int);
 static constexpr auto k_score_mt_4s = k_score_mt<4, true>;
 static const size_t SMEM_MT_4S = (size_t)MtCfg<4, true>::SMEM_FLOATS * sizeof(float);
diff --git a/gru4rec_amd/csrc/g4r_host_step.hpp b/gru4rec_amd/csrc/g4r_host_step.hpp
--- a/gru4rec_amd/csrc/g4r_host_step.hpp
+++ b/gru4rec_amd/csrc/g4r_host_step.hpp
@@ -20,7 +20,7 @@
 #undef G4R_LK_LOSS1
 }
 
-static int launch_step(g4r_model* m, std::vector<EvRec>* recs, int part = 0) {
+static int launch_step(g4r_model* m, std::vector<EvRec>* recs, int part = 0, int slot = 0) {
     DevModel& d = m->dm;
     const StepKernels& k = m->kern;
     const int L = d.n_layers, B = d.B;
@@ -128,7 +128,7 @@
     begin(KN_LOSS);
     {
         const int nown = std::min(cdiv(d.R, LOSS_NW), std::max(2 * m->n_cu - B, 32));
-        const dim3 gloss(B + (merged && k.update == UP_LEAN && d.own_pos ? nown : 0));
+        const dim3 gloss(B + (merged && k.update == UP_LEAN && d.own_pos && !m->own_window ? nown : 0));
         if (!(m->sw.skip_kn && ((m->sw.skip_kn >> KN_LOSS) & 1ull))) launch_loss_rows(m, gloss, recs != nullptr, cur_a, cur_b);
     }
     end();
@@ -226,10 +226,11 @@
             const unsigned packA = (unsigned)m->ntiles16 | ((unsigned)nb8 << 16), packB = (unsigned)d.R | ((unsigned)B << 16);
             const unsigned nbk = 1u + (unsigned)cdiv(d.ldSc, 512);
             const dim3 gl(nbk + m->ntiles16 + nb8);
+            const int* opos = (const int*)(m->d_tiles16 + m->ntiles16) + (m->own_window ? (size_t)slot * d.R * 16 : (size_t)0);
             if (mo) LK(k_update_l<true>, gl, dim3(512), 0, s, (const LeanU*)m->d_leanU, (const DenseTile*)m->d_tiles16, (const int*)d.occ_idx, (int*)d.occ_fl,
-                       (const float*)d.dSx, (const float*)d.dSy, (const float*)d.dSBy, packA, packB, nbk);
+                       (const float*)d.dSx, (const float*)d.dSy, (const float*)d.dSBy, opos, packA, packB, nbk);
             else LK(k_update_l<false>, gl, dim3(512), 0, s, (const LeanU*)m->d_leanU, (const DenseTile*)m->d_tiles16, (const int*)d.occ_idx, (int*)d.occ_fl,
-                    (const float*)d.dSx, (const float*)d.dSy, (const float*)d.dSBy, packA, packB, nbk);
+                    (const float*)d.dSx, (const float*)d.dSy, (const float*)d.dSBy, opos, packA, packB, nbk);
             end();
             HIPCHK(hipGetLastError());
             return 0;
@@ -354,7 +355,7 @@
     hipGraph_t graph = nullptr;
     HIPCHK(hipStreamBeginCapture(m->stream, rccl_in_graph ? hipStreamCaptureModeRelaxed : hipStreamCaptureModeThreadLocal));
     int rc = 0;
-    for (int i = 0; i < G4R_GRAPH_STEPS && !rc; ++i) rc = launch_step(m, nullptr);
+    for (int i = 0; i < G4R_GRAPH_STEPS && !rc; ++i) rc = launch_step(m, nullptr, 0, i);
     hipError_t e = hipStreamEndCapture(m->stream, &graph);
     if (rc || e != hipSuccess || !graph) {
         if (graph) (void)hipGraphDestroy(graph);
@@ -370,7 +371,7 @@
         hipGraph_t g2 = nullptr;
         if (hipStreamBeginCapture(m->stream, hipStreamCaptureModeThreadLocal) == hipSuccess) {
             int rc2 = 0;
-            for (int i = 0; i < G4R_GRAPH_STEPS_SMALL && !rc2; ++i) rc2 = launch_step(m, nullptr);
+            for (int i = 0; i < G4R_GRAPH_STEPS_SMALL && !rc2; ++i) rc2 = launch_step(m, nullptr, 0, i);
             hipError_t e2 = hipStreamEndCapture(m->stream, &g2);
             if (!rc2 && e2 == hipSuccess && g2 && hipGraphInstantiate(&m->gexec_small, g2, nullptr, nullptr, 0) != hipSuccess) m->gexec_small = nullptr;
             if (g2) (void)hipGraphDestroy(g2);
@@ -443,16 +444,36 @@
         if (m->dm.ns > 0 && !m->store_frozen) run = std::min<int64_t>(run, m->gl - (m->gstep % m->gl));
         if (run <= 0) return fail("internal: empty run");
         int64_t done = 0;
-        auto window_open = [&](int64_t nw) {
-            if (!m->defer_on) return;
+        const bool own_win = m->own_window && m->kern.update == UP_LEAN && !(m->profiling && m->profile_split);
+        auto window_open = [&](int64_t nw) -> int {
+            if (own_win && !((m->sw.skip_kn >> KN_OWNER_WINDOW) & 1ull)) {
+                const DevModel& d = m->dm;
+                const bool timed = m->profiling;
+                if (timed) for (auto& e : m->ev_ow) if (!e) (void)hipEventCreate(&e);
+                const dim3 gw((unsigned)(nw * cdiv(2 * d.B, OW_NW)));
+                const size_t lds = (size_t)(((d.R + 3) & ~3) + 16 * OW_NW) * sizeof(int);
+                if (timed) hipExtLaunchKernelGGL(k_owner_window, gw, dim3(OW_T), lds, m->stream, m->ev_ow[0], m->ev_ow[1], 0, (const DevModel*)m->d_dm, (long long)(t + done), (long long)(m->gstep + done), (int)nw);
+                else hipLaunchKernelGGL(k_owner_window, gw, dim3(OW_T), lds, m->stream, (const DevModel*)m->d_dm, (long long)(t + done), (long long)(m->gstep + done), (int)nw);
+                HIPCHK(hipGetLastError());
+            }
+            if (!m->defer_on) return 0;
             wguard.open = true;
             const dim3 gs(cdiv(nw * m->dm.R, 256));
             if (m->profiling) (void)hipEventRecord(m->ev_df[0], m->stream);
             hipLaunchKernelGGL(k_defer_scan, gs, dim3(256), 0, m->stream, (const DevModel*)m->d_dm, (long long)(t + done), (long long)(m->gstep + done), (int)nw, 0);
             hipLaunchKernelGGL(k_defer_scan, gs, dim3(256), 0, m->stream, (const DevModel*)m->d_dm, (long long)(t + done), (long long)(m->gstep + done), (int)nw, 1);
             if (m->profiling) (void)hipEventRecord(m->ev_df[1], m->stream);
+            return 0;
         };
         auto window_close = [&](int64_t nw, int64_t first) -> int {
+            if (own_win) {
+                m->own_last = (int)nw - 1;
+                if (m->profiling) {
+                    HIPCHK(hipStreamSynchronize(m->stream));
+                    float ms = 0.f;
+                    if (hipEventElapsedTime(&ms, m->ev_ow[0], m->ev_ow[1]) == hipSuccess) { m->kn_ms[KN_OWNER_WINDOW] += ms; m->kn_n[KN_OWNER_WINDOW]++; }
+                }
+            }
             if (!m->defer_on) return 0;
             if (m->profiling) (void)hipEventRecord(m->ev_df[2], m->stream);
             hipLaunchKernelGGL(k_sparse_flush, dim3(cdiv(nw * m->dm.dRcap, SP_WAVES * FL_NR)), dim3(SP_WAVES * 64), 0, m->stream, (const DevModel*)m->d_dm, (long long)(m->gstep + first), (int)nw);
@@ -469,26 +490,27 @@
         if (use_graph && run >= G4R_GRAPH_STEPS_SMALL) {
             if (ensure_graph(m)) return -1;
             for (; done + m->graph_steps <= run; done += m->graph_steps) {
-                window_open(m->graph_steps);
+                if (window_open(m->graph_steps)) return -1;
                 HIPCHK(hipGraphLaunch(m->gexec, m->stream));
                 if (window_close(m->graph_steps, done)) return -1;
             }
             if (m->gexec_small)
                 for (; done + G4R_GRAPH_STEPS_SMALL <= run; done += G4R_GRAPH_STEPS_SMALL) {
-                    window_open(G4R_GRAPH_STEPS_SMALL);
+                    if (window_open(G4R_GRAPH_STEPS_SMALL)) return -1;
                     HIPCHK(hipGraphLaunch(m->gexec_small, m->stream));
                     if (window_close(G4R_GRAPH_STEPS_SMALL, done)) return -1;
                 }
         }
         int64_t win_first = -1, win_n = 0;
         for (; done < run; ++done) {
-            if (m->defer_on && win_n == 0) {
+            if ((m->defer_on || own_win) && win_n == 0) {
                 win_n = std::min<int64_t>(G4R_DEFER_SLOTS, run - done); win_first = done;
-                window_open(win_n);
-            }
+                if (window_open(win_n)) return -1;
+            }
+            const int slot = win_n > 0 ? (int)(done - win_first) : 0;
             if (m->profiling) {
                 recs.clear();
-                if (launch_step(m, &recs)) return -1;
+                if (launch_step(m, &recs, 0, slot)) return -1;
                 HIPCHK(hipStreamSynchronize(m->stream));
                 for (auto& r : recs) {
                     float ms = 0.f;
@@ -498,7 +520,7 @@
                 if (ensure_head_graph(m)) return -1;
                 HIPCHK(hipGraphLaunch(m->gexec_head, m->stream));
                 if (launch_step(m, nullptr, 2)) return -1;
-            } else if (launch_step(m, nullptr)) return -1;
+            } else if (launch_step(m, nullptr, 0, slot)) return -1;
             if (win_n > 0 && done + 1 == win_first + win_n) {
                 if (window_close(win_n, win_first)) return -1;
                 win_n = 0;
diff --git a/gru4rec_amd/csrc/g4r_lean_kernels.cuh b/gru4rec_amd/csrc/g4r_lean_kernels.cuh
--- a/gru4rec_amd/csrc/g4r_lean_kernels.cuh
+++ b/gru4rec_amd/csrc/g4r_lean_kernels.cuh
@@ -1059,7 +1059,8 @@
 
 template <bool MOM>
 __global__ __launch_bounds__(512) void k_update_l(const LeanU* __restrict__ ap, const DenseTile* __restrict__ tiles_, const int* occ_idx_, int* occ_fl_,
-                                                  const float* dSx_, const float* dSy_, const float* dSBy_, unsigned packA, unsigned packB, unsigned nbk) {
+                                                  const float* dSx_, const float* dSy_, const float* dSBy_, const int* opos_, unsigned packA, unsigned packB,
+                                                  unsigned nbk) {
     const unsigned ntiles = packA & 0xFFFFu, nblk = packA >> 16, R = packB & 0xFFFFu, B = packB >> 16;
     const LeanU a = *ap;
     LSPAN_BEGIN(a.dbgtile, 2700);
@@ -1068,8 +1069,8 @@
     if (b < ntiles) { lean_dense_tile<MOM>(a, tiles_, b, B); LSPAN_END(); return; }
     const unsigned q = b - ntiles, wid = __builtin_amdgcn_readfirstlane(threadIdx.x >> 6);
     lean_rows_update<MOM>(a, (const GAS int*)occ_idx_, (GAS int*)occ_fl_, (const GAS float*)dSx_, (const GAS float*)dSy_, (const GAS float*)dSBy_,
-                          (const GAS int*)(tiles_ + ntiles), wid * nblk + q, R, B);
+                          (const GAS int*)opos_, wid * nblk + q, R, B);
     LSPAN_END();
 }
-template __global__ void k_update_l<false>(const LeanU*, const DenseTile*, const int*, int*, const float*, const float*, const float*, unsigned, unsigned, unsigned);
-template __global__ void k_update_l<true>(const LeanU*, const DenseTile*, const int*, int*, const float*, const float*, const float*, unsigned, unsigned, unsigned);
+template __global__ void k_update_l<false>(const LeanU*, const DenseTile*, const int*, int*, const float*, const float*, const float*, const int*, unsigned, unsigned, unsigned);
+template __global__ void k_update_l<true>(const LeanU*, const DenseTile*, const int*, int*, const float*, const float*, const float*, const int*, unsigned, unsigned, unsigned);
diff --git a/gru4rec_amd/csrc/g4r_loss_kernel.cuh b/gru4rec_amd/csrc/g4r_loss_kernel.cuh
--- a/gru4rec_amd/csrc/g4r_loss_kernel.cuh
+++ b/gru4rec_amd/csrc/g4r_loss_kernel.cuh
@@ -105,7 +105,7 @@
     const int jt = V * tid;
     constexpr int LOSS_PRE = (V == 4) ? 2 : 4;
 #if defined(G4R_CLK_TRACE)
-    struct Span { GAS long long* p; __device__ ~Span() { if (p) p[1] = wall_clock64(); } } span_{(m.dbgtile && tid == 0 && i < 1024) ? m.dbgtile + 8 * (size_t)(7168 + i) : nullptr};
+    struct Span { GAS long long* p; __device__ ~Span() { if (p) p[1] = wall_clock64(); } } span_{(m.dbgtile && tid == 0 && i < 532) ? m.dbgtile + 8 * (size_t)(7168 + i) : nullptr};
     if (span_.p) span_.p[0] = wall_clock64();
 #endif
     const StepCtx c = load_ctx(st);
diff --git a/gru4rec_amd/csrc/g4r_update_kernels.cuh b/gru4rec_amd/csrc/g4r_update_kernels.cuh
--- a/gru4rec_amd/csrc/g4r_update_kernels.cuh
+++ b/gru4rec_amd/csrc/g4r_update_kernels.cuh
@@ -539,6 +539,86 @@
     GAS int* lu = m.last_use + (size_t)table * m.n_items + item;
     if (pass == 0) atomicMax((int*)lu, (int)(g0 + s));
     else m.dcand[slot] = (*lu == (int)(g0 + s)) ? 1 : 0;
+}
+#define OW_T 1024
+#define OW_NW (OW_T / 64)
+static_assert(G4R_OWN_INLINE + 1 == 16, "an owner-table row is 16 ints: the count and G4R_OWN_INLINE positions");
+static_assert(((size_t)G4R_OWN_WINDOW_MAXR + 16 * OW_NW) * sizeof(int) <= 65536, "k_owner_window: the longest list and the waves' position rows share one workgroup's 64 KB of LDS");
+__global__ __launch_bounds__(OW_T) void k_owner_window(const DevModel* __restrict__ mp, long long t0, long long g0, int nw) {
+    const DevModel& m = *mp;
+    extern __shared__ __attribute__((aligned(16))) int sid[];
+    const int R = m.R, B = m.B, Rp = (R + 3) & ~3;
+    const int gps = (2 * B + OW_NW - 1) / OW_NW;
+    const int s = (int)blockIdx.x / gps, q = (int)blockIdx.x - s * gps;
+#if defined(G4R_CLK_TRACE)
+    struct Span { GAS long long* p; __device__ ~Span() { if (p) p[1] = wall_clock64(); } } span_{(m.dbgtile && threadIdx.x == 0 && blockIdx.x < 400) ? m.dbgtile + 8 * (size_t)(7700 + blockIdx.x) : nullptr};
+    if (span_.p) span_.p[0] = wall_clock64();
+#endif
+    if (s >= nw) return;
+    for (int k = threadIdx.x; k < Rp; k += OW_T) {
+        int table;
+        sid[k] = k < R ? defer_item(m, t0 + s, G4R_MUT_WIN_G(g0, s), k, table) : -1;
+    }
+    __syncthreads();
+    const int lane = threadIdx.x & 63, wid = threadIdx.x >> 6;
+    const int p = q * OW_NW + wid;
+    if (p >= 2 * B) return;
+    const int item = sid[p];
+    if (item < 0) return;
+    const bool constrained = m.embed_mode == G4R_EMBED_CONSTRAINED;
+    const int ta = (constrained || p < B) ? 0 : B, tb = (!constrained && p < B) ? B : R;
+    int* spos = sid + Rp + 16 * wid;
+    const unsigned long long below = (1ull << lane) - 1ull;
+    int cnt = 0, last = p;
+    for (int base0 = ta & ~3; base0 < tb; base0 += 1024) {
+        int4 vv[4];
+#pragma unroll
+        for (int u = 0; u < 4; ++u) vv[u] = *(const int4*)(sid + min(base0 + 256 * u + 4 * lane, Rp - 4));
+#pragma unroll
+        for (int u = 0; u < 4; ++u) {
+            const int j0 = base0 + 256 * u + 4 * lane;
+            const int ids[4] = {vv[u].x, vv[u].y, vv[u].z, vv[u].w};
+            bool hit[4], anyl = false;
+#pragma unroll
+            for (int e = 0; e < 4; ++e) { hit[e] = ids[e] == item && j0 + e >= ta && j0 + e < tb; anyl = anyl || hit[e]; }
+            if (__ballot(anyl) == 0ull) continue;
+            unsigned long long mk[4];
+            int at = cnt;
+#pragma unroll
+            for (int e = 0; e < 4; ++e) {
+                mk[e] = __ballot(hit[e]);
+                at += __popcll(mk[e] & below);
+            }
+            const unsigned long long any = mk[0] | mk[1] | mk[2] | mk[3];
+            if (cnt == 0) {
+                const int l0 = __builtin_ctzll(any);
+                int e0 = 3;
+#pragma unroll
+                for (int e = 2; e >= 0; --e) if ((mk[e] >> l0) & 1ull) e0 = e;
+                if (base0 + 256 * u + 4 * l0 + e0 != p) return;
+            }
+            const int lh = 63 - __builtin_clzll(any);
+#pragma unroll
+            for (int e = 0; e < 4; ++e) if ((mk[e] >> lh) & 1ull) last = base0 + 256 * u + 4 * lh + e;
+#pragma unroll
+            for (int e = 0; e < 4; ++e) {
+                if (hit[e]) {
+                    if (at <= G4R_OWN_INLINE) spos[at] = j0 + e;
+                    ++at;
+                }
+                cnt += __popcll(mk[e]);
+            }
+        }
+    }
+    if (cnt < 2) return;
+    GAS int* pos = m.own_pos + ((size_t)s * (size_t)R + (size_t)last) * 16;
+    if (cnt - 1 > G4R_OWN_INLINE) {
+        if (lane == 0) pos[0] = -1;
+        return;
+    }
+    __builtin_amdgcn_fence(__ATOMIC_ACQ_REL, "wavefront");
+    if (lane < cnt - 1) pos[1 + lane] = spos[lane];
+    if (lane == 0) pos[0] = cnt - 1;
 }
 #define FL_NR 4
 __global__ __launch_bounds__(SP_WAVES * 64) void k_sparse_flush(const DevModel* __restrict__ mp, long long g0, int n) {
```

Result: faster. 27020 (median of 6 runs) (+2.1%).
